# facebookresearch/momentum

Hardware: AMD Instinct MI355X
Metric: character IK solves/sec (72-joint, 10 GN iters) (higher is better)
Workload: dtype f32; 1 GPU; BASELINE configs[1]: B x 72-joint humanoid, P=128, pos+ori on 16 landmarks (M=192), GN lambda=0.05, 10 it; batch_per_gpu=4096, global_batch=4096, joints=72, params=128, rows=192, solved_parameters=96, route=fused, line_search=0, precision=f32

## Files before the change

### include/mmx.h

```cpp
#ifndef MMX_H_
#define MMX_H_

#include <stddef.h>
#include <stdint.h>

#ifdef __cplusplus
extern "C" {
#endif

#define MMX_ABI_VERSION 12
#define MMX_PARAMS_PER_JOINT 7
#define MMX_INVALID_PARENT (-1)
#define MMX_MAX_MODEL_PARAMS 2048

typedef enum mmx_status {
  MMX_OK = 0,
  MMX_ERR_INVALID_ARGUMENT = 1,
  MMX_ERR_SIZE_MISMATCH = 2,
  MMX_ERR_DEVICE = 3,
  MMX_ERR_UNSUPPORTED = 4,
  MMX_ERR_OUT_OF_MEMORY = 5,
  MMX_ERR_NO_DEVICE = 6
} mmx_status;

// ... 135 lines not shown
} mmx_gn_options;

typedef struct mmx_rig mmx_rig;
typedef struct mmx_problem mmx_problem;

void mmx_gn_options_default(mmx_gn_options* opt);

int32_t mmx_abi_version(void);
const char* mmx_last_error(void);
int32_t mmx_device_count(void);

int32_t mmx_rig_create(const mmx_rig_desc* desc, int32_t device, mmx_rig** out);
void mmx_rig_destroy(mmx_rig* rig);
int32_t mmx_rig_num_joints(const mmx_rig* rig);
int32_t mmx_rig_num_params(const mmx_rig* rig);

int32_t mmx_problem_create(
    mmx_rig* rig,
    int32_t batch,
    int32_t num_pos,
    const int32_t* pos_parent,
    int32_t num_ori,
    const int32_t* ori_parent,
    mmx_problem** out);
void mmx_problem_destroy(mmx_problem* problem);

int32_t mmx_problem_set_instance_rig(
    mmx_problem* problem,
    const float* translation_offset,
    const float* pre_rotation,
    int32_t memory,
    void* stream);

int32_t mmx_problem_set_instance_parents(
    mmx_problem* problem,
    const int32_t* pos_parent,
    const int32_t* ori_parent,
    int32_t memory,
    void* stream);

#define MMX_ROUTE_AUTO 0
#define MMX_ROUTE_FUSED 1
#define MMX_ROUTE_WIDE 2
#define MMX_ROUTE_EXPLICIT_JACOBIAN 3
#define MMX_ROUTE_WAVE 4
#define MMX_WAVE_MAX_JOINTS 64
#define MMX_WAVE_MAX_SOLVED 32
#define MMX_WAVE_MAX_UNITS 192
typedef struct mmx_tuning {
  int32_t route;
  int32_t max_refinement_steps;
  float mixed_tolerance;
  int32_t mixed_max_cg;
  int32_t reserved[4];
} mmx_tuning;
int32_t mmx_problem_set_tuning(mmx_problem* problem, const mmx_tuning* tuning);
int32_t mmx_problem_last_route(const mmx_problem* problem);

int32_t mmx_problem_num_rows(const mmx_problem* problem);
int32_t mmx_problem_batch(const mmx_problem* problem);

int32_t mmx_problem_set_enabled(mmx_problem* problem, const uint8_t* enabled);

int32_t mmx_problem_set_constraints(
    mmx_problem* problem,
    const mmx_constraint_data* data,
    void* stream);
int32_t mmx_problem_set_constraints_sized(
    mmx_problem* problem,
    const mmx_constraint_data* data,
    size_t data_size,
    void* stream);

int32_t mmx_eval_jacobian(
    mmx_problem* problem,
    const float* theta_dev,
    float* jac_dev,
    float* res_dev,
    double* err_dev,
    int32_t layout,
    void* stream);

int32_t mmx_eval_jacobian_timed(
    mmx_problem* problem,
    const float* theta_dev,
    float* jac_dev,
    float* res_dev,
    double* err_dev,
    int32_t layout,
    void* stream,
    float* kernel_ms);

int32_t mmx_debug_store_pattern(mmx_problem* problem, float* jac_dev, void* stream, float* kernel_ms);

int32_t mmx_eval_skeleton_state(
    mmx_problem* problem,
    const float* theta_dev,
    float* state_dev,
    void* stream);

int32_t mmx_eval_normal_equations(
    mmx_problem* problem,
    const float* theta_dev,
    float* jtj_dev,
    float* jtr_dev,
    double* err_dev,
    void* stream);

int32_t mmx_solve(
    mmx_problem* problem,
// ... 48 lines not shown
    int32_t* solve_list_host,
    int32_t* num_solved,
    void* stream);

int32_t mmx_debug_tree_normal_equations(mmx_problem* problem, const float* theta_dev, float* jtj_dev, float* jtr_dev, void* stream);

int32_t mmx_solve_host(
    mmx_problem* problem,
    const mmx_gn_options* options,
    float* theta_host,
    double* final_error_host,
    int32_t* iterations_host,
    int32_t* status_host);
int32_t mmx_solve_f64_host(
    mmx_problem* problem,
    const mmx_gn_options* options,
    double* theta_host,
    double* final_error_host,
    int32_t* iterations_host,
    int32_t* status_host);
int32_t mmx_eval_jacobian_host(
    mmx_problem* problem,
    const float* theta_host,
    float* jac_host,
    float* res_host,
    double* err_host,
    int32_t layout);
int32_t mmx_eval_skeleton_state_host(mmx_problem* problem, const float* theta_host, float* state_host);

#define MMX_COMM_ID_BYTES 128
typedef struct mmx_comm mmx_comm;
int32_t mmx_comm_unique_id(uint8_t id[MMX_COMM_ID_BYTES]);
int32_t mmx_comm_create(const uint8_t id[MMX_COMM_ID_BYTES], int32_t world_size, int32_t rank, int32_t device, mmx_comm** out);
int32_t mmx_comm_create_all(int32_t num_devices, const int32_t* devices, mmx_comm** out );
int32_t mmx_comm_world_size(const mmx_comm* comm);
int32_t mmx_comm_rank(const mmx_comm* comm);
int32_t mmx_comm_all_reduce_norms(mmx_comm* comm, double* norms_dev, void* stream);
int32_t mmx_comm_all_reduce_norms_host(mmx_comm* comm, double norms_host[3]);
int32_t mmx_residual_norms(int32_t batch, const double* final_error, const int32_t* iterations, const int32_t* status, double* norms_dev, void* stream);
void mmx_comm_destroy(mmx_comm* comm);

int32_t mmx_host_tables(
    const mmx_rig_desc* desc,
    const uint8_t* enabled,
    int32_t* level,
    int32_t* tin,
    int32_t* tout,
    uint8_t* active_joint_params,
    int32_t* enabled_list,
    int32_t* num_enabled);

int32_t mmx_host_elimination_order(const mmx_rig_desc* desc, const uint8_t* enabled, int32_t* order, int32_t* num_enabled);
int32_t mmx_host_tile_structure(int32_t n, const uint8_t* related, uint32_t* row_mask, uint32_t* col_mask, int64_t* products);
int32_t mmx_problem_tile_structure(mmx_problem* problem, uint32_t* row_mask, uint32_t* col_mask, int32_t* num_blocks, int32_t* num_tiles, int64_t* products);
int32_t mmx_host_tile_level_schedule(int32_t n, const uint8_t* related, int32_t* steps);
int32_t mmx_host_f64_assembly_list(
    const mmx_rig_desc* desc,
    const int32_t* solve_list,
    int32_t n,
    const int32_t* pos_parent,
    int32_t num_pos,
    const int32_t* ori_parent,
    int32_t num_ori,
    int32_t units_per_chunk,
    uint32_t* groups,
    int32_t* num_groups,
    int32_t* extra,
    int32_t* num_extra,
    int32_t* chunk_start,
    int32_t* num_chunks);

#ifdef __cplusplus
}
#endif
#endif
```

### momentum_amd/_abi.py

```python
from __future__ import annotations

import ctypes as C

import numpy as np

c_float_p = C.POINTER(C.c_float)
c_double_p = C.POINTER(C.c_double)
c_int32_p = C.POINTER(C.c_int32)
c_uint8_p = C.POINTER(C.c_uint8)

MMX_ABI_VERSION = 12
MMX_OK = 0
MMX_SOLVE_OK, MMX_SOLVE_NONFINITE, MMX_SOLVE_NOT_PD = 0, 1, 2
MMX_SOLVE_DAMPING_FLOORED = 4
MMX_SOLVE_PRECISION_SUSPECT = 8
MMX_SOLVE_ESCALATED_F64 = 16
MMX_SOLVE_MIXED = 32
MMX_SOLVE_ERROR_MASK = 3
MMX_PRECISION_F32, MMX_PRECISION_F64, MMX_PRECISION_AUTO, MMX_PRECISION_MIXED = 0, 1, 2, 3
MMX_MEM_HOST, MMX_MEM_DEVICE = 0, 1
MMX_LAYOUT_COL_MAJOR, MMX_LAYOUT_ROW_MAJOR = 0, 1
MMX_STEP_GN_FIXED_LAMBDA, MMX_STEP_LM_SCHEDULE, MMX_STEP_TRUST_REGION = 0, 1, 2


# ... 249 lines not shown
        ("do_line_search", C.c_int32),
        ("step_rule", C.c_int32),
        ("lm_lambda_min", C.c_float),
        ("lm_lambda_max", C.c_float),
        ("lm_up", C.c_float),
        ("lm_down", C.c_float),
        ("trust_region_radius", C.c_float),
        ("precision", C.c_int32),
        ("precision_bound", C.c_float),
    ]

    @classmethod
    def make(
        cls,
        min_iterations=1,
        max_iterations=2,
        threshold=1.0,
        regularization=0.05,
        do_line_search=False,
        step_rule=MMX_STEP_GN_FIXED_LAMBDA,
        lm_lambda_min=1e-6,
        lm_lambda_max=1e6,
        lm_up=4.0,
        lm_down=0.5,
        trust_region_radius=1.0,
        precision=MMX_PRECISION_F32,
        precision_bound=1e-5,
    ) -> "GnOptions":
        return cls(
            int(min_iterations),
            int(max_iterations),
            float(threshold),
            float(regularization),
            int(do_line_search),
            int(step_rule),
            float(lm_lambda_min),
            float(lm_lambda_max),
            float(lm_up),
            float(lm_down),
            float(trust_region_radius),
            int(precision),
            float(precision_bound),
        )


ROUTES = {"auto": 0, "fused": 1, "wide": 2, "explicit_jacobian": 3, "wave": 4}
WAVE_MAX_JOINTS = 64
WAVE_MAX_SOLVED = 32
WAVE_MAX_UNITS = 192


class Tuning(C.Structure):

    _fields_ = [("route", C.c_int32), ("max_refinement_steps", C.c_int32), ("mixed_tolerance", C.c_float), ("mixed_max_cg", C.c_int32), ("reserved", C.c_int32 * 4)]


def as_ptr(a: np.ndarray, ctype):
    assert a.flags["C_CONTIGUOUS"], "array must be C-contiguous"
    return a.ctypes.data_as(C.POINTER(ctype))


def void_p(a) -> C.c_void_p:
    if a is None:
        return C.c_void_p(0)
    if isinstance(a, np.ndarray):
        assert a.flags["C_CONTIGUOUS"]
        return C.c_void_p(a.ctypes.data)
    return C.c_void_p(int(a))
```

### momentum_amd/capi.py

```python
from __future__ import annotations

import ctypes as C
import os
from typing import Optional

import numpy as np

from . import _abi
from ._abi import ConstraintData, GnOptions, RigDesc, as_ptr
from .rigs import Rig

_HERE = os.path.dirname(os.path.abspath(__file__))
LIB_PATH = os.environ.get("MMX_LIB") or os.path.join(_HERE, "libmmx_hip.so")
_lib: Optional[C.CDLL] = None

SYMBOLS = [
    "mmx_gn_options_default", "mmx_abi_version", "mmx_last_error", "mmx_device_count",
    "mmx_rig_create", "mmx_rig_destroy", "mmx_rig_num_joints", "mmx_rig_num_params",
    "mmx_problem_create", "mmx_problem_destroy", "mmx_problem_num_rows", "mmx_problem_batch",
    "mmx_problem_set_tuning", "mmx_problem_last_route",
    "mmx_problem_set_enabled", "mmx_problem_set_constraints", "mmx_problem_set_constraints_sized", "mmx_problem_set_instance_rig", "mmx_problem_set_instance_parents", "mmx_eval_jacobian", "mmx_eval_jacobian_timed", "mmx_debug_store_pattern",
    "mmx_eval_skeleton_state", "mmx_eval_normal_equations", "mmx_solve", "mmx_solve_with_history", "mmx_solve_with_step_history", "mmx_problem_solve_diagnostics", "mmx_solve_f64", "mmx_solve_f64_host", "mmx_solve_host",
    "mmx_eval_jacobian_host", "mmx_eval_skeleton_state_host", "mmx_host_tables", "mmx_debug_fused_normal_equations", "mmx_debug_tree_normal_equations",
    "mmx_host_elimination_order", "mmx_host_tile_structure", "mmx_host_tile_level_schedule", "mmx_host_f64_assembly_list", "mmx_problem_tile_structure",
    "mmx_comm_unique_id", "mmx_comm_create", "mmx_comm_create_all", "mmx_comm_world_size", "mmx_comm_rank",
    "mmx_comm_all_reduce_norms", "mmx_comm_all_reduce_norms_host", "mmx_residual_norms", "mmx_comm_destroy",
]


class MmxError(RuntimeError):

    def __init__(self, code: int, msg: str):
        super().__init__(f"mmx error {code}: {msg}")
        self.code = code


def lib() -> C.CDLL:
    global _lib
    if _lib is not None:
        return _lib
    if not os.path.exists(LIB_PATH):
        raise MmxError(-1, f"{LIB_PATH} is missing: build it with `python -m momentum_amd.build` (no CPU fallback exists)")
    try:
        import torch
    except Exception:
        pass
    L = C.CDLL(LIB_PATH)
    vp, i32 = C.c_void_p, C.c_int32
    L.mmx_last_error.restype = C.c_char_p
    L.mmx_gn_options_default.restype = None
    L.mmx_gn_options_default.argtypes = [C.POINTER(GnOptions)]
    L.mmx_rig_create.argtypes = [C.POINTER(RigDesc), i32, C.POINTER(vp)]
    L.mmx_rig_destroy.argtypes = [vp]
    L.mmx_rig_destroy.restype = None
    L.mmx_rig_num_joints.argtypes = [vp]
    L.mmx_rig_num_params.argtypes = [vp]
    L.mmx_problem_create.argtypes = [vp, i32, i32, _abi.c_int32_p, i32, _abi.c_int32_p, C.POINTER(vp)]
    L.mmx_problem_destroy.argtypes = [vp]
    L.mmx_problem_destroy.restype = None
    L.mmx_problem_num_rows.argtypes = [vp]
    L.mmx_problem_batch.argtypes = [vp]
    L.mmx_problem_set_enabled.argtypes = [vp, _abi.c_uint8_p]
    L.mmx_problem_set_tuning.argtypes = [vp, C.POINTER(_abi.Tuning)]
    L.mmx_problem_last_route.argtypes = [vp]
    L.mmx_problem_set_constraints.argtypes = [vp, C.POINTER(ConstraintData), vp]
    L.mmx_problem_set_constraints_sized.argtypes = [vp, C.POINTER(ConstraintData), C.c_size_t, vp]
    L.mmx_problem_set_instance_rig.argtypes = [vp, vp, vp, i32, vp]
    L.mmx_problem_set_instance_parents.argtypes = [vp, vp, vp, i32, vp]
    L.mmx_eval_jacobian.argtypes = [vp, vp, vp, vp, vp, i32, vp]
    L.mmx_eval_jacobian_timed.argtypes = [vp, vp, vp, vp, vp, i32, vp, C.POINTER(C.c_float)]
    L.mmx_debug_store_pattern.argtypes = [vp, vp, vp, C.POINTER(C.c_float)]
    L.mmx_eval_skeleton_state.argtypes = [vp, vp, vp, vp]
    L.mmx_eval_normal_equations.argtypes = [vp, vp, vp, vp, vp, vp]
    L.mmx_solve.argtypes = [vp, C.POINTER(GnOptions), vp, vp, vp, vp, vp, vp]
    L.mmx_solve_with_history.argtypes = [vp, C.POINTER(GnOptions), vp, vp, vp, vp, vp, vp, vp]
    L.mmx_solve_with_step_history.argtypes = [vp, C.POINTER(GnOptions), vp, vp, vp, vp, vp, vp, vp, vp]
    L.mmx_problem_solve_diagnostics.argtypes = [vp, vp, vp]
    L.mmx_solve_f64.argtypes = [vp, C.POINTER(GnOptions), vp, vp, vp, vp, vp, vp]
    L.mmx_solve_host.argtypes = [vp, C.POINTER(GnOptions), vp, vp, vp, vp]
    L.mmx_solve_f64_host.argtypes = [vp, C.POINTER(GnOptions), vp, vp, vp, vp]
    L.mmx_eval_jacobian_host.argtypes = [vp, vp, vp, vp, vp, i32]
    L.mmx_eval_skeleton_state_host.argtypes = [vp, vp, vp]
    L.mmx_debug_tree_normal_equations.argtypes = [vp, vp, vp, vp, vp]
    L.mmx_debug_fused_normal_equations.argtypes = [vp, vp, vp, vp, _abi.c_int32_p, _abi.c_int32_p, vp]
    L.mmx_comm_unique_id.argtypes = [vp]
    L.mmx_comm_create.argtypes = [vp, i32, i32, i32, C.POINTER(vp)]
    L.mmx_comm_create_all.argtypes = [i32, _abi.c_int32_p, C.POINTER(vp)]
    L.mmx_comm_world_size.argtypes = [vp]
    L.mmx_comm_rank.argtypes = [vp]
    L.mmx_comm_all_reduce_norms.argtypes = [vp, vp, vp]
    L.mmx_comm_all_reduce_norms_host.argtypes = [vp, vp]
    L.mmx_residual_norms.argtypes = [i32, vp, vp, vp, vp, vp]
    L.mmx_comm_destroy.argtypes = [vp]
    L.mmx_comm_destroy.restype = None
    L.mmx_host_tables.argtypes = [
        C.POINTER(RigDesc), _abi.c_uint8_p, _abi.c_int32_p, _abi.c_int32_p, _abi.c_int32_p,
        _abi.c_uint8_p, _abi.c_int32_p, _abi.c_int32_p,
    ]
    u32p, i64p = C.POINTER(C.c_uint32), C.POINTER(C.c_int64)
    L.mmx_host_elimination_order.argtypes = [C.POINTER(RigDesc), _abi.c_uint8_p, _abi.c_int32_p, _abi.c_int32_p]
    L.mmx_host_tile_structure.argtypes = [i32, _abi.c_uint8_p, u32p, u32p, i64p]
    L.mmx_host_tile_level_schedule.argtypes = [i32, _abi.c_uint8_p, C.POINTER(C.c_int32)]
    L.mmx_problem_tile_structure.argtypes = [vp, u32p, u32p, _abi.c_int32_p, _abi.c_int32_p, i64p]
    _lib = L
    return L


def _check(rc: int) -> None:
    if rc != 0:
        raise MmxError(rc, lib().mmx_last_error().decode("utf-8", "replace"))


def device_count() -> int:
    return int(lib().mmx_device_count())


def host_tables(rig: Rig, enabled=None) -> dict:
    J, P = rig.num_joints, rig.num_params
    level, tin, tout = (np.zeros(J, np.int32) for _ in range(3))
    active = np.zeros(7 * J, np.uint8)
    elist = np.zeros(P, np.int32)
    n = C.c_int32(0)
    d = rig.desc()
    if enabled is None:
        eptr = _abi.c_uint8_p()
    else:
        e = np.ascontiguousarray(enabled, dtype=np.uint8)
        eptr = as_ptr(e, C.c_uint8)
    _check(
        lib().mmx_host_tables(
            C.byref(d), eptr, as_ptr(level, C.c_int32), as_ptr(tin, C.c_int32), as_ptr(tout, C.c_int32),
            as_ptr(active, C.c_uint8), as_ptr(elist, C.c_int32), C.byref(n),
        )
    )
    order = np.zeros(P, np.int32)
    _check(lib().mmx_host_elimination_order(C.byref(d), eptr, as_ptr(order, C.c_int32), C.byref(n)))
    return dict(level=level, tin=tin, tout=tout, active_joint_params=active, enabled_list=elist[: n.value].copy(),
                elimination_order=order[: n.value].copy())


def host_tile_structure(related: np.ndarray):
    rel = np.ascontiguousarray(related, dtype=np.uint8)
    n = rel.shape[0]
    assert rel.shape == (n, n)
    row, col = np.zeros(32, np.uint32), np.zeros(32, np.uint32)
    prod = C.c_int64(0)
    _check(lib().mmx_host_tile_structure(C.c_int32(n), as_ptr(rel, C.c_uint8), as_ptr(row, C.c_uint32), as_ptr(col, C.c_uint32), C.byref(prod)))
    return dict(row_mask=row, col_mask=col, products=prod.value)


def host_tile_level_schedule(related: np.ndarray):
    rel = np.ascontiguousarray(related, dtype=np.uint8)
    n = rel.shape[0]
    assert rel.shape == (n, n)
    words = np.zeros(1 + 4 * 32, np.int32)
    _check(lib().mmx_host_tile_level_schedule(C.c_int32(n), as_ptr(rel, C.c_uint8), as_ptr(words, C.c_int32)))
    steps = []
    for s in range(int(words[0])):
        steps.append([(int(w) & 0xff, (int(w) >> 8) & 0xf, (int(w) >> 12) & 0xf) for w in words[1 + 4 * s : 5 + 4 * s] if w >= 0])
    return steps


def host_f64_assembly_list(rig: Rig, solve_list, pos_parent, ori_parent, units_per_chunk: int):
    sl = np.ascontiguousarray(solve_list, dtype=np.int32)
    pp = np.ascontiguousarray(pos_parent, dtype=np.int32)
    op = np.ascontiguousarray(ori_parent, dtype=np.int32)
    d = rig.desc()
    ng, ne, nc = C.c_int32(0), C.c_int32(0), C.c_int32(0)
    i32p = C.POINTER(C.c_int32)
    args = lambda g, e, cs: (C.byref(d), as_ptr(sl, C.c_int32), C.c_int32(len(sl)), as_ptr(pp, C.c_int32), C.c_int32(len(pp)), as_ptr(op, C.c_int32),
                             C.c_int32(len(op)), C.c_int32(units_per_chunk), g, C.byref(ng), e, C.byref(ne), cs, C.byref(nc))
    f = lib().mmx_host_f64_assembly_list
    f.restype = C.c_int32
    _check(f(*args(None, None, None)))
    groups = np.zeros(2 * max(ng.value, 1), np.uint32)
    extra = np.zeros(max(ne.value, 1), np.int32)
    cstart = np.zeros(2 * nc.value + 1, np.int32)
    _check(f(*args(groups.ctypes.data_as(C.POINTER(C.c_uint32)), extra.ctypes.data_as(i32p), cstart.ctypes.data_as(i32p))))
    chunks = []
    for ch in range(nc.value):
        entries = []
        for g in range(cstart[ch], cstart[ch + 1]):
            w0, w1 = int(groups[2 * g]), int(groups[2 * g + 1])
            c, ul, count = w0 & 0xfff, (w0 >> 12) & 0x3f, w0 >> 18
            entries.append((c, ul, [w1] if count == 1 else [int(x) for x in extra[w1 : w1 + count]]))
        chunks.append(dict(block_mask=int(cstart[nc.value + 1 + ch]), entries=entries))
    return chunks


def _stream_ptr() -> C.c_void_p:
    import torch
# ... 26 lines not shown
            pass


default_route = "auto"


class Problem:

    def __init__(self, rig_handle: RigHandle, batch: int, pos_parent, ori_parent):
        import torch

        self.rh = rig_handle
        self.B = int(batch)
        self.P = rig_handle.rig.num_params
        self.J = rig_handle.rig.num_joints
        self.pos_parent = np.ascontiguousarray(pos_parent, dtype=np.int32).reshape(-1)
        self.ori_parent = np.ascontiguousarray(ori_parent, dtype=np.int32).reshape(-1)
        self.Kp, self.Ko = len(self.pos_parent), len(self.ori_parent)
        self.M = 3 * self.Kp + 9 * self.Ko
        self.n = self.P
        self.device = torch.device("cuda", rig_handle.device)
        self._h = C.c_void_p(0)
        self._keep = []
        _check(
            lib().mmx_problem_create(
                rig_handle._h, self.B, self.Kp, as_ptr(self.pos_parent, C.c_int32), self.Ko,
                as_ptr(self.ori_parent, C.c_int32), C.byref(self._h),
            )
        )
        self._prefer_wide = default_route == "prefer_wide"
        if default_route not in ("auto", "prefer_wide"):
            self.set_route(default_route)

    def close(self) -> None:
        if self._h:
            lib().mmx_problem_destroy(self._h)
            self._h = C.c_void_p(0)

    def __del__(self):
        try:
            self.close()
        except Exception:
            pass

    def set_route(self, route: str, max_refinement_steps: int = 0) -> None:
        self._prefer_wide = default_route == "prefer_wide" and route == "auto"
        self._set_tuning(route, max_refinement_steps)

    def _set_tuning(self, route: str, max_refinement_steps: int = 0) -> None:
        t = _abi.Tuning()
        t.route = _abi.ROUTES[route]
        t.max_refinement_steps = int(max_refinement_steps)
        t.mixed_tolerance, t.mixed_max_cg = getattr(self, "_mixed", (0.0, 0))
        self._route_args = (route, int(max_refinement_steps))
        _check(lib().mmx_problem_set_tuning(self._h, C.byref(t)))

    def set_mixed(self, tolerance: float = 0.0, max_cg: int = 0) -> None:
        self._mixed = (float(tolerance), int(max_cg))
        self._set_tuning(*getattr(self, "_route_args", ("auto", 0)))

    def last_route(self) -> str:
        r = int(lib().mmx_problem_last_route(self._h))
        return {v: k for k, v in _abi.ROUTES.items()}[r]

    def set_enabled(self, enabled) -> None:
        e = np.ascontiguousarray(enabled, dtype=np.uint8).reshape(-1)
        assert e.shape[0] == self.P
        _check(lib().mmx_problem_set_enabled(self._h, as_ptr(e, C.c_uint8)))
        self.n = int(np.count_nonzero(e))

    def set_constraints(
        self, pos_offset, pos_target, pos_weight, ori_offset, ori_target, ori_weight,
        pos_function_weight: float = 1.0, ori_function_weight: float = 1.0,
        limits=None, limit_function_weight: float = 1.0,
        model_target=None, model_weights=None, model_function_weight: float = 1.0,
        pos_loss=(2.0, 1.0), ori_loss=(2.0, 1.0), joint_blocks=None, ellipsoid_limits=None, function_weights=None,
    ) -> None:
        import torch

        arrs = [pos_offset, pos_target, pos_weight, ori_offset, ori_target, ori_weight]
        shapes = [(self.B, self.Kp, 3), (self.B, self.Kp, 3), (self.B, self.Kp), (self.B, self.Ko, 4), (self.B, self.Ko, 4), (self.B, self.Ko)]
        if model_target is not None:
            arrs += [model_target, model_weights]
            shapes += [(self.B, self.P), (self.B, self.P)]
        on_dev = all(isinstance(a, torch.Tensor) for a in arrs)
        keep, ptrs = [], []
        for a, shp in zip(arrs, shapes):
            if on_dev:
                assert a.is_cuda and a.dtype == torch.float32 and a.is_contiguous() and tuple(a.shape) == shp, (a.shape, shp)
                keep.append(a)
                ptrs.append(C.c_void_p(a.data_ptr() if a.numel() else 0))
            else:
                x = np.ascontiguousarray(a, dtype=np.float32).reshape(shp)
                keep.append(x)
                ptrs.append(C.c_void_p(x.ctypes.data if x.size else 0))
        if model_target is None:
            ptrs += [C.c_void_p(0), C.c_void_p(0)]
        fw_ptr, fw_cols = C.c_void_p(0), 0
        if function_weights is not None:
            if on_dev:
                assert function_weights.is_cuda and function_weights.dtype == torch.float32 and function_weights.is_contiguous() and function_weights.shape[0] == self.B
                keep.append(function_weights)
                fw_ptr, fw_cols = C.c_void_p(function_weights.data_ptr()), int(function_weights.shape[1])
            else:
                fwh = np.ascontiguousarray(function_weights, dtype=np.float32).reshape(self.B, -1)
                keep.append(fwh)
                fw_ptr, fw_cols = C.c_void_p(fwh.ctypes.data), int(fwh.shape[1])
        limits = list(limits) if limits else []
        larr = _abi.limit_array(limits)
        blocks = list(joint_blocks) if joint_blocks else []
        bkeep: list = []
        barr = _abi.joint_block_array(blocks, bkeep, self.B, on_dev)
# ... 285 lines not shown
```

### momentum_amd/csrc/mmx_capi.hip

```cpp
#include "../../include/mmx.h"

#include <hip/hip_runtime.h>

#include <dlfcn.h>

#include <cfloat>
#include <cmath>
#include <cstdio>
#include <cstdlib>
#include <cstring>
#include <algorithm>
#include <new>
#include <map>
#include <memory>
#include <string>
#include <vector>

#include "mmx_host_tables.hpp"
#include "mmx_kernels.hpp"

namespace {

thread_local std::string g_lastError;

// ... 142 lines not shown
  DevBuf oInstOffset, oInstPreRot, oInstPosParent, oInstOriParent, dJointTin;
  std::vector<int32_t> unionPos, unionOri;
  std::vector<int32_t> instPosHost, instOriHost;
  bool instParentsFromHost = false;
  bool instPos = false, instOri = false;
  mmx::HostTables tables;
  mmx::FusedTables fused;
  DevBuf dUnitJoint, dUnitTin, dColStart, dColSources, dEnabledList, dJacRecs, dMultiCols, dZeroCols;
  DevBuf dSubSize, dPosUnitStart, dPosUnits, dSolveList, dSrcStart, dSrcs, dTerms, dTerms16, dComb, dDfsJoint, dLoadedPos;
  DevBuf dLimStart, dLimOf, dPairDest, dPairStart, dPairLim, dPairCols;
  mmx::FusedDev fdev{};
  DevBuf oPosOffset, oPosTarget, oPosWeight, oOriOffset, oOriTarget, oOriWeight, oMpTarget, oMpWeights, dLimits, dEnabledMask, oFnWeights;
  std::vector<mmx_parameter_limit> limits;
  struct JointBlockHost {
    int32_t type = 0, count = 0;
    std::vector<int32_t> parent;
    std::vector<int32_t> parentB;
    DevBuf oLocalPoint, oLocalDir, oGlobal, oPlaneD, oWeight, oProjection;
  };
  std::vector<std::unique_ptr<JointBlockHost>> blocks;
  std::vector<mmx::JointBlockDev> blockDev;
  std::vector<mmx_ellipsoid_limit> ellipsoids;
  DevBuf dEllipsoids;
  DevBuf dBlocks, dGenJoint, dGenTin, dGenBlock;
  int32_t genRows = 0;
  bool haveConstraints = false;
  bool tablesDirty = false;
  mmx::ProblemDev dev{};
  int32_t solveN = 0;
  DevBuf dSolveListV1;
  DevBuf sHess2F64;
  DevBuf dSolveListF64;
  std::vector<int32_t> solveListF64;
  std::vector<std::pair<int32_t, int32_t>> limitPairs;
  DevBuf dTileMasks, dTileList;
  mmx::TileMasks tileMasks;
  std::vector<int32_t> solveListV1;
  DevBuf sJac, sRes, sErr, sJtj, sJtr, sFactor, sThetaInit, sTheta;
  DevBuf sTreeState, sDvec, sRhoVec, sRefState, sGenState;
  DevBuf sJacColMajor;
  DevBuf sJacF64, sHessF64;
  DevBuf dF64Groups, dF64Extra, dF64ChunkStart;
  int32_t f64ListUnitsPerChunk = 0;
  DevBuf sDone, sIters, sStatus, sLastErr, sFinalErr, sHist, sClk, sDelta, sStepIter, sLambda, sTrust;
  DevBuf sFusedArgs;
  DevBuf sDiag;
  DevBuf sDiagAcc;
  DevBuf sDiagErr0;
  bool diagValid = false;
  DevBuf sThetaAuto, sAutoMap, sAutoCount;
  bool autoAbort = false;
  mmx_tuning tuning{};
  int32_t lastRoute = MMX_ROUTE_AUTO;
};

namespace {

std::vector<int32_t> limitParameters(const mmx_rig* rig, const mmx_parameter_limit& lm) {
  std::vector<int32_t> out;
  auto add = [&](int32_t p) {
    if (std::find(out.begin(), out.end(), p) == out.end()) {
      out.push_back(p);
    }
  };
  auto addRow = [&](int32_t row) {
    for (int32_t k = rig->ptOuter[size_t(row)]; k < rig->ptOuter[size_t(row) + 1]; ++k) {
      add(rig->ptInner[size_t(k)]);
    }
  };
  switch (lm.type) {
    case MMX_LIMIT_MINMAX:
      add(lm.index0);
      break;
    case MMX_LIMIT_LINEAR:
    case MMX_LIMIT_HALFPLANE:
      add(lm.index0);
      add(lm.index1);
      break;
    case MMX_LIMIT_MINMAX_JOINT:
      addRow(lm.index0);
      break;
    case MMX_LIMIT_LINEAR_JOINT:
      addRow(lm.index1);
      addRow(lm.index0);
      break;
    default:
      break;
  }
  return out;
}

int32_t uploadProblemTables(mmx_problem* pb) {
  const mmx_rig* rig = pb->rig;
  MMX_HIP(hipSetDevice(rig->device));
  const mmx::HostTables& t = pb->tables;
  std::vector<int32_t> unitJoint(size_t(std::max(pb->U, 1))), unitTin(size_t(std::max(pb->U, 1)));
  for (int32_t c = 0; c < pb->Kp; ++c) {
    unitJoint[c] = pb->posParent[c];
  }
  for (int32_t c = 0; c < pb->Ko; ++c) {
    for (int k = 0; k < 3; ++k) {
      unitJoint[pb->Kp + 3 * c + k] = pb->oriParent[c];
    }
  }
  for (int32_t u = 0; u < pb->U; ++u) {
    unitTin[u] = t.tin[unitJoint[u]];
  }
  static_assert(sizeof(mmx::ColumnSource) == sizeof(mmx::ColumnSourceDev), "ColumnSource layouts must match");
  MMX_HIP(upload(pb->dUnitJoint, unitJoint));
  MMX_HIP(upload(pb->dUnitTin, unitTin));
  MMX_HIP(upload(pb->dJointTin, t.tin));
  pb->dev.jointTin = pb->dJointTin.as<int32_t>();
  {
    std::vector<int32_t> gj, gt, gb, gj2, gt2;
    for (size_t i = 0; i < pb->blocks.size(); ++i) {
      const mmx_problem::JointBlockHost& h = *pb->blocks[i];
      for (size_t c = 0; c < h.parent.size(); ++c) {
        const int32_t j = h.parent[c], j2 = h.parentB.empty() ? -1 : h.parentB[c];
        gj.push_back(j);
        gt.push_back(t.tin[size_t(j)]);
        gb.push_back(int32_t(i));
        gj2.push_back(j2);
        gt2.push_back(j2 < 0 ? -1 : t.tin[size_t(j2)]);
      }
    }
    const size_t G = gb.size();
    gj.insert(gj.end(), gj2.begin(), gj2.end());
    gt.insert(gt.end(), gt2.begin(), gt2.end());
    MMX_HIP(upload(pb->dGenJoint, gj));
    MMX_HIP(upload(pb->dGenTin, gt));
    MMX_HIP(upload(pb->dGenBlock, gb));
    MMX_HIP(upload(pb->dBlocks, pb->blockDev));
    pb->dev.numBlocks = int32_t(pb->blocks.size());
    pb->dev.G = int32_t(G);
    pb->dev.blocks = pb->dBlocks.as<mmx::JointBlockDev>();
    pb->dev.genJoint = pb->dGenJoint.as<int32_t>();
    pb->dev.genTin = pb->dGenTin.as<int32_t>();
    pb->dev.genBlock = pb->dGenBlock.as<int32_t>();
    std::vector<mmx::EllipsoidDev> ed(pb->ellipsoids.size());
    for (size_t i = 0; i < ed.size(); ++i) {
      const mmx_ellipsoid_limit& e = pb->ellipsoids[i];
      static_assert(sizeof(mmx_ellipsoid_limit) == 30 * 4 && sizeof(mmx::EllipsoidDev) == 32 * 4, "ellipsoid layouts");
// ... 317 lines not shown
      std::map<int32_t, std::vector<int32_t>> pairs;
      std::map<int32_t, std::pair<int32_t, int32_t>> pairColumns;
      for (size_t l = 0; l < pb->limits.size(); ++l) {
        std::vector<int32_t> cols;
        for (int32_t p : limitParameters(rig, pb->limits[l])) {
          if (colOf[size_t(p)] >= 0) {
            cols.push_back(colOf[size_t(p)]);
          }
        }
        for (int32_t c : cols) {
          per[size_t(c)].push_back(int32_t(l));
        }
        for (size_t x = 0; x < cols.size(); ++x) {
          for (size_t y = x + 1; y < cols.size(); ++y) {
            const int32_t row = std::max(cols[x], cols[y]), col = std::min(cols[x], cols[y]);
            const int I = row >> 4, Jc = col >> 4, r = row & 15, c = col & 15;
            const int32_t dest = (I * (I + 1) / 2 + Jc) * 256 + r * 16 + ((((c >> 2) ^ (r >> 2)) & 3) << 2) + (c & 3);
            pairs[dest].push_back(int32_t(l));
            pairColumns[dest] = {row, col};
          }
        }
      }
      std::vector<int32_t> limStart(1, 0), limOf, pairDest, pairStart(1, 0), pairLim;
      for (int32_t c = 0; c < fd.n; ++c) {
        limOf.insert(limOf.end(), per[size_t(c)].begin(), per[size_t(c)].end());
        limStart.push_back(int32_t(limOf.size()));
      }
      std::vector<int32_t> pairCols;
      for (const auto& kv : pairs) {
        pairDest.push_back(kv.first);
        pairCols.push_back(pairColumns[kv.first].first);
        pairCols.push_back(pairColumns[kv.first].second);
        pb->limitPairs.push_back(pairColumns[kv.first]);
        pairLim.insert(pairLim.end(), kv.second.begin(), kv.second.end());
        pairStart.push_back(int32_t(pairLim.size()));
      }
      MMX_HIP(upload(pb->dPairCols, pairCols));
      fd.pairCols = pb->dPairCols.as<int32_t>();
      MMX_HIP(upload(pb->dLimStart, limStart));
      MMX_HIP(upload(pb->dLimOf, limOf));
      MMX_HIP(upload(pb->dPairDest, pairDest));
      MMX_HIP(upload(pb->dPairStart, pairStart));
      MMX_HIP(upload(pb->dPairLim, pairLim));
      fd.numLimits = int32_t(pb->limits.size());
      fd.limStart = pb->dLimStart.as<int32_t>();
      fd.limOf = pb->dLimOf.as<int32_t>();
      fd.numPairDests = int32_t(pairDest.size());
      fd.pairDest = pb->dPairDest.as<int32_t>();
      fd.pairStart = pb->dPairStart.as<int32_t>();
      fd.pairLim = pb->dPairLim.as<int32_t>();
    }
    pb->fdev.GT = pb->dev.G + int32_t(pb->ellipsoids.size());
    pb->fdev.genRows = pb->fdev.GT > 0 ? pb->dev.rowsJoint - 3 * pb->U : 0;
  }
  {
    const size_t J = size_t(rig->J);
    std::vector<uint8_t> anyBelow(J, 0), pointBelow(J, 0);
    auto mark = [&](int32_t joint, bool point) {
      for (int32_t a = joint; a >= 0; a = rig->parent[size_t(a)]) {
        anyBelow[size_t(a)] = 1;
        if (point) {
          pointBelow[size_t(a)] = 1;
        }
      }
    };
    for (int32_t c = 0; c < pb->Kp; ++c) {
      mark(pb->posParent[size_t(c)], true);
    }
    for (int32_t c = 0; c < pb->Ko; ++c) {
      mark(pb->oriParent[size_t(c)], false);
    }
    if (pb->instPos) {
      for (int32_t j : pb->unionPos) {
        mark(j, true);
      }
    }
    if (pb->instOri) {
      for (int32_t j : pb->unionOri) {
        mark(j, false);
      }
    }
    for (const auto& h : pb->blocks) {
      const bool fixedAxis = h->type == MMX_JC_FIXED_AXIS_DIFF || h->type == MMX_JC_FIXED_AXIS_COS || h->type == MMX_JC_FIXED_AXIS_ANGLE;
      for (int32_t j : h->parent) {
        mark(j, !fixedAxis);
      }
      for (int32_t j : h->parentB) {
        mark(j, true);
      }
    }
    for (const mmx_ellipsoid_limit& e : pb->ellipsoids) {
      mark(e.parent, true);
    }
    std::vector<uint8_t> keep(size_t(rig->P), pb->dev.hasModel ? 1 : 0);
    for (const mmx_parameter_limit& lm : pb->limits) {
      for (int32_t p : limitParameters(rig, lm)) {
        keep[size_t(p)] = 1;
      }
    }
    std::vector<int32_t> list;
    for (int32_t p : t.eliminationList) {
      bool nz = keep[size_t(p)] != 0;
      for (int32_t e = t.colStart[size_t(p)]; !nz && e < t.colStart[size_t(p) + 1]; ++e) {
        const mmx::ColumnSource& cs = t.colSources[size_t(e)];
        nz = (cs.dof >= 3 && cs.dof < 6) ? anyBelow[size_t(cs.joint)] != 0 : pointBelow[size_t(cs.joint)] != 0;
      }
// ... 25 lines not shown
        for (int32_t e = f.srcStart[size_t(c)]; e < f.srcStart[size_t(c) + 1]; ++e) {
          const mmx::ColumnSource& cs = f.srcs[size_t(e)];
          for (int32_t k = cs.tin; k < cs.tout; ++k) {
            rc[size_t(f.dfsJoint[size_t(k)])] = 1;
          }
          for (int32_t a = cs.parent; a >= 0; a = rig->parent[size_t(a)]) {
            rc[size_t(a)] = 1;
          }
        }
      }
      related.assign(size_t(n) * size_t(n), 0);
      for (int32_t row = 0; row < n; ++row) {
        for (int32_t col = 0; col < row; ++col) {
          const uint8_t* rc = reach.data() + size_t(col) * J;
          bool any = false;
          for (int32_t e = f.srcStart[size_t(row)]; !any && e < f.srcStart[size_t(row) + 1]; ++e) {
            any = rc[size_t(f.srcs[size_t(e)].joint)] != 0;
          }
          related[size_t(row) * size_t(n) + size_t(col)] = any ? 1 : 0;
        }
      }
      for (const auto& rcPair : pb->limitPairs) {
        related[size_t(rcPair.first) * size_t(n) + size_t(rcPair.second)] = 1;
      }
    }
    pb->tileMasks = mmx::eliminationTileMasks(std::min(n, 512), related, dense);
    std::vector<uint32_t> masks(96, 0u);
    uint32_t base = 0;
    for (int i = 0; i < 32; ++i) {
      masks[size_t(i)] = pb->tileMasks.rowMask[i];
      masks[size_t(32 + i)] = pb->tileMasks.colMask[i];
      masks[size_t(64 + i)] = base;
      base += uint32_t(__builtin_popcount(pb->tileMasks.colMask[i]));
    }
    for (int k = 0; k < pb->tileMasks.NB && k < 32; ++k) {
      for (int I = k; I < 32; ++I) {
        if (pb->tileMasks.colMask[k] >> I & 1u) {
          masks.push_back(uint32_t(I) | uint32_t(k) << 8);
        }
      }
    }
    for (int32_t w : pb->tileMasks.levelSteps) {
      masks.push_back(uint32_t(w));
    }
    MMX_HIP(upload(pb->dTileMasks, masks));
    MMX_HIP(upload(pb->dTileList, pb->tileMasks.tiles));
    pb->fdev.tileList = pb->dTileList.as<int32_t>();
    pb->fdev.numTiles = int32_t(pb->tileMasks.tiles.size());
  }

  return MMX_OK;
}

bool fusedUsable(const mmx_problem* pb) {
  const int nb = mmx::fusedBlocksFor(pb->fdev.n);
  if (nb < 0) {
    return false;
  }
  return pb->rig->J < 4096 &&
      mmx::fusedLdsBytes(nb, pb->rig->J, pb->rig->P, pb->U, pb->fdev.nsrc, pb->fdev.n, pb->fdev.numCells, true, pb->fdev.GT, pb->fdev.genRows, true, mmx::fusedCsrFloats(pb->rig->J, pb->fdev.nnz)) +
          size_t(8) * size_t(pb->rig->J + pb->rig->P) <=
      160 * 1024;
}

bool treeNormalEquationsUsable(const mmx_problem* pb) {
  return pb->U > 0 && pb->fdev.n > 0 && pb->fdev.n <= 512 && pb->fdev.nsrc < 4096 &&
      pb->fused.solveList == pb->solveListV1 &&
      mmx::treeNormalEquationsLdsBytes(pb->rig->J, pb->rig->P, pb->U, pb->fdev.nsrc, pb->fdev.n, pb->fdev.GT, pb->fdev.genRows) <= 160 * 1024 - 64 &&
      mmx::treeRefineLdsBytes(pb->rig->J, pb->rig->P, pb->U, pb->fdev.n, pb->fdev.genRows) <= 160 * 1024 - 64;
}

int32_t refineSteps(const mmx_problem* pb) {
  const int32_t m = pb->tuning.max_refinement_steps;
  return m == 0 ? 3 : (m < 0 ? 0 : (m > 3 ? 3 : m));
}

bool phaseClocksWanted() {
  static const bool wanted = getenv("MMX_PHASE_CLOCKS") != nullptr;
  return wanted;
}

hipError_t armPhaseStop(long long* clk, hipStream_t s) {
  static const long long stop = getenv("MMX_PHASE_STOP") != nullptr ? atoll(getenv("MMX_PHASE_STOP")) + 1 : 0;
  return stop > 0 ? hipMemcpyAsync(clk + 31, &stop, sizeof(long long), hipMemcpyHostToDevice, s) : hipSuccess;
}

int32_t checkProblem(const mmx_problem* pb, bool needConstraints) {
  (void)hipGetLastError();
  if (pb == nullptr || pb->rig == nullptr) {
    return fail(MMX_ERR_INVALID_ARGUMENT, "problem handle is null");
  }
  if (needConstraints && !pb->haveConstraints && pb->U > 0) {
    return fail(MMX_ERR_INVALID_ARGUMENT, "mmx_problem_set_constraints has not been called");
  }
  return MMX_OK;
}

}

extern "C" {

void mmx_gn_options_default(mmx_gn_options* o) {
  if (o == nullptr) {
    return;
  }
  o->min_iterations = 1;
// ... 26 lines not shown
    return 0;
  }
  return n;
}

int32_t mmx_host_tables(
    const mmx_rig_desc* desc,
    const uint8_t* enabled,
    int32_t* level,
    int32_t* tin,
    int32_t* tout,
    uint8_t* active_joint_params,
    int32_t* enabled_list,
    int32_t* num_enabled) {
  mmx::HostTables t;
  std::string err;
  const int32_t rc = mmx::buildHostTables(desc, enabled, t, err);
  if (rc != MMX_OK) {
    return fail(rc, err);
  }
  if (level) {
    std::memcpy(level, t.level.data(), sizeof(int32_t) * t.J);
  }
  if (tin) {
    std::memcpy(tin, t.tin.data(), sizeof(int32_t) * t.J);
  }
  if (tout) {
    std::memcpy(tout, t.tout.data(), sizeof(int32_t) * t.J);
  }
  if (active_joint_params) {
    std::memcpy(active_joint_params, t.activeJointParams.data(), t.activeJointParams.size());
  }
  if (enabled_list) {
    std::memcpy(enabled_list, t.enabledList.data(), sizeof(int32_t) * t.enabledList.size());
  }
  if (num_enabled) {
    *num_enabled = int32_t(t.enabledList.size());
  }
  return MMX_OK;
}

int32_t mmx_host_elimination_order(const mmx_rig_desc* desc, const uint8_t* enabled, int32_t* order, int32_t* num_enabled) {
  mmx::HostTables t;
  std::string err;
  const int32_t rc = mmx::buildHostTables(desc, enabled, t, err);
  if (rc != MMX_OK) {
    return fail(rc, err);
  }
  if (order) {
    std::memcpy(order, t.eliminationList.data(), sizeof(int32_t) * t.eliminationList.size());
  }
  if (num_enabled) {
    *num_enabled = int32_t(t.eliminationList.size());
  }
  return MMX_OK;
}

int32_t mmx_host_tile_structure(int32_t n, const uint8_t* related, uint32_t* row_mask, uint32_t* col_mask, int64_t* products) {
  if (n < 0 || n > 512 || (n > 0 && related == nullptr)) {
    return fail(MMX_ERR_INVALID_ARGUMENT, "mmx_host_tile_structure: n outside 0..512 or related is null");
  }
  const std::vector<uint8_t> rel(related, related + size_t(n) * size_t(n));
  const mmx::TileMasks m = mmx::eliminationTileMasks(n, rel, false);
  for (int i = 0; i < 32; ++i) {
    if (row_mask) {
      row_mask[i] = m.rowMask[i];
    }
    if (col_mask) {
      col_mask[i] = m.colMask[i];
    }
  }
  if (products) {
    *products = m.products;
  }
  return MMX_OK;
}

int32_t mmx_host_tile_level_schedule(int32_t n, const uint8_t* related, int32_t* steps) {
  if (n < 0 || n > 512 || (n > 0 && related == nullptr) || steps == nullptr) {
    return fail(MMX_ERR_INVALID_ARGUMENT, "mmx_host_tile_level_schedule: n outside 0..512, or related / steps is null");
  }
  const std::vector<uint8_t> rel(related, related + size_t(n) * size_t(n));
  const mmx::TileMasks m = mmx::eliminationTileMasks(n, rel, false);
  if (m.levelSteps.size() > size_t(1 + 4 * 32)) {
    return fail(MMX_ERR_UNSUPPORTED, "mmx_host_tile_level_schedule: more than 32 steps");
  }
  std::copy(m.levelSteps.begin(), m.levelSteps.end(), steps);
  return MMX_OK;
}

int32_t mmx_host_f64_assembly_list(
    const mmx_rig_desc* desc,
    const int32_t* solve_list,
    int32_t n,
    const int32_t* pos_parent,
    int32_t num_pos,
    const int32_t* ori_parent,
    int32_t num_ori,
    int32_t units_per_chunk,
    uint32_t* groups,
    int32_t* num_groups,
    int32_t* extra,
    int32_t* num_extra,
    int32_t* chunk_start,
    int32_t* num_chunks) {
  if (n < 0 || num_pos < 0 || num_ori < 0 || units_per_chunk <= 0 || units_per_chunk > 64 || (n > 0 && solve_list == nullptr) ||
// ... 82 lines not shown
    return fail(rc, err);
  }
  const int ndev = mmx_device_count();
  if (ndev <= 0) {
    return fail(MMX_ERR_NO_DEVICE, "no HIP device visible; the MI355X path has no CPU fallback");
  }
  if (device < 0 || device >= ndev) {
    return fail(MMX_ERR_INVALID_ARGUMENT, "device index out of range");
  }
  mmx_rig* r = new (std::nothrow) mmx_rig();
  if (r == nullptr) {
    return fail(MMX_ERR_OUT_OF_MEMORY, "host allocation failed");
  }
  r->device = device;
  r->J = d->num_joints;
  r->P = d->num_params;
  const int32_t R = MMX_PARAMS_PER_JOINT * r->J;
  r->parent.assign(d->parent, d->parent + r->J);
  r->preRot.assign(d->pre_rotation, d->pre_rotation + 4 * r->J);
  r->offset.assign(d->translation_offset, d->translation_offset + 3 * r->J);
  r->ptOuter.assign(d->pt_outer, d->pt_outer + R + 1);
  const int32_t nnz = r->ptOuter[R];
  r->ptInner.assign(d->pt_inner, d->pt_inner + nnz);
  r->ptValue.assign(d->pt_value, d->pt_value + nnz);
  if (d->pt_offsets != nullptr) {
    r->ptOffsets.assign(d->pt_offsets, d->pt_offsets + R);
  } else {
    r->ptOffsets.assign(R, 0.f);
  }
  r->topo = std::move(topo);
  auto cleanup = [&](int32_t code) {
    delete r;
    return code;
  };
  if (hipSetDevice(device) != hipSuccess) {
    return cleanup(fail(MMX_ERR_DEVICE, "hipSetDevice failed"));
  }
#define UP(buf, vec)                                                             \
  do {                                                                           \
    hipError_t e_ = upload(buf, vec);                                            \
    if (e_ != hipSuccess) {                                                      \
      return cleanup(fail(MMX_ERR_DEVICE, std::string("rig upload: ") + hipGetErrorString(e_))); \
    }                                                                            \
  } while (0)
  UP(r->dParent, r->parent);
  UP(r->dPreRot, r->preRot);
  UP(r->dOffset, r->offset);
  UP(r->dPtOuter, r->ptOuter);
  UP(r->dPtInner, r->ptInner);
  UP(r->dPtValue, r->ptValue);
  UP(r->dPtOffsets, r->ptOffsets);
  UP(r->dLevelOrder, r->topo.levelOrder);
  UP(r->dLevelStart, r->topo.levelStart);
  std::vector<int32_t> ell(size_t(R) * 4, 0), jumpParent(size_t(r->J));
  bool ellOk = true;
  for (int32_t row = 0; row < R; ++row) {
    const int32_t k0 = r->ptOuter[row], k1 = r->ptOuter[row + 1];
    if (k1 - k0 > 2) {
      ellOk = false;
      break;
    }
    for (int s = 0; s < 2; ++s) {
      int32_t idx = -1, bits = 0;
      if (k0 + s < k1) {
        idx = r->ptInner[k0 + s];
        std::memcpy(&bits, &r->ptValue[k0 + s], 4);
      }
      ell[4 * size_t(row) + 2 * s] = idx;
      ell[4 * size_t(row) + 2 * s + 1] = bits;
    }
  }
  for (int32_t j = 0; j < r->J; ++j) {
    jumpParent[j] = ((r->parent[j] + 1) << 16) | (r->parent[j] + 1);
  }
  if (ellOk) {
    UP(r->dPtEll, ell);
  }
  UP(r->dJumpParent, jumpParent);
  std::vector<int32_t> rowRec;
  if (R < 65536 && r->P <= 65535) {
    std::vector<int32_t> rows;
    for (int32_t row = 0; row < R; ++row) {
      if (r->ptOuter[row + 1] > r->ptOuter[row]) {
        rows.push_back(row);
      }
    }
    for (size_t t = 0; t < rows.size(); ++t) {
      const int32_t row = rows[t], next = t + 1 < rows.size() ? rows[t + 1] : R;
      const int32_t k0 = r->ptOuter[row], cnt = r->ptOuter[row + 1] - k0;
      if (cnt > 65535 || next - row > 65535) {
        rowRec.clear();
        break;
      }
      int32_t bits = 0;
      std::memcpy(&bits, &r->ptValue[k0], 4);
      rowRec.insert(rowRec.end(), {row | ((next - row) << 16), r->ptInner[k0] | (cnt << 16), bits, k0});
    }
    if (!rowRec.empty()) {
      UP(r->dPtRowRec, rowRec);
    }
  }
#undef UP
  mmx::RigDev& dv = r->dev;
  dv.ptRowRec = rowRec.empty() ? nullptr : r->dPtRowRec.as<int4>();
  dv.numRowRec = int32_t(rowRec.size() / 4);
  dv.ptEll = ellOk ? r->dPtEll.as<int4>() : nullptr;
  dv.jumpParent = r->dJumpParent.as<int32_t>();
  dv.jumpRounds = 0;
  while ((1 << dv.jumpRounds) < int32_t(r->topo.levelStart.size()) - 1) {
    ++dv.jumpRounds;
  }
  dv.J = r->J;
  dv.P = r->P;
  dv.R = R;
  dv.numLevels = int32_t(r->topo.levelStart.size()) - 1;
  dv.parent = r->dParent.as<int32_t>();
  dv.preRot = r->dPreRot.as<float>();
  dv.offset = r->dOffset.as<float>();
  dv.ptOuter = r->dPtOuter.as<int32_t>();
  dv.ptInner = r->dPtInner.as<int32_t>();
  dv.ptValue = r->dPtValue.as<float>();
  dv.ptOffsets = r->dPtOffsets.as<float>();
  dv.ptOffsetsNonZero = 0;
  for (float v : r->ptOffsets) {
    dv.ptOffsetsNonZero |= v != 0.f ? 1 : 0;
  }
  dv.levelOrder = r->dLevelOrder.as<int32_t>();
  dv.levelStart = r->dLevelStart.as<int32_t>();
  *out = r;
  return MMX_OK;
}

void mmx_rig_destroy(mmx_rig* rig) {
  if (rig != nullptr) {
    (void)hipSetDevice(rig->device);
    delete rig;
  }
}

int32_t mmx_rig_num_joints(const mmx_rig* rig) {
  return rig ? rig->J : 0;
}
int32_t mmx_rig_num_params(const mmx_rig* rig) {
  return rig ? rig->P : 0;
}

int32_t mmx_problem_create(
    mmx_rig* rig,
    int32_t batch,
    int32_t num_pos,
    const int32_t* pos_parent,
    int32_t num_ori,
    const int32_t* ori_parent,
    mmx_problem** out) {
  MMX_ZONE("mmx_problem_create");
  if (out == nullptr) {
    return fail(MMX_ERR_INVALID_ARGUMENT, "out is null");
  }
  *out = nullptr;
  if (rig == nullptr) {
    return fail(MMX_ERR_INVALID_ARGUMENT, "rig handle is null");
  }
  if (batch <= 0 || num_pos < 0 || num_ori < 0) {
    return fail(MMX_ERR_INVALID_ARGUMENT, "batch must be > 0 and constraint counts >= 0");
  }
// ... 24 lines not shown
  pb->dev.lossOri = mmx::LossDev{0, 2.f, 1.f, 1.f};
  if (num_pos > 0) {
    pb->posParent.assign(pos_parent, pos_parent + num_pos);
  }
  if (num_ori > 0) {
    pb->oriParent.assign(ori_parent, ori_parent + num_ori);
  }
  pb->tables = rig->topo;
  pb->rigDev = rig->dev;
  pb->dev.wPos = 1.f;
  pb->dev.wOri = 1.f;
  const int32_t rc = uploadProblemTables(pb);
  if (rc != MMX_OK) {
    delete pb;
    return rc;
  }
  *out = pb;
  return MMX_OK;
}

void mmx_problem_destroy(mmx_problem* pb) {
  if (pb != nullptr) {
    if (pb->rig != nullptr) {
      (void)hipSetDevice(pb->rig->device);
    }
    delete pb;
  }
}

int32_t mmx_problem_num_rows(const mmx_problem* pb) {
  return pb ? pb->M : 0;
}
int32_t mmx_problem_batch(const mmx_problem* pb) {
  return pb ? pb->B : 0;
}

int32_t mmx_problem_set_tuning(mmx_problem* pb, const mmx_tuning* tuning) {
  int32_t rc = checkProblem(pb, false);
  if (rc != MMX_OK) {
    return rc;
  }
  if (tuning == nullptr) {
    return fail(MMX_ERR_INVALID_ARGUMENT, "tuning is null");
  }
  if (tuning->route < MMX_ROUTE_AUTO || tuning->route > MMX_ROUTE_WAVE) {
    return fail(MMX_ERR_INVALID_ARGUMENT, "mmx_tuning::route: unknown MMX_ROUTE_* value");
  }
  if (tuning->max_refinement_steps < -1 || tuning->max_refinement_steps > 3) {
    return fail(MMX_ERR_INVALID_ARGUMENT, "mmx_tuning::max_refinement_steps: -1 (none), 0 (default) or 1..3");
  }
  if (!(tuning->mixed_tolerance >= 0.f) || tuning->mixed_tolerance > 1e-2f || tuning->mixed_max_cg < 0 || tuning->mixed_max_cg > 64) {
    return fail(MMX_ERR_INVALID_ARGUMENT, "mmx_tuning::mixed_tolerance: 0 (default) or (0, 1e-2]; mixed_max_cg: 0 (default) or 1..64");
  }
  for (int32_t r : tuning->reserved) {
    if (r != 0) {
      return fail(MMX_ERR_INVALID_ARGUMENT, "mmx_tuning::reserved must be zero");
    }
  }
  pb->tuning = *tuning;
  return MMX_OK;
}

int32_t mmx_problem_last_route(const mmx_problem* pb) {
  return pb != nullptr ? pb->lastRoute : MMX_ROUTE_AUTO;
}

int32_t mmx_problem_set_enabled(mmx_problem* pb, const uint8_t* enabled) {
  MMX_ZONE("mmx_problem_set_enabled");
  int32_t rc = checkProblem(pb, false);
  if (rc != MMX_OK) {
    return rc;
  }
  if (enabled == nullptr) {
    return fail(MMX_ERR_INVALID_ARGUMENT, "enabled is null");
  }
  if (!pb->tablesDirty && pb->tables.enabled.size() == size_t(pb->rig->P)) {
    bool same = true;
    for (size_t p = 0; p < pb->tables.enabled.size() && same; ++p) {
      same = (pb->tables.enabled[p] != 0) == (enabled[p] != 0);
    }
    if (same) {
      return MMX_OK;
    }
  }
  const mmx_rig_desc d = pb->rig->desc();
  std::string err;
  mmx::HostTables t;
  rc = mmx::buildHostTables(&d, enabled, t, err);
  if (rc != MMX_OK) {
    return fail(rc, err);
  }
  pb->tables = std::move(t);
  return uploadProblemTables(pb);
}

int32_t mmx_problem_set_instance_rig(mmx_problem* pb, const float* translation_offset, const float* pre_rotation, int32_t memory, void* stream) {
  MMX_ZONE("mmx_problem_set_instance_rig");
  int32_t rc = checkProblem(pb, false);
  if (rc != MMX_OK) {
    return rc;
  }
  if (memory != MMX_MEM_HOST && memory != MMX_MEM_DEVICE) {
    return fail(MMX_ERR_INVALID_ARGUMENT, "instance rig: unknown memory space");
  }
  MMX_HIP(hipSetDevice(pb->rig->device));
  hipStream_t s = static_cast<hipStream_t>(stream);
  const size_t B = size_t(pb->B), J = size_t(pb->rig->J);
  auto bring = [&](DevBuf& buf, const float* src, size_t count, const float*& dst) -> hipError_t {
    if (src == nullptr) {
      dst = nullptr;
      return hipSuccess;
    }
    if (memory == MMX_MEM_DEVICE) {
      dst = src;
      return hipSuccess;
    }
    hipError_t e = buf.ensure(count * sizeof(float));
// ... 542 lines not shown
  MMX_HIP(pb->sErr.ensure(B * sizeof(double)));
  MMX_HIP(pb->sJtj.ensure(B * n * n * sizeof(float)));
  MMX_HIP(pb->sJtr.ensure(B * n * sizeof(float)));
  return MMX_OK;
}
}

int32_t mmx_eval_normal_equations(
    mmx_problem* pb,
    const float* theta_dev,
    float* jtj_dev,
    float* jtr_dev,
    double* err_dev,
    void* stream) {
  MMX_ZONE("mmx_eval_normal_equations (Get JtJ and JtR)");
  int32_t rc = checkProblem(pb, true);
  if (rc != MMX_OK) {
    return rc;
  }
  if (theta_dev == nullptr || jtj_dev == nullptr || jtr_dev == nullptr) {
    return fail(MMX_ERR_INVALID_ARGUMENT, "theta / jtj / jtr is null");
  }
  if (pb->dev.n > mmx::kMaxSolved) {
    return fail(MMX_ERR_UNSUPPORTED, "more than 2048 enabled parameters (kMaxModelParams)");
  }
  MMX_HIP(hipSetDevice(pb->rig->device));
  hipStream_t s = static_cast<hipStream_t>(stream);
  rc = ensureStepScratch(pb);
  if (rc != MMX_OK) {
    return rc;
  }
  MMX_HIP(mmx::launchFkJacobian(
      pb->rigDev, pb->dev, theta_dev, pb->sJac.as<float>(), pb->sRes.as<float>(), err_dev, nullptr, nullptr, s));
  MMX_HIP(mmx::launchNormalEquations(
      pb->dev, pb->rig->P, pb->sJac.as<float>(), pb->sRes.as<float>(), jtj_dev, jtr_dev, nullptr, false, s));
  return MMX_OK;
}

int32_t mmx_debug_tree_normal_equations(mmx_problem* pb, const float* theta_dev, float* jtj_dev, float* jtr_dev, void* stream) {
  MMX_ZONE("mmx_debug_tree_normal_equations");
  int32_t rc = checkProblem(pb, true);
  if (rc != MMX_OK) {
    return rc;
  }
  if (theta_dev == nullptr || jtj_dev == nullptr || jtr_dev == nullptr) {
    return fail(MMX_ERR_INVALID_ARGUMENT, "theta / jtj / jtr is null");
  }
  if (!treeNormalEquationsUsable(pb) || pb->solveN != pb->dev.n) {
    return fail(MMX_ERR_UNSUPPORTED, "mmx_debug_tree_normal_equations: problem outside the tree-moment kernel's scope (or structurally zero columns present)");
  }
  MMX_HIP(hipSetDevice(pb->rig->device));
  hipStream_t s = static_cast<hipStream_t>(stream);
  MMX_HIP(mmx::zeroAsync(jtj_dev, size_t(pb->B) * size_t(pb->dev.n) * size_t(pb->dev.n) * sizeof(float), s));
  MMX_HIP(mmx::launchTreeNormalEquations(pb->rigDev, pb->dev, pb->fdev, theta_dev, jtj_dev, jtr_dev, nullptr, nullptr, nullptr, nullptr, nullptr, false, s));
  return MMX_OK;
}

static int32_t solveImpl(
    mmx_problem* pb,
    const mmx_gn_options* o,
    float* theta_dev,
    double* final_error,
    int32_t* iterations,
    int32_t* status,
    double* error_history,
    float* parameter_history,
    double* step_history,
    void* stream);

int32_t mmx_solve(
    mmx_problem* pb,
    const mmx_gn_options* o,
    float* theta_dev,
    double* final_error,
    int32_t* iterations,
    int32_t* status,
    double* error_history,
    void* stream) {
  return solveImpl(pb, o, theta_dev, final_error, iterations, status, error_history, nullptr, nullptr, stream);
}

int32_t mmx_solve_with_history(
    mmx_problem* pb,
    const mmx_gn_options* o,
    float* theta_dev,
    double* final_error,
    int32_t* iterations,
    int32_t* status,
    double* error_history,
    float* parameter_history,
    void* stream) {
  return solveImpl(pb, o, theta_dev, final_error, iterations, status, error_history, parameter_history, nullptr, stream);
}

int32_t mmx_solve_with_step_history(
    mmx_problem* pb,
    const mmx_gn_options* o,
    float* theta_dev,
    double* final_error,
    int32_t* iterations,
    int32_t* status,
    double* error_history,
    float* parameter_history,
    double* step_history,
    void* stream) {
  if (step_history != nullptr && o != nullptr && o->step_rule != MMX_STEP_LM_SCHEDULE) {
    return fail(MMX_ERR_INVALID_ARGUMENT, "mmx_solve_with_step_history: step_history is the LM schedule's (MMX_STEP_LM_SCHEDULE)");
// ... 115 lines not shown
    return fail(MMX_ERR_INVALID_ARGUMENT, "unknown do_line_search rule");
  }
  const size_t B = size_t(pb->B), P = size_t(pb->rig->P);
  hipStream_t s = static_cast<hipStream_t>(stream);
  const bool escalation = sel.map != nullptr;
  pb->lastRoute = MMX_ROUTE_FUSED;
  MMX_HIP(pb->sIters.ensure(B * sizeof(int32_t)));
  MMX_HIP(pb->sStatus.ensure(B * sizeof(int32_t)));
  MMX_HIP(pb->sFinalErr.ensure(B * sizeof(double)));
  mmx::SolveStateDev fst{};
  fst.iterations = iterations != nullptr ? iterations : pb->sIters.as<int32_t>();
  fst.status = status != nullptr ? status : pb->sStatus.as<int32_t>();
  fst.finalError = final_error != nullptr ? final_error : pb->sFinalErr.as<double>();
  fst.errorHistory = error_history;
  fst.paramHistory = parameter_history;
  fst.stepHistory = step_history;
  if (!escalation) {
    MMX_HIP(pb->sDiag.ensure(B * 4 * sizeof(float)));
    fst.diag = pb->sDiag.as<float>();
    pb->diagValid = true;
    if (step_history != nullptr && o->max_iterations > 0) {
      MMX_HIP(mmx::zeroAsync(step_history, B * size_t(o->max_iterations) * 2 * sizeof(double), s));
    }
    if (error_history != nullptr && o->max_iterations > 0) {
      MMX_HIP(mmx::zeroAsync(error_history, B * size_t(o->max_iterations) * sizeof(double), s));
    }
    if (parameter_history != nullptr && o->max_iterations > 0) {
      MMX_HIP(mmx::zeroAsync(parameter_history, B * size_t(o->max_iterations) * P * sizeof(float), s));
    }
  }
  fst.precisionBound = o->precision_bound > 0.f ? o->precision_bound : 1e-5f;
  mmx::FusedParams fp{};
  fp.lambda = o->regularization;
  fp.threshold = o->threshold;
  fp.minIterations = o->min_iterations;
  fp.maxIterations = o->max_iterations;
  fp.refine = 0;
  fp.doLineSearch = o->do_line_search;
  fp.stepRule = o->step_rule;
  fp.lmLambdaMin = o->lm_lambda_min;
  fp.lmLambdaMax = o->lm_lambda_max;
  fp.lmUp = o->lm_up;
  fp.lmDown = o->lm_down;
  fp.trustRadius = 1.f;
  fp.mixTol = pb->tuning.mixed_tolerance > 0.f ? pb->tuning.mixed_tolerance : 3e-9f;
  fp.mixMaxCg = pb->tuning.mixed_max_cg > 0 ? pb->tuning.mixed_max_cg : 12;
  long long* clk = nullptr;
  if (phaseClocksWanted()) {
    MMX_HIP(pb->sClk.ensure(32 * sizeof(long long)));
    MMX_HIP(hipMemsetAsync(pb->sClk.p, 0, 32 * sizeof(long long), s));
    clk = pb->sClk.as<long long>();
    MMX_HIP(armPhaseStop(clk, s));
  }
  MMX_HIP(mmx::launchFusedMixed(pb->rigDev, pb->dev, pb->fdev, theta_dev, fst, fp, sel, pb->B, clk, s));
  if (clk != nullptr) {
    long long h[32];
    MMX_HIP(hipMemcpyAsync(h, clk, sizeof(h), hipMemcpyDeviceToHost, s));
    MMX_HIP(hipStreamSynchronize(s));
    static const char* names[24] = {"-", "A-C fk + units (double)", "(reused state)", "D subtree sums", "E srcTables", "F g (double adjoint)",
                                    "G combine + pull", "H cholesky(tail)", "-", "-", "K update",
                                    "G extras: records", "G term records", "H.bc panel", "H.d mfma", "D own sums", "CG z0 solve + rz",
                                    "CG operator (double)", "CG decide + direction", "CG dots + update", "CG solve", "G extras: loads", "H.b load+barrier", "H.b chain"};
    long long tot = 0;
    for (int i = 0; i < 24; ++i) {
      tot += h[i];
    }
    fprintf(stderr, "[mmx phase clocks, MIXED, block 0, all iterations] total %lld\n", tot);
    for (int i = 0; i < 24; ++i) {
      fprintf(stderr, "  %-26s %10lld  %5.1f%%\n", names[i], h[i], 100.0 * double(h[i]) / double(tot > 0 ? tot : 1));
    }
  }
  return MMX_OK;
}

static int32_t solveImpl(
    mmx_problem* pb,
    const mmx_gn_options* o,
    float* theta_dev,
    double* final_error,
    int32_t* iterations,
    int32_t* status,
    double* error_history,
    float* parameter_history,
    double* step_history,
    void* stream) {
  if (o == nullptr || o->precision == MMX_PRECISION_F32) {
    return solveF32Impl(pb, o, theta_dev, final_error, iterations, status, error_history, parameter_history, step_history, stream);
  }
  if (o->precision != MMX_PRECISION_F64 && o->precision != MMX_PRECISION_AUTO && o->precision != MMX_PRECISION_MIXED) {
    return fail(MMX_ERR_INVALID_ARGUMENT, "unknown precision (MMX_PRECISION_*)");
  }
  int32_t rc = checkProblem(pb, true);
  if (rc != MMX_OK) {
    return rc;
  }
  if (theta_dev == nullptr) {
    return fail(MMX_ERR_INVALID_ARGUMENT, "options / theta is null");
  }
  if (pb->tuning.route == MMX_ROUTE_WAVE) {
    return fail(MMX_ERR_UNSUPPORTED, "MMX_ROUTE_WAVE: only MMX_PRECISION_F32 (not F64 / AUTO / MIXED)");
  }
  const bool mixedOk = mixedUsable(pb, o);
  if (parameter_history != nullptr && !(o->precision == MMX_PRECISION_MIXED && mixedOk)) {
    return fail(MMX_ERR_UNSUPPORTED, "parameter_history is single precision's (MMX_PRECISION_F32) and the mixed-precision instantiation's: the double instantiation does not record it");
  }
  const size_t B = size_t(pb->B), P = size_t(pb->rig->P);
  MMX_HIP(hipSetDevice(pb->rig->device));
// ... 57 lines not shown
    return fail(MMX_ERR_INVALID_ARGUMENT, "options / theta is null");
  }
  if (o->max_iterations < 0 || o->min_iterations < 0) {
    return fail(MMX_ERR_INVALID_ARGUMENT, "iteration counts must be >= 0");
  }
  if (o->step_rule != MMX_STEP_GN_FIXED_LAMBDA && o->step_rule != MMX_STEP_LM_SCHEDULE && o->step_rule != MMX_STEP_TRUST_REGION) {
    return fail(MMX_ERR_INVALID_ARGUMENT, "unknown step_rule");
  }
  if (o->do_line_search != MMX_LINE_SEARCH_NONE && o->do_line_search != MMX_LINE_SEARCH_GAUSS_NEWTON &&
      o->do_line_search != MMX_LINE_SEARCH_DIRECTIONAL) {
    return fail(MMX_ERR_INVALID_ARGUMENT, "unknown do_line_search rule");
  }
  const size_t B = size_t(pb->B), P = size_t(pb->rig->P);
  mmx::ProblemDev ds = pb->dev;
  ds.n = pb->solveN;
  ds.enabledList = pb->dSolveListV1.as<int32_t>();
  const int n = ds.n;
  MMX_HIP(hipSetDevice(pb->rig->device));
  hipStream_t s = static_cast<hipStream_t>(stream);
  const int32_t route = pb->tuning.route;
  if (route == MMX_ROUTE_WAVE) {
    if (const char* why = waveRefusal(pb, o)) {
      return fail(MMX_ERR_UNSUPPORTED, why);
    }
    if (step_history != nullptr) {
      return fail(MMX_ERR_UNSUPPORTED, "MMX_ROUTE_WAVE: step_history is the LM schedule's");
    }
    pb->lastRoute = MMX_ROUTE_WAVE;
    pb->diagValid = false;
    MMX_HIP(pb->sIters.ensure(B * sizeof(int32_t)));
    MMX_HIP(pb->sStatus.ensure(B * sizeof(int32_t)));
    MMX_HIP(pb->sFinalErr.ensure(B * sizeof(double)));
    mmx::SolveStateDev wst{};
    wst.iterations = iterations != nullptr ? iterations : pb->sIters.as<int32_t>();
    wst.status = status != nullptr ? status : pb->sStatus.as<int32_t>();
    wst.finalError = final_error != nullptr ? final_error : pb->sFinalErr.as<double>();
    wst.errorHistory = error_history;
    wst.paramHistory = parameter_history;
    if (error_history != nullptr && o->max_iterations > 0) {
      MMX_HIP(mmx::zeroAsync(error_history, B * size_t(o->max_iterations) * sizeof(double), s));
    }
    if (parameter_history != nullptr && o->max_iterations > 0) {
      MMX_HIP(mmx::zeroAsync(parameter_history, B * size_t(o->max_iterations) * P * sizeof(float), s));
    }
    mmx::FusedParams wp{};
    wp.lambda = o->regularization;
    wp.threshold = o->threshold;
    wp.minIterations = o->min_iterations;
    wp.maxIterations = o->max_iterations;
    wp.refine = refineSteps(pb);
    wp.doLineSearch = o->do_line_search;
    wp.stepRule = o->step_rule;
    MMX_ZONE("wave solve: all iterations in one launch, one wavefront per instance");
    MMX_HIP(mmx::launchWaveSolve(pb->rigDev, pb->dev, pb->fdev, theta_dev, wst, wp, s));
    return MMX_OK;
  }
  const bool forceWide = route == MMX_ROUTE_WIDE;
  const bool trust = o->step_rule == MMX_STEP_TRUST_REGION;
  const bool trustNeedsWide = trust && (!fusedUsable(pb) || pb->fdev.GT > 0);
  const bool preferWide = (forceWide || trustNeedsWide || (!trust && mmx::fusedBlocksFor(pb->fdev.n) >= 10)) &&
      treeNormalEquationsUsable(pb) && route != MMX_ROUTE_FUSED && route != MMX_ROUTE_EXPLICIT_JACOBIAN;
  const bool legacy = route == MMX_ROUTE_EXPLICIT_JACOBIAN;
  const bool takeFused = fusedUsable(pb) && !legacy && !preferWide && !(pb->fdev.GT > 0 && o->step_rule == MMX_STEP_TRUST_REGION);
  if (route == MMX_ROUTE_FUSED && !takeFused) {
    return fail(MMX_ERR_UNSUPPORTED, "MMX_ROUTE_FUSED: the problem does not fit the one-launch solve (more than 224 solved parameters, or its tables beyond the LDS budget)");
  }
  if (route == MMX_ROUTE_WIDE && !preferWide) {
    return fail(MMX_ERR_UNSUPPORTED, "MMX_ROUTE_WIDE: the problem is outside the tree kernels' scope");
  }
  if (takeFused) {
    pb->lastRoute = MMX_ROUTE_FUSED;
    MMX_HIP(pb->sIters.ensure(B * sizeof(int32_t)));
    MMX_HIP(pb->sStatus.ensure(B * sizeof(int32_t)));
    MMX_HIP(pb->sFinalErr.ensure(B * sizeof(double)));
    mmx::SolveStateDev fst{};
    fst.done = nullptr;
    fst.iterations = iterations != nullptr ? iterations : pb->sIters.as<int32_t>();
    fst.status = status != nullptr ? status : pb->sStatus.as<int32_t>();
    fst.lastError = nullptr;
    fst.finalError = final_error != nullptr ? final_error : pb->sFinalErr.as<double>();
    fst.errorHistory = error_history;
    fst.paramHistory = parameter_history;
    fst.stepHistory = step_history;
    MMX_HIP(pb->sDiag.ensure(B * 4 * sizeof(float)));
    fst.diag = pb->sDiag.as<float>();
    fst.precisionBound = o->precision_bound > 0.f ? o->precision_bound : 1e-5f;
    pb->diagValid = true;
    if (step_history != nullptr && o->max_iterations > 0) {
      MMX_HIP(mmx::zeroAsync(step_history, B * size_t(o->max_iterations) * 2 * sizeof(double), s));
    }
    if (error_history != nullptr && o->max_iterations > 0) {
      MMX_HIP(mmx::zeroAsync(error_history, B * size_t(o->max_iterations) * sizeof(double), s));
    }
    if (parameter_history != nullptr && o->max_iterations > 0) {
      MMX_HIP(mmx::zeroAsync(parameter_history, B * size_t(o->max_iterations) * P * sizeof(float), s));
    }
    mmx::FusedParams fp{};
    fp.lambda = o->regularization;
    fp.threshold = o->threshold;
    fp.minIterations = o->min_iterations;
    fp.maxIterations = o->max_iterations;
    fp.refine = refineSteps(pb);
    fp.doLineSearch = o->do_line_search;
    fp.stepRule = o->step_rule;
    fp.lmLambdaMin = o->lm_lambda_min;
    fp.lmLambdaMax = o->lm_lambda_max;
    fp.lmUp = o->lm_up;
    fp.lmDown = o->lm_down;
    fp.trustRadius = o->trust_region_radius > 0.f ? o->trust_region_radius : 1.f;
    fp.autoAbort = pb->autoAbort ? 1 : 0;
    long long* clk = nullptr;
    if (phaseClocksWanted()) {
      MMX_HIP(pb->sClk.ensure(32 * sizeof(long long)));
      MMX_HIP(hipMemsetAsync(pb->sClk.p, 0, 32 * sizeof(long long), s));
      clk = pb->sClk.as<long long>();
      MMX_HIP(armPhaseStop(clk, s));
    }
    {
      MMX_ZONE("fused solve: all iterations of GaussNewtonSolverT::doIteration in one launch");
      MMX_HIP(pb->sFusedArgs.ensure(mmx::fusedArgsBytes()));
      MMX_HIP(mmx::launchFusedSolve(pb->rigDev, pb->dev, pb->fdev, theta_dev, fst, fp, nullptr, nullptr, clk, pb->sFusedArgs.p, s));
    }
    if (clk != nullptr) {
      long long h[32];
      MMX_HIP(hipMemcpyAsync(h, clk, sizeof(h), hipMemcpyDeviceToHost, s));
      MMX_HIP(hipStreamSynchronize(s));
      static const char* names[24] = {"A jointParams", "B fk", "C units", "D subtree sums", "E srcTables", "F g + zero tiles",
                                      "G combine + pull", "H cholesky(tail)", "I solve", "J tail (d0 += rho)", "K update",
                                      "G extras: records", "G term records", "H.bc panel", "H.d mfma", "D own sums", "J jd",
                                      "J tangent+own", "J subtree", "J rho", "J solve", "G extras: loads", "H.b load+barrier", "H.b chain"};
      long long tot = h[24] + h[25] + h[26];
      for (int i = 0; i < 24; ++i) {
        tot += h[i];
      }
      fprintf(stderr, "[mmx phase clocks, block 0, all iterations] total %lld  (termRounds %d, numComb %d, nsrc %d, n %d)\n", tot, pb->fdev.termRounds, pb->fdev.numComb, pb->fdev.nsrc, pb->fdev.n);
      for (int i = 0; i < 24; ++i) {
        fprintf(stderr, "  %-16s %10lld  %5.1f%%\n", names[i], h[i], 100.0 * double(h[i]) / double(tot > 0 ? tot : 1));
      }
      fprintf(stderr, "  (of B fk: joint parameters %lld, local transforms %lld, pointer jumping %lld, axes = the rest of B)\n", h[26], h[24], h[25]);
    }
    return MMX_OK;
  }
  if (trust && !(preferWide && treeNormalEquationsUsable(pb) && route != MMX_ROUTE_EXPLICIT_JACOBIAN)) {
    return fail(MMX_ERR_UNSUPPORTED, "MMX_STEP_TRUST_REGION: available in the one-launch solve and on the wide route (tree kernels); this problem takes neither (MMX_ROUTE_EXPLICIT_JACOBIAN, or outside the tree kernels' scope)");
  }
  if (n > mmx::kMaxSolved) {
    return fail(MMX_ERR_UNSUPPORTED, "more than 2048 solved parameters (kMaxModelParams; 512 on the tree routes, the explicit-Jacobian route takes the rest)");
  }
  const bool wide = mmx::choleskyStepLdsBytes(ds.n, ds.M) > 160 * 1024;
  const bool treeRefine = (wide || preferWide) && treeNormalEquationsUsable(pb) && route != MMX_ROUTE_EXPLICIT_JACOBIAN;
  if (route == MMX_ROUTE_WIDE && !treeRefine) {
    return fail(MMX_ERR_UNSUPPORTED, "MMX_ROUTE_WIDE: the tree-refined wide solve is not available for this problem");
  }
  pb->lastRoute = treeRefine ? MMX_ROUTE_WIDE : MMX_ROUTE_EXPLICIT_JACOBIAN;
  rc = ensureStepScratch(pb, !treeRefine);
  if (rc != MMX_OK) {
    return rc;
  }
  MMX_HIP(pb->sThetaInit.ensure(B * P * sizeof(float)));
  MMX_HIP(pb->sDone.ensure(B * sizeof(int32_t)));
  MMX_HIP(pb->sIters.ensure(B * sizeof(int32_t)));
  MMX_HIP(pb->sStatus.ensure(B * sizeof(int32_t)));
  MMX_HIP(pb->sLastErr.ensure(B * sizeof(double)));
  MMX_HIP(pb->sFinalErr.ensure(B * sizeof(double)));
  mmx::SolveStateDev st{};
  st.done = pb->sDone.as<int32_t>();
  st.iterations = iterations != nullptr ? iterations : pb->sIters.as<int32_t>();
  st.status = status != nullptr ? status : pb->sStatus.as<int32_t>();
  st.lastError = pb->sLastErr.as<double>();
  st.finalError = final_error != nullptr ? final_error : pb->sFinalErr.as<double>();
  st.errorHistory = error_history;
  st.paramHistory = nullptr;
  st.stepHistory = step_history;
  pb->diagValid = false;
// ... 29 lines not shown
  sp.diagErr0 = wideDiag ? pb->sDiagErr0.as<float>() : nullptr;
  sp.lambda = o->regularization;
  sp.threshold = o->threshold;
  sp.minIterations = o->min_iterations;
  sp.maxIterations = o->max_iterations;
  sp.refine = refineSteps(pb);
  sp.tileMasks = pb->dTileMasks.as<uint32_t>();
  sp.numTiles = int32_t(pb->tileMasks.tiles.size());
  sp.delta = deferred ? pb->sDelta.as<float>() : nullptr;
  sp.stepIter = deferred ? pb->sStepIter.as<int32_t>() : nullptr;
  sp.lambdaPer = schedule ? pb->sLambda.as<float>() : nullptr;
  sp.stepHistory = step_history;
  sp.doLineSearch = trust ? 0 : o->do_line_search;
  sp.stepRule = o->step_rule;
  if (trust) {
    MMX_HIP(pb->sTrust.ensure(B * 6 * sizeof(int32_t) + 16));
    char* base = static_cast<char*>(pb->sTrust.p);
    sp.tr.lambda = reinterpret_cast<float*>(base);
    sp.tr.radius = reinterpret_cast<float*>(base + B * 4);
    sp.tr.phase = reinterpret_cast<int32_t*>(base + B * 8);
    sp.tr.newton = reinterpret_cast<int32_t*>(base + B * 12);
    sp.tr.step = reinterpret_cast<int32_t*>(base + B * 16);
    sp.tr.mask = reinterpret_cast<int32_t*>(base + B * 20);
    sp.tr.active = reinterpret_cast<int32_t*>(base + B * 24);
    MMX_HIP(mmx::launchTrustInit(sp.tr, pb->B, o->trust_region_radius > 0.f ? o->trust_region_radius : 1.f, s));
  }
  sp.lmLambdaMin = o->lm_lambda_min;
  sp.lmLambdaMax = o->lm_lambda_max;
  sp.lmUp = o->lm_up;
  sp.lmDown = o->lm_down;
  if (phaseClocksWanted()) {
    MMX_HIP(pb->sClk.ensure(32 * sizeof(long long)));
    MMX_HIP(hipMemsetAsync(pb->sClk.p, 0, 32 * sizeof(long long), s));
    sp.clk = pb->sClk.as<long long>();
  }
  float* factorScratch = nullptr;
  if (wide || treeRefine) {
    MMX_HIP(pb->sFactor.ensure(size_t(B) * mmx::choleskyFactorFloats(ds.n) * sizeof(float)));
    factorScratch = pb->sFactor.as<float>();
  }
  const size_t NPs = (size_t(n) + 15) & ~size_t(15);
  float* genState = nullptr;
  if (treeRefine) {
    MMX_HIP(pb->sJtj.ensure(std::max(size_t(B) * size_t(pb->dev.n) * size_t(pb->dev.n), size_t(B) * mmx::choleskyFactorFloats(ds.n)) * sizeof(float)));
    MMX_HIP(pb->sTreeState.ensure(size_t(B) * mmx::treeStateFloats(pb->rig->J, pb->fdev.U) * sizeof(float)));
    MMX_HIP(pb->sDvec.ensure(size_t(B) * NPs * sizeof(float)));
    MMX_HIP(pb->sRhoVec.ensure(size_t(B) * NPs * sizeof(float)));
    MMX_HIP(pb->sRefState.ensure(size_t(B) * sizeof(int32_t)));
    if (pb->fdev.GT > 0) {
      MMX_HIP(pb->sGenState.ensure(size_t(B) * mmx::treeGenStateFloats(pb->fdev.n, pb->fdev.genRows) * sizeof(float)));
      genState = pb->sGenState.as<float>();
    }
  }
  for (int it = 0; it < o->max_iterations; ++it) {
    sp.iteration = it;
    MMX_ZONE("GaussNewtonSolverT::doIteration");
    if (treeRefine) {
      {
        MMX_ZONE("Get JtJ and JtR");
        MMX_HIP(mmx::launchTreeNormalEquations(
            pb->rigDev, pb->dev, pb->fdev, theta_dev, pb->sJtj.as<float>(), pb->sJtr.as<float>(), st.done, pb->sErr.as<double>(),
            pb->sTreeState.as<float>(), sp.clk != nullptr ? sp.clk + 8 : nullptr, genState, true, s));
      }
      MMX_ZONE("Dense gauss newton step");
      auto linearSolve = [&](const mmx::SolveStateDev& who) -> int32_t {
        MMX_HIP(mmx::launchCholeskyFactorTiled(
            ds, pb->rig->P, pb->sJtj.as<float>(), pb->sJtr.as<float>(), factorScratch, pb->sDvec.as<float>(), pb->sRefState.as<int32_t>(),
            pb->sErr.as<double>(), theta_dev, who, sp, s));
        for (int round = 0; round < sp.refine; ++round) {
          MMX_HIP(mmx::launchTreeRefine(
              pb->rigDev, pb->dev, pb->fdev, theta_dev, pb->sTreeState.as<float>(), genState, pb->sDvec.as<float>(), pb->sRhoVec.as<float>(), pb->sRefState.as<int32_t>(),
              sp.lambda, sp.lambdaPer, s));
          MMX_HIP(mmx::launchCholeskyFinishTiled(
              ds, pb->rig->P, factorScratch, pb->sDvec.as<float>(), pb->sRhoVec.as<float>(), pb->sRefState.as<int32_t>(), pb->sErr.as<double>(),
              theta_dev, who, sp, round, s));
        }
        return MMX_OK;
      };
      if (trust) {
        MMX_ZONE("TrustRegionQR: trust steps");
        MMX_HIP(mmx::launchTrustBegin(sp.tr, st, sp.lambdaPer, pb->B, s));
        mmx::SolveStateDev masked = st;
        masked.done = sp.tr.mask;
        for (int pass = 0; pass < 40; ++pass) {
          rc = linearSolve(masked);
          if (rc != MMX_OK) {
            return rc;
          }
          MMX_HIP(mmx::launchTrustDecide(ds, factorScratch, pb->sJtr.as<float>(), pb->sErr.as<double>(), st, sp, s));
          MMX_HIP(mmx::zeroAsync(sp.tr.active, sizeof(int32_t), s));
          MMX_HIP(mmx::launchStepUpdate(pb->rigDev, ds, theta_dev, pb->sJtr.as<float>(), pb->sErr.as<double>(), sp, s));
          int32_t active = 0;
          MMX_HIP(hipMemcpyAsync(&active, sp.tr.active, sizeof(int32_t), hipMemcpyDeviceToHost, s));
          MMX_HIP(hipStreamSynchronize(s));
          if (active == 0) {
            break;
          }
        }
        MMX_HIP(mmx::launchTrustEnd(st, sp, pb->sErr.as<double>(), pb->B, s));
      } else {
        rc = linearSolve(st);
        if (rc != MMX_OK) {
          return rc;
        }
      }
    } else {
      {
        MMX_ZONE("Get JtJ and JtR");
        MMX_HIP(mmx::launchFkJacobian(
            pb->rigDev, pb->dev, theta_dev, pb->sJac.as<float>(), pb->sRes.as<float>(), pb->sErr.as<double>(), nullptr, st.done, s, nullptr, nullptr, true));
        MMX_HIP(mmx::launchNormalEquations(
            ds, pb->rig->P, pb->sJac.as<float>(), pb->sRes.as<float>(), pb->sJtj.as<float>(), pb->sJtr.as<float>(), st.done, wide, s));
      }
      {
        MMX_ZONE("Dense gauss newton step");
        MMX_HIP(mmx::launchCholeskyStep(
            ds, pb->rig->P, pb->sJac.as<float>(), pb->sRes.as<float>(), pb->sJtj.as<float>(), pb->sJtr.as<float>(), pb->sErr.as<double>(),
            theta_dev, st, sp, factorScratch, s));
      }
    }
    if (deferred && !trust) {
      MMX_ZONE("Line search");
      MMX_HIP(mmx::launchStepUpdate(pb->rigDev, ds, theta_dev, pb->sJtr.as<float>(), pb->sErr.as<double>(), sp, s));
    }
// ... 157 lines not shown
        }
      }
      alist = mmx::F64AssemblyList{pb->dF64Groups.as<uint2>(), pb->dF64Extra.as<int32_t>(), pb->dF64ChunkStart.as<int32_t>(), uc};
    }
  }
  MMX_HIP(mmx::launchSolveF64(
      pb->rigDev, pb->dev, pb->dSolveListF64.as<int32_t>(), pb->solveN, theta_dev, st, fp, pb->sJacF64.as<double>(), pb->sHessF64.as<double>(), trustF64 ? pb->sHess2F64.as<double>() : nullptr, s, alist, select));
  return MMX_OK;
}

int32_t mmx_debug_fused_normal_equations(
    mmx_problem* pb,
    const float* theta_dev,
    float* jtj_dev,
    float* jtr_dev,
    int32_t* solve_list_host,
    int32_t* num_solved,
    void* stream) {
  int32_t rc = checkProblem(pb, true);
  if (rc != MMX_OK) {
    return rc;
  }
  const int n = pb->fdev.n;
  if (num_solved != nullptr) {
    *num_solved = n;
  }
  if (solve_list_host != nullptr) {
    std::memcpy(solve_list_host, pb->fused.solveList.data(), sizeof(int32_t) * size_t(n));
  }
  if (theta_dev == nullptr || jtj_dev == nullptr || jtr_dev == nullptr) {
    return MMX_OK;
  }
  if (!fusedUsable(pb)) {
    return fail(MMX_ERR_UNSUPPORTED, "problem shape outside the fused kernel's instantiations");
  }
  const size_t B = size_t(pb->B), P = size_t(pb->rig->P);
  MMX_HIP(hipSetDevice(pb->rig->device));
  hipStream_t s = static_cast<hipStream_t>(stream);
  MMX_HIP(pb->sTheta.ensure(B * P * sizeof(float)));
  MMX_HIP(pb->sIters.ensure(B * sizeof(int32_t)));
  MMX_HIP(pb->sStatus.ensure(B * sizeof(int32_t)));
  MMX_HIP(pb->sFinalErr.ensure(B * sizeof(double)));
  MMX_HIP(hipMemcpyAsync(pb->sTheta.p, theta_dev, B * P * sizeof(float), hipMemcpyDeviceToDevice, s));
  mmx::SolveStateDev fst{};
  fst.iterations = pb->sIters.as<int32_t>();
  fst.status = pb->sStatus.as<int32_t>();
  fst.finalError = pb->sFinalErr.as<double>();
  mmx::FusedParams fp{};
  fp.lambda = 0.05f;
  fp.threshold = 1.f;
  fp.minIterations = 1;
  fp.maxIterations = 1;
  fp.refine = 0;
  MMX_HIP(mmx::launchFusedSolve(pb->rigDev, pb->dev, pb->fdev, pb->sTheta.as<float>(), fst, fp, jtj_dev, jtr_dev, nullptr, nullptr, s));
  return MMX_OK;
}

int32_t mmx_solve_host(
    mmx_problem* pb,
    const mmx_gn_options* o,
    float* theta_host,
    double* final_error_host,
    int32_t* iterations_host,
    int32_t* status_host) {
  MMX_ZONE("mmx_solve_host");
  int32_t rc = checkProblem(pb, true);
  if (rc != MMX_OK) {
    return rc;
  }
  if (theta_host == nullptr) {
    return fail(MMX_ERR_INVALID_ARGUMENT, "theta is null");
  }
  const size_t B = size_t(pb->B), P = size_t(pb->rig->P);
  MMX_HIP(hipSetDevice(pb->rig->device));
  MMX_HIP(pb->sTheta.ensure(B * P * sizeof(float)));
  MMX_HIP(pb->sIters.ensure(B * sizeof(int32_t)));
  MMX_HIP(pb->sStatus.ensure(B * sizeof(int32_t)));
  MMX_HIP(pb->sFinalErr.ensure(B * sizeof(double)));
  MMX_HIP(hipMemcpy(pb->sTheta.p, theta_host, B * P * sizeof(float), hipMemcpyHostToDevice));
  rc = mmx_solve(pb, o, pb->sTheta.as<float>(), pb->sFinalErr.as<double>(), pb->sIters.as<int32_t>(), pb->sStatus.as<int32_t>(), nullptr, nullptr);
  if (rc != MMX_OK) {
    return rc;
  }
  MMX_HIP(hipDeviceSynchronize());
  MMX_HIP(hipMemcpy(theta_host, pb->sTheta.p, B * P * sizeof(float), hipMemcpyDeviceToHost));
  if (final_error_host) {
    MMX_HIP(hipMemcpy(final_error_host, pb->sFinalErr.p, B * sizeof(double), hipMemcpyDeviceToHost));
  }
  if (iterations_host) {
    MMX_HIP(hipMemcpy(iterations_host, pb->sIters.p, B * sizeof(int32_t), hipMemcpyDeviceToHost));
  }
  if (status_host) {
    MMX_HIP(hipMemcpy(status_host, pb->sStatus.p, B * sizeof(int32_t), hipMemcpyDeviceToHost));
  }
  return MMX_OK;
}

int32_t mmx_solve_f64_host(
    mmx_problem* pb,
    const mmx_gn_options* o,
    double* theta_host,
    double* final_error_host,
    int32_t* iterations_host,
    int32_t* status_host) {
  MMX_ZONE("mmx_solve_f64_host");
  int32_t rc = checkProblem(pb, true);
  if (rc != MMX_OK) {
// ... 94 lines not shown
```

### momentum_amd/csrc/mmx_device.hpp

```cpp
#pragma once

#include <hip/hip_runtime.h>

#include <cstdint>

#include "../../include/mmx.h"

namespace mmx {

constexpr int kJs = 17;
constexpr float kPivotFloor = 3.814697265625e-6f;
constexpr float kFactorDamping = 1e-5f;
constexpr float kPrecisionGain = 0.042f;
constexpr float kPivotFloorOrOne = kPivotFloor > 0.f ? kPivotFloor : 1.f;

constexpr float kLn2 = 0.693147180559945309417232121458176568f;

struct F3 {
  float x, y, z;
};
struct Q4 {
  float x, y, z, w;
};

// ... 21 lines not shown
      a.w * b.y + a.y * b.w + a.z * b.x - a.x * b.z,
      a.w * b.z + a.z * b.w + a.x * b.y - a.y * b.x,
      a.w * b.w - a.x * b.x - a.y * b.y - a.z * b.z};
}
__device__ __forceinline__ F3 qrot(Q4 q, F3 v) {
  const F3 qv{q.x, q.y, q.z};
  F3 uv = cross(qv, v);
  uv = uv + uv;
  return v + q.w * uv + cross(qv, uv);
}
__device__ __forceinline__ F3 qmatCol(Q4 q, int c) {
  const float tx = 2.f * q.x, ty = 2.f * q.y, tz = 2.f * q.z;
  const float twx = tx * q.w, twy = ty * q.w, twz = tz * q.w;
  const float txx = tx * q.x, txy = ty * q.x, txz = tz * q.x;
  const float tyy = ty * q.y, tyz = tz * q.y, tzz = tz * q.z;
  if (c == 0) {
    return F3{1.f - (tyy + tzz), txy + twz, txz - twy};
  }
  if (c == 1) {
    return F3{txy - twz, 1.f - (txx + tzz), tyz + twx};
  }
  return F3{txz + twy, tyz - twx, 1.f - (txx + tyy)};
}
__device__ __forceinline__ Q4 qnormalized(Q4 q) {
  const float n2 = q.x * q.x + q.y * q.y + q.z * q.z + q.w * q.w;
  if (n2 > 0.f) {
    const float n = sqrtf(n2);
    return Q4{q.x / n, q.y / n, q.z / n, q.w / n};
  }
  return q;
}

struct ColumnSourceDev {
  int32_t joint, dof, tin, tout, parent;
  float weight;
};

struct JacRecDev {
  int32_t joint, dof, col, tin, tout, parent;
  float weight;
  int32_t valid;
};

struct RigDev {
  int32_t J, P, R, numLevels;
  const int32_t* parent;
  const float* preRot;
  const float* offset;
  const int32_t* ptOuter;
  const int32_t* ptInner;
  const float* ptValue;
  const float* ptOffsets;
  int32_t ptOffsetsNonZero;
  const int32_t* levelOrder;
  const int32_t* levelStart;
  const int4* ptEll;
  const int4* ptRowRec;
  int32_t numRowRec;
  const int32_t* jumpParent;
  int32_t jumpRounds;
  const float* instPreRot;
  const float* instOffset;
};

template <class T>
__device__ __forceinline__ T* asGlobal(T* p) {
  return (T*)(__attribute__((address_space(1))) T*)(unsigned long long)p;
}

__device__ __forceinline__ void selectInstanceRig(RigDev& rig, int b) {
  if (rig.instPreRot != nullptr) {
    rig.preRot = rig.instPreRot + size_t(b) * 4 * size_t(rig.J);
  }
  if (rig.instOffset != nullptr) {
    rig.offset = rig.instOffset + size_t(b) * 3 * size_t(rig.J);
  }
}

struct LossDev {
  int32_t type;
  float alpha, invC2;
  float c;
};
__device__ __forceinline__ float lossValue(const LossDev& l, float s) {
  const float q = s * l.invC2;
  switch (l.type) {
    case 0:
      return q;
    case 1:
      return sqrtf(q + 1.f) - 1.f;
    case 2:
      return logf(0.5f * q + 1.f);
    case 3:
      return 1.f - expf(-0.5f * q);
    default:
      return (powf(q / fabsf(l.alpha - 2.f) + 1.f, 0.5f * l.alpha) - 1.f) * fabsf(l.alpha - 2.f) / l.alpha;
  }
}
__device__ __forceinline__ float lossDeriv(const LossDev& l, float s) {
  const float q = s * l.invC2;
  switch (l.type) {
    case 0:
      return l.invC2;
    case 1:
      return 0.5f * l.invC2 / sqrtf(q + 1.f);
    case 2:
// ... 945 lines not shown
```

### momentum_amd/csrc/mmx_fused.hip

```cpp
#include "mmx_device.hpp"
#include "mmx_kernels.hpp"
#include "mmx_mixed.hpp"
#include "mmx_tree.hpp"

#include <cfloat>
#include <cstdlib>

namespace mmx {

struct FusedLds {
  int16_t* mStart;
  int* mTin;
  int* mInfo;
  float* mW;
  float* th;
  float* js;
  float* up;
  float* ur;
  float* uy;
  float* us;
  float* own1;
  float* sub1;
  float* g;
  float* d0;
// ... 417 lines not shown
  __syncthreads();
  for (int lvl = 1; lvl < rig.numLevels; ++lvl) {
    if (j < rig.J && myLevel == lvl) {
      const double* w = m.js + kJsD * rig.parent[j];
      const DQ qp{w[3], w[4], w[5], w[6]};
      const D3 t = D3{w[0], w[1], w[2]} + dqrot(qp, w[7] * D3{loc[0], loc[1], loc[2]});
      const DQ q = dqmul(qp, DQ{loc[3], loc[4], loc[5], loc[6]});
      slot[0] = t.x, slot[1] = t.y, slot[2] = t.z, slot[3] = q.x, slot[4] = q.y, slot[5] = q.z, slot[6] = q.w, slot[7] = w[7] * loc[7];
    }
    __syncthreads();
  }
  if (withAxes) {
    if (j < rig.J) {
      fkAxesInPlaceD(rig.preRot + 4 * j, j, rig.parent[j], m.js);
    }
    __syncthreads();
  }
}

template <bool kStore>
__device__ __forceinline__ double mixUnits(const ProblemDev& pb, const FusedLds& s, const MixLds& m, int b, int U, int tid) {
  double e = 0.0;
  for (int u = tid; u < U; u += 256) {
    const UnitD un = evalUnitD(pb, loadUnitInput(pb, b, u), m.js, u);
    if (kStore) {
      m.up[3 * u] = un.v.x, m.up[3 * u + 1] = un.v.y, m.up[3 * u + 2] = un.v.z;
      m.uf[3 * u] = un.f.x, m.uf[3 * u + 1] = un.f.y, m.uf[3 * u + 2] = un.f.z;
      m.us[u] = un.sigma;
    }
    e += un.werr;
  }
  return e;
}

template <bool kStore>
__device__ __forceinline__ double blockErrorD(
    const RigView& rig, const ProblemDev& pb, const FusedLds& s, const MixLds& m, const double* th, int b, int U, int tid, int myLevel, double* unrounded = nullptr, const MixRowRec& regRec = MixRowRec{},
    const RigDev* rowsRig = nullptr, bool hasRows = false) {
  blockFkD(rig, m, th, tid, myLevel, kStore, regRec);
  double e = mixUnits<kStore>(pb, s, m, b, U, tid);
  if (hasRows) {
    e += paramRowsErrorD<false>(*rowsRig, pb, rig.P, th, b, tid);
  }
  const double tot = blockSumD(s.red, e, tid);
  if (unrounded != nullptr) {
    *unrounded = tot;
  }
  return double(float(tot));
}

template <class FV, typename YFn>
__device__ __forceinline__ void mixAdjoint(const FV& fd, const FusedLds& s, const MixLds& m, int J, int NP, int n, int nsrc, int tid, YFn yOf, double* out) {
  double *sub, *slot;
  if (size_t(7 * fd.U) <= mixXDoubles(J, nsrc) && size_t(nsrc) <= mixYDoubles(J, 0)) {
    for (int u = tid; u < fd.U; u += 256) {
      const D3 pu{m.up[3 * u], m.up[3 * u + 1], m.up[3 * u + 2]};
      const D3 y = yOf(u, fd.unitPos[u], pu);
      const D3 Nv = dcross(pu, y);
      const bool point = u < fd.Kp;
      double* o = m.X + 7 * u;
      o[0] = point ? y.x : 0.0, o[1] = point ? y.y : 0.0, o[2] = point ? y.z : 0.0;
      o[3] = Nv.x, o[4] = Nv.y, o[5] = Nv.z;
      o[6] = point ? ddot(pu, y) : 0.0;
    }
    __syncthreads();
    for (int item = tid; item < 7 * fd.numLoaded; item += 256) {
      const int li = item / 7, c = item - 7 * li;
      const int k = fd.loadedPos[li];
      double acc = 0.0;
      const int e1 = fd.posUnitStart[k + 1];
      for (int e = fd.posUnitStart[k]; e < e1; ++e) {
        acc += m.X[7 * fd.posUnits[e] + c];
      }
      m.Y[item] = acc;
    }
    __syncthreads();
    for (int item = tid; item < 7 * J; item += 256) {
      const int k = item / 7, c = item - 7 * k;
      double acc = 0.0;
      const int l1 = m.hi[k];
      for (int li = m.lo[k]; li < l1; ++li) {
        acc += m.Y[7 * li + c];
      }
      m.X[item] = acc;
    }
    sub = m.X, slot = m.Y;
  } else {
    for (int li = tid; li < fd.numLoaded; li += 256) {
      const int k = fd.loadedPos[li];
      D3 Fv{0.0, 0.0, 0.0}, Nv{0.0, 0.0, 0.0};
      double Dd = 0.0;
      const int e1 = fd.posUnitStart[k + 1];
      for (int e = fd.posUnitStart[k]; e < e1; ++e) {
        const int u = fd.posUnits[e];
        const D3 pu{m.up[3 * u], m.up[3 * u + 1], m.up[3 * u + 2]};
        const D3 y = yOf(u, k, pu);
        Nv = Nv + dcross(pu, y);
        if (u < fd.Kp) {
          Fv = Fv + y;
          Dd += ddot(pu, y);
        }
      }
      double* o = m.X + 7 * li;
      o[0] = Fv.x, o[1] = Fv.y, o[2] = Fv.z, o[3] = Nv.x, o[4] = Nv.y, o[5] = Nv.z, o[6] = Dd;
    }
    __syncthreads();
    for (int item = tid; item < 7 * J; item += 256) {
// ... 734 lines not shown
}
template <int NB, int MODE, bool kTR, bool kGen = false, int kRule = -1, bool kArgLazy = false, bool kMix = false>
__global__ void __launch_bounds__(256, (NB <= 6 && !kGen ? (FusedFour<NB, kTR, kGen, kRule>::value && !kMix ? 4 : 3) : (NB <= 8 ? 2 : 1))) fusedSolveKernel(
    const FusedArgs* __restrict__ argsDev,
    const RigDev rigArg,
    const ProblemDev pbArg,
    FusedDev fdV,
    float* __restrict__ theta,
    SolveStateDev stV,
    FusedParams fpV,
    float* __restrict__ dbgH,
    float* __restrict__ dbgG,
    long long* __restrict__ dbgClk,
    MixSelect sel) {
  static_assert(!kMix || (!kTR && !kGen && kRule == -1 && !kArgLazy), "the mixed-precision instantiation: generic rule, reference rows");
  constexpr int T = NB * (NB + 1) / 2;
  constexpr int NP = 16 * NB;
  constexpr bool kLook = NB <= 8;
  long long clkLast = 0;
  const int dbgStop = (MODE == 2 && dbgClk != nullptr) ? int(dbgClk[31]) : 0;
#define MMX_CLK(slot)                                             \
  if (MODE == 2 && blockIdx.x == 0 && threadIdx.x == 0) {         \
    const long long now_ = clock64();                             \
    dbgClk[slot] += now_ - clkLast;                               \
    clkLast = now_;                                               \
  }                                                               \
  if (MODE == 2 && dbgStop == (slot) + 1) {                       \
    __builtin_amdgcn_endpgm();                                    \
  }
  extern __shared__ __attribute__((aligned(16))) float smem[];
  int bSel = blockIdx.x;
  if (kMix && sel.map != nullptr) {
    if (int(blockIdx.x) >= *sel.count) {
      return;
    }
    bSel = sel.map[blockIdx.x];
  }
  const int b = bSel, tid = threadIdx.x;
  const int wave = tid >> 6, lane = tid & 63;
  RigDev rigV;
  ProblemDev pbV;
  if (!kArgLazy) {
    rigV = rigArg;
    pbV = pbArg;
    selectInstanceRig(rigV, b);
    selectInstanceWeights(pbV, b);
  }
  const RigDev& rig = kArgLazy ? argsDev->rig : rigV;
  const ProblemDev& pb = kArgLazy ? argsDev->pb : pbV;
  const FusedDev& fd = kArgLazy ? argsDev->fd : fdV;
  const SolveStateDev& st = kArgLazy ? argsDev->st : stV;
  const FusedParams& fp = kArgLazy ? argsDev->fp : fpV;
  const int J = rig.J, P = rig.P, U = fd.U, n = fd.n, nsrc = fd.nsrc;
  const int kR = rig.R;

  FusedLds s;
  int16_t *lParentPos, *lSubSize, *lPosUnitStart, *lPosUnits, *lUnitJoint, *lSolveList, *lDfsJoint, *lLoadedPos, *lColToSolve;
  int *lParent, *lPtOuter = nullptr, *lPtInner = nullptr;
  float *srcGu, *cells, *arena, *lPtValue = nullptr;
  constexpr bool kFour = FusedFour<NB, kTR, kGen, kRule>::value && !kMix;
  constexpr bool kCsrLds = !kFour && !kMix;
  constexpr bool kLeanSolve = kFour;
  constexpr bool kRide = kFour && NB >= 2;
  constexpr bool kLeanOps = kFour;
  constexpr bool kLeanAcc = kFour;
  const int kNnz = fd.nnz;
  const FusedLayout lay = fusedLayout(NB, J, P, U, nsrc, n, fd.numCells, kRule < 0, kGen ? fd.GT : 0, kGen ? fd.genRows : 0, kTR, 0, kMix);
  MixLds m{};
  {
    float* p = smem;
    auto take = [&](size_t count) {
      float* r = p;
      p += alignUp4(count);
      return r;
    };
    auto takeS = [&](size_t count) { return reinterpret_cast<int16_t*>(take((count + 1) / 2)); };
    s.mStart = takeS(NP + 1);
    s.mTin = reinterpret_cast<int*>(take(nsrc));
    s.mInfo = reinterpret_cast<int*>(take(nsrc));
    s.mW = take(nsrc);
    lParent = reinterpret_cast<int*>(take(J));
    lParentPos = takeS(J);
    lSubSize = takeS(J);
    lPosUnitStart = takeS(J + 1);
    lPosUnits = takeS(U);
    lUnitJoint = takeS(U);
    lSolveList = takeS(n);
    lDfsJoint = takeS(J);
    lLoadedPos = takeS(J);
    lColToSolve = takeS(P);
    if (kCsrLds) {
      lPtOuter = reinterpret_cast<int*>(take(kR + 1));
      lPtInner = reinterpret_cast<int*>(take(kNnz));
      lPtValue = take(kNnz);
    }
    if (kMix) {
      s.th = s.js = s.up = s.us = s.ur = s.g = s.d0 = nullptr;
      m.lo = takeS(J);
      m.hi = takeS(J);
    } else {
      s.th = take(P);
      s.js = take(size_t(kJs) * J);
      s.up = take(3 * size_t(U));
      s.ur = take(3 * size_t(U));
      s.us = take(U);
      s.g = take(NP);
      s.d0 = take(NP);
    }
    s.uy = take(lay.uyFloats);
    s.rho = s.uy + lay.auxOff, s.invDiag = s.rho + NP, srcGu = s.rho, cells = s.rho + lay.cellOff;
    s.red = reinterpret_cast<double*>(take(kMix ? 40 : 16));
    s.flags = reinterpret_cast<int*>(take(8));
    s.gEv = s.gRes = s.gW = s.gJ = nullptr;
    if (kGen) {
      const int rowsGp = (fd.genRows + 3) & ~3;
      s.gEv = take(size_t(kGenEv) * size_t(fd.GT));
      s.gRes = take(rowsGp);
      s.gW = take(rowsGp);
      s.gJ = take(size_t(rowsGp) * size_t(srcStrideFor(NP)));
    }
    arena = take(lay.arenaFloats);
    if (kMix) {
      m.X = reinterpret_cast<double*>(arena);
      m.Y = m.X + mixXDoubles(J, nsrc);
    }
    s.srcT = arena;
    s.tanOwn = arena, s.jd = arena + lay.t9, s.tanPre = arena + lay.t9, s.dfull = arena + 2 * lay.t9;
    float* region = p;
    s.fkA = reinterpret_cast<double*>(take(fkBufFloats(J)));
    s.fkB = reinterpret_cast<double*>(p);
    s.own2 = take(size_t(kC2) * J);
    s.sub2 = take(size_t(kC2) * J);
    s.umom = take(lay.umomFloats);
    s.own1 = region, s.sub1 = s.umom;
    s.L = region;
    if (kMix) {
      double* d = reinterpret_cast<double*>(smem + (lay.total - alignUp4(2 * mixPersistentDoubles(J, P, U, NP))));
      m.th = d, d += P;
      m.js = d, d += size_t(kJsD) * J;
      m.up = d, d += 3 * size_t(U);
      m.uf = d, d += 3 * size_t(U);
      m.us = d, d += U;
      m.g = d, d += NP;
      m.x = d, d += NP;
      m.r = d, d += NP;
      m.p = d, d += NP;
      m.q = d;
    }
  }

  float* thg = theta + size_t(b) * P;
  if (kMix) {
    const float* th0 = sel.thetaInit != nullptr ? sel.thetaInit + size_t(b) * P : thg;
    for (int i = tid; i < P; i += 256) {
      m.th[i] = double(th0[i]);
    }
  } else {
    for (int i = tid; i < P; i += 256) {
      s.th[i] = thg[i];
    }
  }
  for (int c = tid; c <= NP; c += 256) {
    s.mStart[c] = int16_t(fd.srcStart[c]);
  }
  for (int e = tid; e < nsrc; e += 256) {
    const ColumnSourceDev cs = fd.srcs[e];
    s.mTin[e] = cs.tin | (cs.tout << 16);
    s.mInfo[e] = cs.joint | (cs.dof << 12) | ((cs.parent + 1) << 16);
    s.mW[e] = cs.weight;
  }
  for (int i = tid; i < J; i += 256) {
    lParent[i] = rig.parent[i];
    lSubSize[i] = int16_t(fd.subSize[i]);
  }
  for (int i = tid; i <= J; i += 256) {
    lPosUnitStart[i] = int16_t(fd.posUnitStart[i]);
  }
  if (kCsrLds) {
    for (int i = tid; i <= kR; i += 256) {
      lPtOuter[i] = rig.ptOuter[i];
    }
    for (int i = tid; i < kNnz; i += 256) {
      lPtInner[i] = rig.ptInner[i];
      lPtValue[i] = rig.ptValue[i];
    }
  }
  for (int i = tid; i < U; i += 256) {
    lPosUnits[i] = int16_t(fd.posUnits[i]);
    lUnitJoint[i] = int16_t(pb.unitTin[i]);
  }
  for (int i = tid; i < n; i += 256) {
    lSolveList[i] = int16_t(fd.solveList[i]);
// ... 786 lines not shown
    MMX_CLK(8)
    const int nRefine = (!notPd && !kMix) ? fp.refine : 0;
    float prevCorr2 = FLT_MAX;
    for (int rf = 0; rf < nRefine; ++rf) {
      {
        auto xd = [&](int c) {
          const int cs = fv.colToSolve[c];
          return cs >= 0 ? s.d0[cs] : 0.f;
        };
        auto od = [&](int r, float a) { s.jd[r] = a; };
        if (kCsrLds) {
          for (int r = tid; r < rv.R; r += 256) {
            float a = 0.f;
            const int k1 = rv.ptOuter[r + 1];
            for (int k = rv.ptOuter[r]; k < k1; ++k) {
              a += rv.ptValue[k] * xd(rv.ptInner[k]);
            }
            od(r, a);
          }
        } else if (rv.rowRec != nullptr) {
          csrRowsFromRecords<256>(rv.rowRec, rv.numRowRec, rv.ptInner, rv.ptValue, rv.R, tid, xd, od);
        } else {
          csrRowsPrefetched<256>(rv.ptOuter, rv.ptInner, rv.ptValue, rv.R, tid, xd, od);
        }
      }
      __syncthreads();
      MMX_CLK(16)
      if (kGen) {
        const int gst = srcStrideFor(NP);
        for (int r = tid; r < fd.genRows; r += 256) {
          float a = s.gRes[r];
          for (int c = 0; c < n; ++c) {
            a -= s.gJ[r * gst + c] * s.d0[c];
          }
          s.gW[r] = a;
        }
      }
      for (int k = tid; k < J; k += 256) {
        const int q = fv.dfsJoint[k];
        const float* ja = s.js + kJs * q;
        const float* d = s.jd + 7 * q;
        const F3 ta{ja[0], ja[1], ja[2]};
        F3 Tv{0.f, 0.f, 0.f};
        if (d[0] != 0.f || d[1] != 0.f || d[2] != 0.f) {
          const int par = rv.parent[q];
          Tv = d[0] * transAxisCol(s.js, par, 0) + d[1] * transAxisCol(s.js, par, 1) + d[2] * transAxisCol(s.js, par, 2);
        }
        const F3 Om = d[3] * F3{ja[8], ja[9], ja[10]} + d[4] * F3{ja[11], ja[12], ja[13]} + d[5] * F3{ja[14], ja[15], ja[16]};
        const F3 C = Tv - cross(Om, ta) - (kLn2 * d[6]) * ta;
        float* o = s.tanOwn + kTan * k;
        o[0] = C.x, o[1] = C.y, o[2] = C.z, o[3] = Om.x, o[4] = Om.y, o[5] = Om.z, o[6] = d[6], o[7] = 0.f;
      }
      __syncthreads();
      if (J <= 256) {
        float acc[7];
        int target = -1;
        if (tid < J) {
#pragma unroll
          for (int c = 0; c < 7; ++c) {
            acc[c] = s.tanOwn[kTan * tid + c];
          }
          target = lParentPos[tid];
          s.tanPre[kTan * tid + 7] = __int_as_float(target);
#pragma unroll
          for (int c = 0; c < 7; ++c) {
            s.tanPre[kTan * tid + c] = acc[c];
          }
        }
        __syncthreads();
        for (int r = 0; r < rv.jumpRounds; ++r) {
          int next = -1;
          if (target >= 0) {
            const float* t = s.tanPre + kTan * target;
#pragma unroll
            for (int c = 0; c < 7; ++c) {
              acc[c] += t[c];
            }
            next = __float_as_int(t[7]);
          }
          __syncthreads();
          if (target >= 0) {
            float* o = s.tanPre + kTan * tid;
#pragma unroll
            for (int c = 0; c < 7; ++c) {
              o[c] = acc[c];
            }
            o[7] = __int_as_float(next);
          }
          target = next;
          __syncthreads();
        }
      } else {
        treeSum<7, false, kTan>(fv, s.tanOwn, s.tanPre, J, wave, lane);
        __syncthreads();
      }
      const bool unitPath = U <= J;
      float* refOwn = unitPath ? arena + lay.t9 : arena;
      float* refSub = unitPath ? arena : arena + lay.t9;
      FusedLds sr = s;
      sr.own1 = refOwn;
      if (unitPath) {
        for (int u = tid; u < U; u += 256) {
          const float* pre = s.tanPre + kTan * fv.unitPos[u];
          const F3 p{s.up[3 * u], s.up[3 * u + 1], s.up[3 * u + 2]};
          const bool point = u < fv.Kp;
          F3 v = cross(F3{pre[3], pre[4], pre[5]}, p);
          if (point) {
            v = F3{pre[0], pre[1], pre[2]} + v + (kLn2 * pre[6]) * p;
          }
          const float sg = s.us[u];
          firstOrderMoments(
              refSub + kC1 * u, p, sg * (s.ur[3 * u] - sg * v.x), sg * (s.ur[3 * u + 1] - sg * v.y), sg * (s.ur[3 * u + 2] - sg * v.z), point);
        }
        __syncthreads();
        gatherOwnSums<kC1, kC1, 256, FusedViewS>(fv, sr, refSub, tid);
      } else {
        for (int k = tid; k < J; k += 256) {
          const int e0 = fv.posUnitStart[k], e1 = fv.posUnitStart[k + 1];
          float a1[kC1] = {0.f, 0.f, 0.f, 0.f, 0.f, 0.f, 0.f};
          if (e1 > e0) {
            const float* pre = s.tanPre + kTan * k;
            for (int e = e0; e < e1; ++e) {
              const int u = fv.posUnits[e];
              const F3 p{s.up[3 * u], s.up[3 * u + 1], s.up[3 * u + 2]};
              const bool point = u < fv.Kp;
              F3 v = cross(F3{pre[3], pre[4], pre[5]}, p);
              if (point) {
                v = F3{pre[0], pre[1], pre[2]} + v + (kLn2 * pre[6]) * p;
              }
              const float sg = s.us[u];
              float o[kC1];
              firstOrderMoments(o, p, sg * (s.ur[3 * u] - sg * v.x), sg * (s.ur[3 * u + 1] - sg * v.y), sg * (s.ur[3 * u + 2] - sg * v.z), point);
#pragma unroll
              for (int c = 0; c < kC1; ++c) {
                a1[c] += o[c];
              }
            }
          }
#pragma unroll
          for (int c = 0; c < kC1; ++c) {
            refOwn[kC1 * k + c] = a1[c];
          }
        }
      }
      __syncthreads();
      MMX_CLK(17)
      treeSum<kC1, true>(fv, refOwn, refSub, J, wave, lane);
      __syncthreads();
      MMX_CLK(18)
      const bool perSource = nsrc <= kTan * J;
      float* perS = refOwn;
      if (perSource) {
        for (int e = tid; e < nsrc; e += 256) {
          const int info = s.mInfo[e];
          perS[e] = s.mW[e] * sourceGradient(info & 0xfff, (info >> 12) & 7, (info >> 16) - 1, s.js, refSub + kC1 * (s.mTin[e] & 0xffff));
        }
        __syncthreads();
      }
      for (int c = tid; c < NP; c += 256) {
        float a = 0.f;
        if (c < n) {
          auto slotShare = [&](int sl) {
            if (perSource) {
              return perS[sl];
            }
            const int info = s.mInfo[sl];
            return s.mW[sl] * sourceGradient(info & 0xfff, (info >> 12) & 7, (info >> 16) - 1, s.js, refSub + kC1 * (s.mTin[sl] & 0xffff));
          };
          a = slotShare(c);
          const int e1 = NP + s.mStart[c + 1];
          for (int e = NP + s.mStart[c]; e < e1; ++e) {
            a += slotShare(e);
          }
          if (hasParamRows) {
            a += paramRowsColumn(rig, pb, fd, s.th, s.d0, lColToSolve, P, b, c, lSolveList[c]).g;
          }
          if (kGen) {
            const int gst = srcStrideFor(NP);
            for (int r = 0; r < fd.genRows; ++r) {
              a += s.gJ[r * gst + c] * s.gW[r];
            }
          }
          a -= mu * s.d0[c];
        }
        s.rho[c] = a;
      }
      __syncthreads();
      MMX_CLK(19)
      solveLLt<NB, kLeanSolve>(s.L, s.invDiag, s.rho, tid);
      MMX_CLK(20)
      float c2 = 0.f, d2 = 0.f;
      for (int c = tid; c < n; c += 256) {
        const float cr = s.rho[c], dn = s.d0[c] + cr;
        s.d0[c] = dn;
        c2 += cr * cr;
        d2 += dn * dn;
      }
      c2 = waveReduceSumF(c2);
      d2 = waveReduceSumF(d2);
      if (lane == 0) {
        s.red[4 + wave] = double(c2);
        s.red[wave] = double(d2);
      }
// ... 450 lines not shown
    out->up = sc + a, out->uy = sc + a + u3, out->us = sc + a + 2 * u3;
    out->umom = sc + endU;
    out->own2 = sc, out->own1 = sc + oOwn1;
    out->sub2 = sc + a, out->sub1 = sc + a + o2;
    out->srcT = sc;
  }
  return X + S;
}

struct TreeNeExtraLds {
  int* col;
  float* pdiag;
  float *gEv, *gRes, *gJ;
  int* unitPos;
};
__host__ __device__ inline size_t treeNeExtraLdsFloats(int P, int n, int GT, int genRows, int U, TreeNeExtraLds* out, float* base) {
  const size_t NP = (size_t(n) + 15) & ~size_t(15), rowsGp = (size_t(genRows) + 3) & ~size_t(3);
  const size_t oCol = 0, oPd = oCol + alignUp4(P), oGev = oPd + NP, oGres = oGev + alignUp4(size_t(kGenEv) * GT), oGj = oGres + rowsGp;
  if (out != nullptr) {
    out->col = reinterpret_cast<int*>(base + oCol), out->pdiag = base + oPd, out->gEv = base + oGev, out->gRes = base + oGres, out->gJ = base + oGj;
  }
  const size_t oUp = oGj + rowsGp * size_t(srcStrideFor(int(NP)));
  if (out != nullptr) {
    out->unitPos = reinterpret_cast<int*>(base + oUp);
  }
  return oUp + alignUp4(U);
}

template <bool kExtraRows, int kWaves = 4, bool kCompact = false>
__global__ void __launch_bounds__(64 * kWaves, kCompact ? 2 : 1) treeNormalEquationsKernel(
    RigDev rig,
    ProblemDev pb,
    FusedDev fd,
    const float* __restrict__ theta,
    float* __restrict__ jtj,
    float* __restrict__ jtr,
    const int32_t* __restrict__ done,
    double* __restrict__ errOut,
    float* __restrict__ state,
    long long* __restrict__ clk,
    float* __restrict__ genState,
    int tileMajor) {
  extern __shared__ __attribute__((aligned(16))) float smem[];
  static_assert(kWaves == 4 || ((kWaves == 8 || kWaves == 16) && !kExtraRows), "the helpers of the extra rows are written for 256 threads");
  constexpr int kT = 64 * kWaves;
  const int b = blockIdx.x, tid = threadIdx.x;
  const int wave = __builtin_amdgcn_readfirstlane(tid >> 6), lane = tid & 63;
  if (done != nullptr && done[b] != 0) {
    return;
  }
  selectInstanceRig(rig, b);
  selectInstanceWeights(pb, b);
  const int J = rig.J, P = rig.P, U = fd.U, n = fd.n, nsrc = fd.nsrc;
  const int NB = (n + 15) >> 4, NP = 16 * NB, T = NB * (NB + 1) / 2;
  static_assert(!kCompact || !kExtraRows, "the compact carve is the plain instantiation's");
  TreeNeLds t;
  const size_t baseFloats = kCompact ? treeNeCompactLdsFloats(J, P, U, nsrc, &t, smem) : treeNeLdsFloats(J, P, U, nsrc, &t, smem);
  TreeNeExtraLds x{};
  if (kExtraRows) {
    treeNeExtraLdsFloats(P, n, fd.GT, fd.genRows, U, &x, smem + baseFloats);
  }
  const bool hasParamRows = kExtraRows && pb.M > pb.rowsJoint;
  const bool hasGen = kExtraRows && fd.GT > 0;
  const int gst = srcStrideFor(NP), rowsGp = (fd.genRows + 3) & ~3;
  if (hasGen) {
    for (int i = tid; i < rowsGp * gst; i += 256) {
      x.gJ[i] = 0.f;
    }
    for (int i = tid; i < rowsGp; i += 256) {
      x.gRes[i] = 0.f;
    }
  }
  long long tclk = clock64();
#define MMX_TCLK(slot)                 \
  if (clk != nullptr && b == 0) {      \
    __syncthreads();                   \
    if (tid == 0) {                    \
      const long long now = clock64(); \
      clk[slot] += now - tclk;         \
      tclk = now;                      \
    }                                  \
  }
  FusedLds s{};
  s.th = t.th, s.js = t.js, s.fkA = t.fkA, s.fkB = t.fkB, s.jd = t.jd;
  s.up = t.up, s.uy = t.uy, s.us = t.us, s.own1 = t.own1, s.own2 = t.own2, s.sub1 = t.sub1, s.sub2 = t.sub2, s.umom = t.umom;
  s.srcT = t.srcT, s.red = t.red;
  RigView rv;
  rv.J = J, rv.P = P, rv.R = rig.R, rv.numLevels = rig.numLevels, rv.jumpRounds = rig.jumpRounds;
  rv.parent = rig.parent, rv.preRot = rig.preRot, rv.offset = rig.offset;
  rv.ptOuter = rig.ptOuter, rv.ptInner = rig.ptInner, rv.ptValue = rig.ptValue, rv.ptOffsets = rig.ptOffsets;
  rv.hasOffsets = rig.ptOffsetsNonZero != 0;
  rv.levelOrder = rig.levelOrder, rv.levelStart = rig.levelStart;
  rv.rowRec = rig.ptRowRec, rv.numRowRec = rig.numRowRec;
  FusedView fv;
  fv.U = U, fv.Kp = fd.Kp, fv.subSize = t.subSize, fv.dfsJoint = fd.dfsJoint, fv.loadedPos = t.loadedPos, fv.numLoaded = fd.numLoaded;
  fv.colToSolve = nullptr, fv.unitPos = pb.unitTin, fv.posUnitStart = t.posUnitStart, fv.posUnits = t.posUnits, fv.solveList = fd.solveList;
  for (int i = tid; i < P; i += kT) {
    s.th[i] = theta[size_t(b) * P + i];
  }
  for (int i = tid; i < J; i += kT) {
    t.subSize[i] = fd.subSize[i];
    t.loadedPos[i] = i < fd.numLoaded ? fd.loadedPos[i] : 0;
  }
  for (int i = tid; i <= J; i += kT) {
    t.posUnitStart[i] = fd.posUnitStart[i];
  }
  for (int i = tid; i < U; i += kT) {
    t.posUnits[i] = fd.posUnits[i];
  }
  for (int e = tid; e < nsrc; e += kT) {
// ... 296 lines not shown
    __syncthreads();
    auto hEntry = [&](int row, int col) {
      return tileMajor ? Ht + size_t(tileIndex(row >> 4, col >> 4)) * 256 + (col & 15) * 16 + (row & 15) : Hb + size_t(row) * n + col;
    };
    for (int c = tid; c < n; c += 256) {
      *hEntry(c, c) += x.pdiag[c];
    }
    if (pb.wLimit > 0.f) {
      const float tWeight = 1e+1f * pb.wLimit;
      for (int d = tid; d < fd.numPairDests; d += 256) {
        float accp = 0.f;
        const int k1 = fd.pairStart[d + 1];
        for (int k = fd.pairStart[d]; k < k1; ++k) {
          const LimitRow row = evalLimit(rig, pb.limits[fd.pairLim[k]], s.th, pb.enabledMask, tWeight);
          float ca = 0.f, cb = 0.f;
#pragma unroll
          for (int e = 0; e < kLimitEntries; ++e) {
            const int sc = row.idx[e] >= 0 ? x.col[row.idx[e]] : -1;
            ca += sc == fd.pairCols[2 * d] ? row.coef[e] : 0.f;
            cb += sc == fd.pairCols[2 * d + 1] ? row.coef[e] : 0.f;
          }
          accp += ca * cb;
        }
        *hEntry(fd.pairCols[2 * d], fd.pairCols[2 * d + 1]) += accp;
      }
    }
  }
  MMX_TCLK(7)
#undef MMX_TCLK
}

size_t treeNormalEquationsLdsBytes(int J, int P, int U, int nsrc, int n, int GT, int genRows) {
  return (treeNeLdsFloats(J, P, U, nsrc, nullptr, nullptr) + treeNeExtraLdsFloats(P, n, GT, genRows, U, nullptr, nullptr)) * sizeof(float);
}
size_t treeGenStateFloats(int n, int genRows) {
  const size_t rowsGp = (size_t(genRows) + 3) & ~size_t(3);
  return rowsGp * size_t(srcStrideFor((n + 15) & ~15)) + rowsGp;
}

hipError_t launchTreeNormalEquations(
    const RigDev& rig,
    const ProblemDev& pb,
    const FusedDev& fd,
    const float* theta,
    float* jtj,
    float* jtr,
    const int32_t* done,
    double* errOut,
    float* state,
    long long* clk,
    float* genState,
    bool tileMajor,
    hipStream_t stream) {
  const size_t lds = treeNormalEquationsLdsBytes(rig.J, rig.P, fd.U, fd.nsrc, fd.n, fd.GT, fd.genRows);
  if (lds > 160 * 1024 - 64) {
    return hipErrorInvalidValue;
  }
  const bool extra = pb.M > pb.rowsJoint || fd.GT > 0 || pb.instPosParent != nullptr || pb.instOriParent != nullptr;
  if (!extra && state != nullptr) {
    const size_t compact = treeNeCompactLdsFloats(rig.J, rig.P, fd.U, fd.nsrc, nullptr, nullptr) * sizeof(float);
    if (compact > 0 && compact <= 80 * 1024 - 64) {
      static LdsLimitCache ldsLimitC;
      hipError_t rc = ldsLimitC.ensure(reinterpret_cast<const void*>(treeNormalEquationsKernel<false, 8, true>), compact);
      if (rc != hipSuccess) {
        return rc;
      }
      hipLaunchKernelGGL((treeNormalEquationsKernel<false, 8, true>), dim3(pb.B), dim3(512), compact, stream, rig, pb, fd, theta, jtj, jtr, done, errOut, state, clk, genState, tileMajor ? 1 : 0);
      return hipGetLastError();
    }
  }
  if (!extra) {
    constexpr int kNeWaves = 16;
    static LdsLimitCache ldsLimit8;
    hipError_t rc = ldsLimit8.ensure(reinterpret_cast<const void*>(treeNormalEquationsKernel<false, kNeWaves>), lds);
    if (rc != hipSuccess) {
      return rc;
    }
    hipLaunchKernelGGL((treeNormalEquationsKernel<false, kNeWaves>), dim3(pb.B), dim3(64 * kNeWaves), lds, stream, rig, pb, fd, theta, jtj, jtr, done, errOut, state, clk, genState, tileMajor ? 1 : 0);
    return hipGetLastError();
  }
  static LdsLimitCache ldsLimit;
  {
    hipError_t rc = ldsLimit.ensure(reinterpret_cast<const void*>(treeNormalEquationsKernel<true>), lds);
    if (rc != hipSuccess) {
      return rc;
    }
  }
  hipLaunchKernelGGL(treeNormalEquationsKernel<true>, dim3(pb.B), dim3(256), lds, stream, rig, pb, fd, theta, jtj, jtr, done, errOut, state, clk, genState, tileMajor ? 1 : 0);
  return hipGetLastError();
}

struct TreeRefLds {
  float *js, *up, *ur, *us, *jd, *tanOwn, *tanPre, *own1, *sub1, *d0, *th, *gJ, *gRes;
  int *col, *subSize, *loadedPos, *posUnitStart, *posUnits, *kRange, *unitPos;
};
__host__ __device__ inline size_t treeRefineLdsFloats(int J, int P, int U, int n, TreeRefLds* out, float* base, int genRows = 0) {
  size_t off = 0;
  auto take = [&](size_t count) {
    const size_t o = off;
    off += alignUp4(count);
    return o;
  };
  const size_t NP = (size_t(n) + 15) & ~size_t(15);
  const size_t oJs = take(size_t(kJs) * J), oUp = take(3 * size_t(U)), oUr = take(3 * size_t(U)), oUs = take(U);
  const size_t r1 = size_t(kC1) * (U > J ? U : J);
  const size_t oR1 = take(r1 > 7 * size_t(J) ? r1 : 7 * size_t(J));
  const size_t oR2 = take(size_t(kTan > kC1 ? kTan : kC1) * J);
  const size_t oPre = take(size_t(kTan) * J);
  const size_t oD = take(NP), oCol = take(P), oSub = take(J), oLoaded = take(J), oPus = take(size_t(J) + 1), oPu = take(U);
  const size_t oKr = take(2 * ((size_t(J) + 15) / 16)), oTh = take(P);
  const size_t rowsGp = (size_t(genRows) + 3) & ~size_t(3);
  const size_t oGj = take(rowsGp * size_t(srcStrideFor(int(NP)))), oGres = take(rowsGp), oUpos = take(U);
  if (out != nullptr) {
    out->gJ = base + oGj, out->gRes = base + oGres;
    out->unitPos = reinterpret_cast<int*>(base + oUpos);
    out->kRange = reinterpret_cast<int*>(base + oKr);
    out->th = base + oTh;
    out->posUnitStart = reinterpret_cast<int*>(base + oPus), out->posUnits = reinterpret_cast<int*>(base + oPu);
    out->subSize = reinterpret_cast<int*>(base + oSub), out->loadedPos = reinterpret_cast<int*>(base + oLoaded);
    out->js = base + oJs, out->up = base + oUp, out->ur = base + oUr, out->us = base + oUs;
    out->jd = base + oR1, out->sub1 = base + oR1, out->tanOwn = base + oR2, out->own1 = base + oR2, out->tanPre = base + oPre;
    out->d0 = base + oD;
    out->col = reinterpret_cast<int*>(base + oCol);
  }
  return off;
}

template <int kWaves>
__global__ void __launch_bounds__(64 * kWaves, kWaves == 4 ? 2 : 1) treeRefineKernel(
    RigDev rig,
    ProblemDev pb,
    FusedDev fd,
    const float* __restrict__ theta,
    const float* __restrict__ state,
    const float* __restrict__ genState,
    const float* __restrict__ dvec,
    float* __restrict__ rhoVec,
    const int32_t* __restrict__ refState,
    float lambdaAll,
    const float* __restrict__ lambdaPer) {
  extern __shared__ __attribute__((aligned(16))) float smem[];
  constexpr int kT = 64 * kWaves;
  const int b = blockIdx.x, tid = threadIdx.x;
  const int wave = __builtin_amdgcn_readfirstlane(tid >> 6), lane = tid & 63;
  if (refState[b] != 0) {
    return;
  }
  selectInstanceWeights(pb, b);
  const int J = rig.J, P = rig.P, U = fd.U, n = fd.n;
  const int NP = (n + 15) & ~15;
  const float lambda = lambdaPer != nullptr ? lambdaPer[b] : lambdaAll;
  TreeRefLds t;
  treeRefineLdsFloats(J, P, U, n, &t, smem, fd.genRows);
  const bool hasGen = fd.GT > 0 && genState != nullptr;
  const int gst = srcStrideFor(NP), rowsGp = (fd.genRows + 3) & ~3;
  FusedLds s{};
  s.js = t.js, s.up = t.up, s.ur = t.ur, s.us = t.us, s.own1 = t.own1, s.sub1 = t.sub1, s.jd = t.jd, s.tanOwn = t.tanOwn, s.tanPre = t.tanPre, s.d0 = t.d0;
  FusedView fv;
  fv.U = U, fv.Kp = fd.Kp, fv.subSize = t.subSize, fv.dfsJoint = fd.dfsJoint, fv.loadedPos = t.loadedPos, fv.numLoaded = fd.numLoaded;
  fv.colToSolve = t.col, fv.unitPos = pb.unitTin, fv.posUnitStart = t.posUnitStart, fv.posUnits = t.posUnits, fv.solveList = fd.solveList;
  {
    const TreeStateLayout sl = treeStateLayout(J, U);
    const float* stb = state + size_t(b) * sl.total;
    for (int i = tid; i < kJs * J; i += kT) {
      s.js[i] = stb[sl.js + i];
    }
    for (int i = tid; i < 3 * U; i += kT) {
      s.up[i] = stb[sl.up + i];
      s.ur[i] = stb[sl.ur + i];
    }
    for (int i = tid; i < U; i += kT) {
      s.us[i] = stb[sl.us + i];
    }
    for (int i = tid; i < NP; i += kT) {
      s.d0[i] = i < n ? dvec[size_t(b) * NP + i] : 0.f;
    }
    for (int i = tid; i < P; i += kT) {
      t.col[i] = -1;
      t.th[i] = theta[size_t(b) * P + i];
    }
    if (hasGen) {
      const float* gs = genState + size_t(b) * (size_t(rowsGp) * gst + rowsGp);
      for (int i = tid; i < rowsGp * gst; i += kT) {
        t.gJ[i] = gs[i];
      }
      for (int i = tid; i < rowsGp; i += kT) {
        t.gRes[i] = gs[size_t(rowsGp) * gst + i];
      }
    }
    for (int i = tid; i < J; i += kT) {
      t.subSize[i] = fd.subSize[i];
      t.loadedPos[i] = i < fd.numLoaded ? fd.loadedPos[i] : 0;
    }
    for (int i = tid; i <= J; i += kT) {
      t.posUnitStart[i] = fd.posUnitStart[i];
    }
    for (int i = tid; i < U; i += kT) {
      t.posUnits[i] = fd.posUnits[i];
    }
  }
  __syncthreads();
  if (pb.instPosParent != nullptr || pb.instOriParent != nullptr) {
    fv.numLoaded = buildInstanceUnitTables(pb, fd, b, J, U, tid, t.unitPos, t.posUnitStart, t.posUnits, t.loadedPos);
    fv.unitPos = t.unitPos;
  }
  treeSumRanges(t.subSize, t.loadedPos, fv.numLoaded, J, tid, t.kRange);
  for (int c = tid; c < n; c += kT) {
    t.col[fd.solveList[c]] = c;
  }
  if (hasGen) {
    for (int r = tid; r < fd.genRows; r += kT) {
      float a = t.gRes[r];
      for (int c = 0; c < n; ++c) {
        a -= t.gJ[r * gst + c] * s.d0[c];
      }
      t.gRes[r] = a;
    }
  }
  __syncthreads();
  csrRowsPrefetched<kT>(
      rig.ptOuter, rig.ptInner, rig.ptValue, rig.R, tid,
      [&](int c) {
        const int cs = t.col[c];
        return cs >= 0 ? s.d0[cs] : 0.f;
      },
      [&](int r, float a) { s.jd[r] = a; });
  __syncthreads();
  for (int k = tid; k < J; k += kT) {
    const int q = fd.dfsJoint[k];
    const float* ja = s.js + kJs * q;
    const float* d = s.jd + 7 * q;
    const F3 ta{ja[0], ja[1], ja[2]};
    F3 Tv{0.f, 0.f, 0.f};
    if (d[0] != 0.f || d[1] != 0.f || d[2] != 0.f) {
      const int par = rig.parent[q];
      Tv = d[0] * transAxisCol(s.js, par, 0) + d[1] * transAxisCol(s.js, par, 1) + d[2] * transAxisCol(s.js, par, 2);
    }
    const F3 Om = d[3] * F3{ja[8], ja[9], ja[10]} + d[4] * F3{ja[11], ja[12], ja[13]} + d[5] * F3{ja[14], ja[15], ja[16]};
    const F3 C = Tv - cross(Om, ta) - (kLn2 * d[6]) * ta;
    float* o = s.tanOwn + kTan * k;
    o[0] = C.x, o[1] = C.y, o[2] = C.z, o[3] = Om.x, o[4] = Om.y, o[5] = Om.z, o[6] = d[6], o[7] = 0.f;
  }
  __syncthreads();
  treeSumT<7, false, kTan, 8>(fv.subSize, fv.loadedPos, fv.numLoaded, s.tanOwn, s.tanPre, J, wave, kWaves, lane);
  __syncthreads();
  if (U <= J) {
    for (int u = tid; u < U; u += kT) {
      const float* pre = s.tanPre + kTan * fv.unitPos[u];
      const F3 p{s.up[3 * u], s.up[3 * u + 1], s.up[3 * u + 2]};
      const bool point = u < fv.Kp;
      F3 v = cross(F3{pre[3], pre[4], pre[5]}, p);
      if (point) {
        v = F3{pre[0], pre[1], pre[2]} + v + (kLn2 * pre[6]) * p;
      }
      const float sg = s.us[u];
      firstOrderMoments(s.sub1 + kC1 * u, p, sg * (s.ur[3 * u] - sg * v.x), sg * (s.ur[3 * u + 1] - sg * v.y), sg * (s.ur[3 * u + 2] - sg * v.z), point);
    }
    __syncthreads();
    gatherOwnSums<kC1, kC1, kT>(fv, s, s.sub1, tid);
  } else {
    for (int k = tid; k < J; k += kT) {
      const int e0 = fv.posUnitStart[k], e1 = fv.posUnitStart[k + 1];
      float a1[kC1] = {0.f, 0.f, 0.f, 0.f, 0.f, 0.f, 0.f};
      if (e1 > e0) {
        const float* pre = s.tanPre + kTan * k;
        for (int e = e0; e < e1; ++e) {
          const int u = fv.posUnits[e];
          const F3 p{s.up[3 * u], s.up[3 * u + 1], s.up[3 * u + 2]};
          const bool point = u < fv.Kp;
          F3 v = cross(F3{pre[3], pre[4], pre[5]}, p);
          if (point) {
            v = F3{pre[0], pre[1], pre[2]} + v + (kLn2 * pre[6]) * p;
          }
          const float sg = s.us[u];
          float o[kC1];
          firstOrderMoments(o, p, sg * (s.ur[3 * u] - sg * v.x), sg * (s.ur[3 * u + 1] - sg * v.y), sg * (s.ur[3 * u + 2] - sg * v.z), point);
#pragma unroll
          for (int c = 0; c < kC1; ++c) {
            a1[c] += o[c];
          }
        }
      }
#pragma unroll
      for (int c = 0; c < kC1; ++c) {
        s.own1[kC1 * k + c] = a1[c];
      }
    }
  }
  __syncthreads();
  treeSumT<kC1, true, kC1, 8>(fv.subSize, fv.loadedPos, fv.numLoaded, s.own1, s.sub1, J, wave, kWaves, lane, t.kRange);
  __syncthreads();
  for (int c = tid; c < NP; c += kT) {
    float a = 0.f;
    if (c < n) {
      auto slotShare = [&](int e) {
        const ColumnSourceDev cs = fd.srcs[e];
        return cs.weight * sourceGradient(cs.joint, cs.dof, cs.parent, s.js, s.sub1 + kC1 * cs.tin);
      };
      a = slotShare(c);
      const int e1 = fd.slotBase + fd.srcStart[c + 1];
      for (int e = fd.slotBase + fd.srcStart[c]; e < e1; ++e) {
        a += slotShare(e);
      }
      if (pb.M > pb.rowsJoint) {
        a += paramRowsColumn(rig, pb, fd, t.th, s.d0, t.col, P, b, c, fd.solveList[c]).g;
      }
      if (hasGen) {
        for (int r = 0; r < fd.genRows; ++r) {
          a += t.gJ[r * gst + c] * t.gRes[r];
        }
      }
      a -= lambda * s.d0[c];
    }
    rhoVec[size_t(b) * NP + c] = a;
  }
}

size_t treeStateFloats(int J, int U) {
  return treeStateLayout(J, U).total;
}
size_t treeRefineLdsBytes(int J, int P, int U, int n, int genRows) {
  return treeRefineLdsFloats(J, P, U, n, nullptr, nullptr, genRows) * sizeof(float);
}

hipError_t launchTreeRefine(
    const RigDev& rig,
    const ProblemDev& pb,
    const FusedDev& fd,
    const float* theta,
    const float* state,
    const float* genState,
    const float* dvec,
    float* rhoVec,
    const int32_t* refState,
    float lambda,
    const float* lambdaPer,
    hipStream_t stream) {
  const size_t lds = treeRefineLdsBytes(rig.J, rig.P, fd.U, fd.n, fd.genRows);
  if (lds > 160 * 1024 - 64) {
    return hipErrorInvalidValue;
  }
  const bool extra = pb.M > pb.rowsJoint || fd.GT > 0 || pb.instPosParent != nullptr || pb.instOriParent != nullptr;
  if (!extra) {
    constexpr int kRefWaves = 8;
    static LdsLimitCache ldsLimitWide;
    hipError_t rc = ldsLimitWide.ensure(reinterpret_cast<const void*>(treeRefineKernel<kRefWaves>), lds);
    if (rc != hipSuccess) {
      return rc;
    }
    hipLaunchKernelGGL((treeRefineKernel<kRefWaves>), dim3(pb.B), dim3(64 * kRefWaves), lds, stream, rig, pb, fd, theta, state, genState, dvec, rhoVec, refState, lambda, lambdaPer);
    return hipGetLastError();
  }
  static LdsLimitCache ldsLimit;
  {
    hipError_t rc = ldsLimit.ensure(reinterpret_cast<const void*>(treeRefineKernel<4>), lds);
    if (rc != hipSuccess) {
      return rc;
    }
  }
  hipLaunchKernelGGL(treeRefineKernel<4>, dim3(pb.B), dim3(256), lds, stream, rig, pb, fd, theta, state, genState, dvec, rhoVec, refState, lambda, lambdaPer);
  return hipGetLastError();
}
#endif

#if !defined(MMX_FUSED_GROUP) || MMX_FUSED_GROUP == 0
size_t fusedCsrFloats(int J, int nnz) {
  auto a4 = [](size_t x) { return (x + 3) & ~size_t(3); };
  return a4(7 * size_t(J) + 1) + 2 * a4(nnz);
}
size_t fusedLdsBytes(int NB, int J, int P, int U, int nsrc, int n, int numCells, bool cellsBehindRho, int GT, int genRows, bool separateUy, size_t csrFloats, bool mix) {
  return fusedLayout(NB, J, P, U, nsrc, n, numCells, cellsBehindRho, GT, genRows, separateUy, csrFloats, mix).total * sizeof(float);
}
#endif

template <int NB, int MODE, bool kTR, bool kGen = false, int kRule = -1>
static hipError_t launchFusedMode(
    const RigDev& rig,
    const ProblemDev& pb,
    const FusedDev& fd,
    float* theta,
    const SolveStateDev& st,
    const FusedParams& fp,
    float* dbgH,
    float* dbgG,
    long long* dbgClk,
    void* argsBuf,
    hipStream_t stream) {
  constexpr bool kFourL = FusedFour<NB, kTR, kGen, kRule>::value;
  const size_t lds = fusedLdsBytes(NB, rig.J, rig.P, fd.U, fd.nsrc, fd.n, fd.numCells, kRule < 0, kGen ? fd.GT : 0, kGen ? fd.genRows : 0, kTR, kFourL ? 0 : fusedCsrFloats(rig.J, fd.nnz));
  if (lds > 160 * 1024) {
    return hipErrorInvalidValue;
  }
  constexpr bool kLazyBuilt = kFourL && MODE == 0;
  const bool lazy = kLazyBuilt && argsBuf != nullptr && rig.instPreRot == nullptr && rig.instOffset == nullptr && pb.fnWeights == nullptr;
  if (lazy) {
    static LdsLimitCache ldsLimit;
    hipError_t rc = ldsLimit.ensure(reinterpret_cast<const void*>(fusedSolveKernel<NB, MODE, kTR, kGen, kRule, kLazyBuilt>), lds);
    if (rc != hipSuccess) {
      return rc;
    }
    FusedArgs* dst = static_cast<FusedArgs*>(argsBuf);
    hipLaunchKernelGGL(stashFusedArgsKernel, dim3(1), dim3(1), 0, stream, FusedArgs{rig, pb, fd, st, fp}, dst);
    hipLaunchKernelGGL((fusedSolveKernel<NB, MODE, kTR, kGen, kRule, kLazyBuilt>), dim3(pb.B), dim3(256), lds, stream, dst, RigDev{}, ProblemDev{}, FusedDev{}, theta, SolveStateDev{}, FusedParams{}, dbgH, dbgG, dbgClk, MixSelect{});
  } else {
    static LdsLimitCache ldsLimit;
    hipError_t rc = ldsLimit.ensure(reinterpret_cast<const void*>(fusedSolveKernel<NB, MODE, kTR, kGen, kRule, false>), lds);
    if (rc != hipSuccess) {
      return rc;
    }
    hipLaunchKernelGGL((fusedSolveKernel<NB, MODE, kTR, kGen, kRule, false>), dim3(pb.B), dim3(256), lds, stream, static_cast<const FusedArgs*>(nullptr), rig, pb, fd, theta, st, fp, dbgH, dbgG, dbgClk, MixSelect{});
  }
  return hipGetLastError();
}

template <int NB>
static hipError_t launchFusedNB(
    const RigDev& rig,
    const ProblemDev& pb,
    const FusedDev& fd,
    float* theta,
    const SolveStateDev& st,
    const FusedParams& fp,
    float* dbgH,
    float* dbgG,
    long long* dbgClk,
    void* argsBuf,
    hipStream_t stream) {
  if (fd.GT > 0) {
    if (fp.stepRule == 2) {
      return hipErrorInvalidValue;
    }
    if (dbgH != nullptr || dbgG != nullptr) {
      return launchFusedMode<NB, 1, false, true>(rig, pb, fd, theta, st, fp, dbgH, dbgG, nullptr, argsBuf, stream);
    }
    return launchFusedMode<NB, 0, false, true>(rig, pb, fd, theta, st, fp, nullptr, nullptr, nullptr, argsBuf, stream);
  }
  if (fp.stepRule == 2) {
    return launchFusedMode<NB, 0, true>(rig, pb, fd, theta, st, fp, nullptr, nullptr, nullptr, argsBuf, stream);
  }
  if (dbgClk != nullptr) {
    return launchFusedMode<NB, 2, false>(rig, pb, fd, theta, st, fp, dbgH, dbgG, dbgClk, argsBuf, stream);
  }
  if (dbgH != nullptr || dbgG != nullptr) {
    return launchFusedMode<NB, 1, false>(rig, pb, fd, theta, st, fp, dbgH, dbgG, dbgClk, argsBuf, stream);
  }
  if (pb.M == pb.rowsJoint) {
    if (fp.stepRule == 0 && fp.doLineSearch == 0) {
      return launchFusedMode<NB, 0, false, false, 0>(rig, pb, fd, theta, st, fp, nullptr, nullptr, nullptr, argsBuf, stream);
    }
    if (fp.stepRule == 1) {
      return launchFusedMode<NB, 0, false, false, 1>(rig, pb, fd, theta, st, fp, nullptr, nullptr, nullptr, argsBuf, stream);
    }
  }
  return launchFusedMode<NB, 0, false>(rig, pb, fd, theta, st, fp, dbgH, dbgG, dbgClk, argsBuf, stream);
}

template <int NB>
static hipError_t launchFusedMixedNB(const RigDev& rig, const ProblemDev& pb, const FusedDev& fd, float* theta, const SolveStateDev& st, const FusedParams& fp, const MixSelect& sel, int blocks, long long* dbgClk, hipStream_t stream) {
  const size_t lds = fusedLdsBytes(NB, rig.J, rig.P, fd.U, fd.nsrc, fd.n, fd.numCells, true, 0, 0, false, 0, true);
  if (lds > 160 * 1024) {
    return hipErrorInvalidValue;
  }
  if (NB == 6 && dbgClk != nullptr) {
    static LdsLimitCache ldsLimitClk;
    hipError_t rc = ldsLimitClk.ensure(reinterpret_cast<const void*>(fusedSolveKernel<NB == 6 ? 6 : 1, 2, false, false, -1, false, true>), lds);
    if (rc != hipSuccess) {
      return rc;
    }
    hipLaunchKernelGGL((fusedSolveKernel<NB == 6 ? 6 : 1, 2, false, false, -1, false, true>), dim3(blocks), dim3(256), lds, stream, static_cast<const FusedArgs*>(nullptr), rig, pb, fd, theta, st, fp, nullptr, nullptr, dbgClk, sel);
    return hipGetLastError();
  }
  static LdsLimitCache ldsLimit;
  hipError_t rc = ldsLimit.ensure(reinterpret_cast<const void*>(fusedSolveKernel<NB, 0, false, false, -1, false, true>), lds);
  if (rc != hipSuccess) {
    return rc;
  }
  hipLaunchKernelGGL((fusedSolveKernel<NB, 0, false, false, -1, false, true>), dim3(blocks), dim3(256), lds, stream, static_cast<const FusedArgs*>(nullptr), rig, pb, fd, theta, st, fp, nullptr, nullptr, nullptr, sel);
  return hipGetLastError();
}

#ifndef MMX_FUSED_GROUP
#define MMX_FUSED_GROUP 0
#endif

#define MMX_FUSED_ARGS \
  const RigDev &rig, const ProblemDev &pb, const FusedDev &fd, float *theta, const SolveStateDev &st, const FusedParams &fp, \
      float *dbgH, float *dbgG, long long *dbgClk, void *argsBuf, hipStream_t stream
#define MMX_FUSED_PASS rig, pb, fd, theta, st, fp, dbgH, dbgG, dbgClk, argsBuf, stream

hipError_t launchFusedGroup0(int nb, MMX_FUSED_ARGS);
hipError_t launchFusedGroup1(int nb, MMX_FUSED_ARGS);
hipError_t launchFusedGroup2(int nb, MMX_FUSED_ARGS);
hipError_t launchFusedGroup3(int nb, MMX_FUSED_ARGS);
#define MMX_MIXED_ARGS \
  const RigDev &rig, const ProblemDev &pb, const FusedDev &fd, float *theta, const SolveStateDev &st, const FusedParams &fp, const MixSelect &sel, int blocks, long long *dbgClk, hipStream_t stream
hipError_t launchFusedMixedGroup5(int nb, MMX_MIXED_ARGS);
hipError_t launchFusedMixedGroup6(int nb, MMX_MIXED_ARGS);
#define MMX_MIXED_CASE(NB_) \
  case NB_:                 \
    return launchFusedMixedNB<NB_>(rig, pb, fd, theta, st, fp, sel, blocks, dbgClk, stream);

#define MMX_CASE(NB_) \
  case NB_:           \
    return launchFusedNB<NB_>(MMX_FUSED_PASS);

#if MMX_FUSED_GROUP == 0
hipError_t launchFusedGroup0(int nb, MMX_FUSED_ARGS) {
  switch (nb) {
    MMX_CASE(1) MMX_CASE(2) MMX_CASE(3) default : return hipErrorInvalidValue;
  }
}
#elif MMX_FUSED_GROUP == 1
// ... 90 lines not shown
```

### momentum_amd/csrc/mmx_host_tables.cpp

```cpp
#include "mmx_host_tables.hpp"

#include <algorithm>

namespace mmx {

int32_t validateRigDesc(const mmx_rig_desc* d, std::string& err) {
  if (d == nullptr) {
    err = "rig descriptor is null";
    return MMX_ERR_INVALID_ARGUMENT;
  }
  const int32_t J = d->num_joints, P = d->num_params;
  if (J <= 0 || P <= 0) {
    err = "rig needs at least one joint and one model parameter";
    return MMX_ERR_INVALID_ARGUMENT;
  }
  if (J > 32767) {
    err = "num_joints exceeds 32767 (joint and level indices are packed into 16 bits on the device)";
    return MMX_ERR_INVALID_ARGUMENT;
  }
  if (P > MMX_MAX_MODEL_PARAMS) {
    err = "num_params exceeds kMaxModelParams (2048)";
    return MMX_ERR_INVALID_ARGUMENT;
  }
  if (!d->parent || !d->pre_rotation || !d->translation_offset || !d->pt_outer || !d->pt_inner || !d->pt_value) {
// ... 257 lines not shown
    markLoaded(f.unitJoint[u]);
  }
  for (const std::vector<int32_t>* lst : {unionPos, unionOri}) {
    if (lst != nullptr) {
      for (int32_t j : *lst) {
        markLoaded(j);
      }
    }
  }
  std::vector<uint8_t> hasPoint(J, 0);
  auto markPoint = [&](int32_t a) {
    while (a >= 0 && !hasPoint[a]) {
      hasPoint[a] = 1;
      a = d->parent[a];
    }
  };
  for (int32_t c = 0; c < Kp; ++c) {
    markPoint(posParent[c]);
  }
  if (unionPos != nullptr) {
    for (int32_t j : *unionPos) {
      markPoint(j);
    }
  }
  f.solveList.clear();
  f.srcStart.assign(1, 0);
  f.srcs.clear();
  f.structNonZero.assign(size_t(P), 0);
  for (int32_t p : t.eliminationList) {
    bool nz = false;
    for (int32_t e = t.colStart[p]; e < t.colStart[p + 1]; ++e) {
      const ColumnSource& s = t.colSources[e];
      const bool rot = s.dof >= 3 && s.dof < 6;
      if (rot ? loaded[s.joint] : hasPoint[s.joint]) {
        nz = true;
      }
    }
    f.structNonZero[size_t(p)] = nz ? 1 : 0;
    if (!nz && !(forceSolve != nullptr && forceSolve[p] != 0)) {
      continue;
    }
    f.solveList.push_back(p);
    for (int32_t e = t.colStart[p]; nz && e < t.colStart[p + 1]; ++e) {
      const ColumnSource& s = t.colSources[e];
      const bool rot = s.dof >= 3 && s.dof < 6;
      if (rot ? loaded[s.joint] : hasPoint[s.joint]) {
        f.srcs.push_back(s);
      }
    }
    f.srcStart.push_back(int32_t(f.srcs.size()));
  }
  (void)err;
  return MMX_OK;
}

TileMasks eliminationTileMasks(int32_t n, const std::vector<uint8_t>& related, bool dense) {
  TileMasks m;
  const int32_t NB = (n + 15) / 16;
  m.NB = NB;
  if (NB > 32) {
    return m;
  }
  for (int32_t I = 0; I < NB; ++I) {
    m.rowMask[I] = dense ? (I == 31 ? 0xffffffffu : ((1u << (I + 1)) - 1u)) : (1u << I);
  }
  if (!dense) {
    for (int32_t row = 0; row < n; ++row) {
      for (int32_t col = 0; col < row; ++col) {
        if (related[size_t(row) * size_t(n) + size_t(col)]) {
          m.rowMask[row >> 4] |= 1u << (col >> 4);
        }
      }
    }
    for (int32_t k = 0; k < NB; ++k) {
      for (int32_t a = k + 1; a < NB; ++a) {
        if (!(m.rowMask[a] >> k & 1u)) {
          continue;
        }
        for (int32_t bb = k + 1; bb <= a; ++bb) {
          if (m.rowMask[bb] >> k & 1u) {
            m.rowMask[a] |= 1u << bb;
          }
        }
      }
    }
  }
  for (int32_t I = 0; I < NB; ++I) {
    for (int32_t k = 0; k <= I; ++k) {
      if (m.rowMask[I] >> k & 1u) {
        m.colMask[k] |= 1u << I;
        m.tiles.push_back(I | (k << 8));
        const uint32_t below = k == 0 ? 0u : ((1u << k) - 1u);
        m.products += __builtin_popcount(m.rowMask[I] & m.rowMask[k] & below);
      }
    }
  }
  {
    int32_t level[32] = {};
    int32_t maxLevel = -1;
    for (int32_t k = 0; k < NB; ++k) {
      int32_t lv = 0;
      for (int32_t j = 0; j < k; ++j) {
        if (m.rowMask[k] >> j & 1u) {
          lv = std::max(lv, level[j] + 1);
        }
      }
// ... 109 lines not shown
```

### momentum_amd/csrc/mmx_host_tables.hpp

```cpp
#pragma once

#include <cstdint>
#include <string>
#include <vector>

#include "../../include/mmx.h"

namespace mmx {

struct ColumnSource {
  int32_t joint;
  int32_t dof;
  int32_t tin;
  int32_t tout;
  int32_t parent;
  float weight;
};

struct JacRec {
  int32_t joint, dof, col, tin, tout, parent;
  float weight;
  int32_t valid;
};

// ... 11 lines not shown
  std::vector<int32_t> colStart;
  std::vector<ColumnSource> colSources;
  int32_t maxColSources = 0;
  std::vector<JacRec> jacRecs;
  std::vector<int32_t> multiCols;
  std::vector<int32_t> zeroCols;
};

struct FusedTables {
  int32_t U = 0;
  std::vector<int32_t> dfsJoint;
  std::vector<int32_t> subSize;
  std::vector<int32_t> unitJoint;
  std::vector<int32_t> posUnitStart;
  std::vector<int32_t> posUnits;
  std::vector<uint8_t> structNonZero;
  std::vector<int32_t> solveList;
  std::vector<int32_t> srcStart;
  std::vector<ColumnSource> srcs;
  int32_t maxDepth = 0;
};

int32_t buildFusedTables(
    const mmx_rig_desc* d,
    const HostTables& t,
    int32_t Kp,
    const int32_t* posParent,
    int32_t Ko,
    const int32_t* oriParent,
    const uint8_t* forceSolve,
    const std::vector<int32_t>* unionPos,
    const std::vector<int32_t>* unionOri,
    FusedTables& out,
    std::string& err);

struct TileMasks {
  int32_t NB = 0;
  uint32_t rowMask[32] = {};
  uint32_t colMask[32] = {};
  std::vector<int32_t> tiles;
  int64_t products = 0;
  std::vector<int32_t> levelSteps;
};
TileMasks eliminationTileMasks(int32_t n, const std::vector<uint8_t>& related , bool dense);

struct F64AssemblyListHost {
  std::vector<uint32_t> groups;
  std::vector<int32_t> extra, chunkStart;
};
bool buildF64AssemblyListHost(
    const HostTables& t, const std::vector<int32_t>& solveList, const int32_t* posParent, int32_t Kp, const int32_t* oriParent, int32_t Ko,
    int32_t unitsPerChunk, F64AssemblyListHost& out);

int32_t validateRigDesc(const mmx_rig_desc* d, std::string& err);

int32_t buildHostTables(const mmx_rig_desc* d, const uint8_t* enabled, HostTables& out, std::string& err);

}
```

### momentum_amd/csrc/mmx_mixed.hpp

```cpp
#pragma once

#include "mmx_device.hpp"
#include "mmx_device_d.hpp"

namespace mmx {

constexpr int kJsD = 17;
constexpr int kTanD = 8;
constexpr float kMixFactorDamping = 1e-6f;
constexpr double kLn2D = 0.693147180559945309417232121458176568;

struct MixLds {
  double* th;
  double* js;
  double* up;
  double* uf;
  double* us;
  double* g;
  double* x;
  double* r;
  double* p;
  double* q;
  double* X;
  double* Y;
  int16_t* lo;
  int16_t* hi;
};
__host__ __device__ inline size_t mixXDoubles(int J, int nsrc) {
  return size_t(7 * J > nsrc ? 7 * J : nsrc);
}
__host__ __device__ inline size_t mixYDoubles(int J, int P) {
  return size_t(kTanD * J > P ? kTanD * J : P);
}
__host__ __device__ inline size_t mixPersistentDoubles(int J, int P, int U, int NP) {
  return size_t(P) + size_t(kJsD) * J + 7 * size_t(U) + 5 * size_t(NP);
}

__device__ __forceinline__ void mixSinCos(double x, double* sOut, double* cOut) {
  if (!(fabs(x) < 1e5)) {
    x = fma(-rint(x * 1.59154943091895335769e-01), 6.28318530717958647693e+00, x);
  }
  const double fn = rint(x * 6.36619772367581382433e-01);
  double r = fma(-fn, 1.57079632673412561417e+00, x);
  r = fma(-fn, 6.07710050650619224932e-11, r);
  const int q = int(fn) & 3;
  const double z = r * r;
  const double ps = 8.33333333332248946124e-03 + z * (-1.98412698298579493134e-04 + z * (2.75573137070700676789e-06 + z * (-2.50507602534068634195e-08 + z * 1.58969099521155010221e-10)));
  const double sn = r + (z * r) * (-1.66666666666666324348e-01 + z * ps);
  const double pc = z * (4.16666666666666019037e-02 + z * (-1.38888888888741095749e-03 + z * (2.48015872894767294178e-05 + z * (-2.75573143513906633035e-07 + z * (2.08757232129817482790e-09 + z * -1.13596475577881948265e-11)))));
  const double hz = 0.5 * z, w = 1.0 - hz;
  const double cs = w + (((1.0 - w) - hz) + z * pc);
  const double sv = (q & 1) ? cs : sn, cv = (q & 1) ? sn : cs;
  *sOut = (q & 2) ? -sv : sv;
  *cOut = ((q + 1) & 2) ? -cv : cv;
}
__device__ __forceinline__ void fkLocalFromParamsD(const double* p, const float* pre, const float* off, double* o, double* oq) {
  double sx, cx, sy, cy, sz, cz;
  mixSinCos(0.5 * p[3], &sx, &cx);
  mixSinCos(0.5 * p[4], &sy, &cy);
  mixSinCos(0.5 * p[5], &sz, &cz);
  const DQ q0{double(pre[0]), double(pre[1]), double(pre[2]), double(pre[3])};
  const DQ q1 = dqmul(q0, DQ{0.0, 0.0, sz, cz});
  const DQ q2 = dqmul(q1, DQ{0.0, sy, 0.0, cy});
  const DQ ql = dqmul(q2, DQ{sx, 0.0, 0.0, cx});
  o[0] = double(off[0]) + p[0], o[1] = double(off[1]) + p[1], o[2] = double(off[2]) + p[2];
  o[3] = ql.x, o[4] = ql.y, o[5] = ql.z, o[6] = ql.w;
  o[7] = exp2(p[6]);
  oq[0] = q1.x, oq[1] = q1.y, oq[2] = q1.z, oq[3] = q1.w;
  oq[4] = q2.x, oq[5] = q2.y, oq[6] = q2.z, oq[7] = q2.w;
}
__device__ __forceinline__ void fkStoreLocalDD(double* bufA, int Jp, int j, const double* o, int parentPlus1) {
  FkXf x;
  x.tx = o[0], x.ty = o[1], x.tz = o[2], x.qx = o[3], x.qy = o[4], x.qz = o[5], x.qw = o[6];
  x.s = o[7], x.jl = parentPlus1;
  fkStoreD(bufA, Jp, j, x);
}
__device__ __forceinline__ void fkAxesInPlaceD(const float* pre, int j, int par, double* js) {
  DQ qp{0.0, 0.0, 0.0, 1.0};
  if (par >= 0) {
// ... 116 lines not shown
```

Baseline: 2.097 million solves/s.

## Prune joints not referenced by constraints into a compacted solve view

```diff
diff --git a/include/mmx.h b/include/mmx.h
--- a/include/mmx.h
+++ b/include/mmx.h
@@ -211,10 +211,12 @@
   int32_t max_refinement_steps;
   float mixed_tolerance;
   int32_t mixed_max_cg;
-  int32_t reserved[4];
+  int32_t joint_pruning;
+  int32_t reserved[3];
 } mmx_tuning;
 int32_t mmx_problem_set_tuning(mmx_problem* problem, const mmx_tuning* tuning);
 int32_t mmx_problem_last_route(const mmx_problem* problem);
+int32_t mmx_problem_num_solve_joints(const mmx_problem* problem);
 
 int32_t mmx_problem_num_rows(const mmx_problem* problem);
 int32_t mmx_problem_batch(const mmx_problem* problem);
@@ -369,6 +371,7 @@
 
 int32_t mmx_host_elimination_order(const mmx_rig_desc* desc, const uint8_t* enabled, int32_t* order, int32_t* num_enabled);
 int32_t mmx_host_tile_structure(int32_t n, const uint8_t* related, uint32_t* row_mask, uint32_t* col_mask, int64_t* products);
+int32_t mmx_host_live_joints(const mmx_rig_desc* desc, int32_t n, const int32_t* joints, uint8_t* live, int32_t* compact_of, int32_t* num_live);
 int32_t mmx_problem_tile_structure(mmx_problem* problem, uint32_t* row_mask, uint32_t* col_mask, int32_t* num_blocks, int32_t* num_tiles, int64_t* products);
 int32_t mmx_host_tile_level_schedule(int32_t n, const uint8_t* related, int32_t* steps);
 int32_t mmx_host_f64_assembly_list(
diff --git a/momentum_amd/_abi.py b/momentum_amd/_abi.py
--- a/momentum_amd/_abi.py
+++ b/momentum_amd/_abi.py
@@ -325,7 +325,7 @@
 
 class Tuning(C.Structure):
 
-    _fields_ = [("route", C.c_int32), ("max_refinement_steps", C.c_int32), ("mixed_tolerance", C.c_float), ("mixed_max_cg", C.c_int32), ("reserved", C.c_int32 * 4)]
+    _fields_ = [("route", C.c_int32), ("max_refinement_steps", C.c_int32), ("mixed_tolerance", C.c_float), ("mixed_max_cg", C.c_int32), ("joint_pruning", C.c_int32), ("reserved", C.c_int32 * 3)]
 
 
 def as_ptr(a: np.ndarray, ctype):
diff --git a/momentum_amd/capi.py b/momentum_amd/capi.py
--- a/momentum_amd/capi.py
+++ b/momentum_amd/capi.py
@@ -18,11 +18,11 @@
     "mmx_gn_options_default", "mmx_abi_version", "mmx_last_error", "mmx_device_count",
     "mmx_rig_create", "mmx_rig_destroy", "mmx_rig_num_joints", "mmx_rig_num_params",
     "mmx_problem_create", "mmx_problem_destroy", "mmx_problem_num_rows", "mmx_problem_batch",
-    "mmx_problem_set_tuning", "mmx_problem_last_route",
+    "mmx_problem_set_tuning", "mmx_problem_last_route", "mmx_problem_num_solve_joints",
     "mmx_problem_set_enabled", "mmx_problem_set_constraints", "mmx_problem_set_constraints_sized", "mmx_problem_set_instance_rig", "mmx_problem_set_instance_parents", "mmx_eval_jacobian", "mmx_eval_jacobian_timed", "mmx_debug_store_pattern",
     "mmx_eval_skeleton_state", "mmx_eval_normal_equations", "mmx_solve", "mmx_solve_with_history", "mmx_solve_with_step_history", "mmx_problem_solve_diagnostics", "mmx_solve_f64", "mmx_solve_f64_host", "mmx_solve_host",
     "mmx_eval_jacobian_host", "mmx_eval_skeleton_state_host", "mmx_host_tables", "mmx_debug_fused_normal_equations", "mmx_debug_tree_normal_equations",
-    "mmx_host_elimination_order", "mmx_host_tile_structure", "mmx_host_tile_level_schedule", "mmx_host_f64_assembly_list", "mmx_problem_tile_structure",
+    "mmx_host_elimination_order", "mmx_host_tile_structure", "mmx_host_tile_level_schedule", "mmx_host_f64_assembly_list", "mmx_problem_tile_structure", "mmx_host_live_joints",
     "mmx_comm_unique_id", "mmx_comm_create", "mmx_comm_create_all", "mmx_comm_world_size", "mmx_comm_rank",
     "mmx_comm_all_reduce_norms", "mmx_comm_all_reduce_norms_host", "mmx_residual_norms", "mmx_comm_destroy",
 ]
@@ -63,6 +63,7 @@
     L.mmx_problem_set_enabled.argtypes = [vp, _abi.c_uint8_p]
     L.mmx_problem_set_tuning.argtypes = [vp, C.POINTER(_abi.Tuning)]
     L.mmx_problem_last_route.argtypes = [vp]
+    L.mmx_problem_num_solve_joints.argtypes = [vp]
     L.mmx_problem_set_constraints.argtypes = [vp, C.POINTER(ConstraintData), vp]
     L.mmx_problem_set_constraints_sized.argtypes = [vp, C.POINTER(ConstraintData), C.c_size_t, vp]
     L.mmx_problem_set_instance_rig.argtypes = [vp, vp, vp, i32, vp]
@@ -102,6 +103,7 @@
     L.mmx_host_tile_structure.argtypes = [i32, _abi.c_uint8_p, u32p, u32p, i64p]
     L.mmx_host_tile_level_schedule.argtypes = [i32, _abi.c_uint8_p, C.POINTER(C.c_int32)]
     L.mmx_problem_tile_structure.argtypes = [vp, u32p, u32p, _abi.c_int32_p, _abi.c_int32_p, i64p]
+    L.mmx_host_live_joints.argtypes = [C.POINTER(RigDesc), i32, _abi.c_int32_p, _abi.c_uint8_p, _abi.c_int32_p, _abi.c_int32_p]
     _lib = L
     return L
 
@@ -137,6 +139,17 @@
     _check(lib().mmx_host_elimination_order(C.byref(d), eptr, as_ptr(order, C.c_int32), C.byref(n)))
     return dict(level=level, tin=tin, tout=tout, active_joint_params=active, enabled_list=elist[: n.value].copy(),
                 elimination_order=order[: n.value].copy())
+
+
+def host_live_joints(rig: Rig, joints) -> dict:
+    J = rig.num_joints
+    jl = np.ascontiguousarray(joints, dtype=np.int32).reshape(-1)
+    live, compact = np.zeros(J, np.uint8), np.zeros(J, np.int32)
+    n = C.c_int32(0)
+    d = rig.desc()
+    jptr = as_ptr(jl, C.c_int32) if jl.size else _abi.c_int32_p()
+    _check(lib().mmx_host_live_joints(C.byref(d), C.c_int32(jl.size), jptr, as_ptr(live, C.c_uint8), as_ptr(compact, C.c_int32), C.byref(n)))
+    return dict(live=live, compact_of=compact, num_live=int(n.value))
 
 
 def host_tile_structure(related: np.ndarray):
@@ -269,12 +282,20 @@
         t.route = _abi.ROUTES[route]
         t.max_refinement_steps = int(max_refinement_steps)
         t.mixed_tolerance, t.mixed_max_cg = getattr(self, "_mixed", (0.0, 0))
+        t.joint_pruning = 0 if getattr(self, "_joint_pruning", True) else -1
         self._route_args = (route, int(max_refinement_steps))
         _check(lib().mmx_problem_set_tuning(self._h, C.byref(t)))
 
     def set_mixed(self, tolerance: float = 0.0, max_cg: int = 0) -> None:
         self._mixed = (float(tolerance), int(max_cg))
         self._set_tuning(*getattr(self, "_route_args", ("auto", 0)))
+
+    def set_joint_pruning(self, on: bool = True) -> None:
+        self._joint_pruning = bool(on)
+        self._set_tuning(*getattr(self, "_route_args", ("auto", 0)))
+
+    def num_solve_joints(self) -> int:
+        return int(lib().mmx_problem_num_solve_joints(self._h))
 
     def last_route(self) -> str:
         r = int(lib().mmx_problem_last_route(self._h))
diff --git a/momentum_amd/csrc/mmx_capi.hip b/momentum_amd/csrc/mmx_capi.hip
--- a/momentum_amd/csrc/mmx_capi.hip
+++ b/momentum_amd/csrc/mmx_capi.hip
@@ -218,6 +218,13 @@
   bool autoAbort = false;
   mmx_tuning tuning{};
   int32_t lastRoute = MMX_ROUTE_AUTO;
+  mmx::LiveJoints liveJoints;
+  bool viewBuilt = false;
+  mmx::RigDev vRig{};
+  int32_t vNnz = 0;
+  DevBuf vParent, vPreRot, vOffset, vPtOuter, vPtInner, vPtValue, vPtOffsets, vLevelOrder, vLevelStart, vPtEll, vJumpParent, vPtRowRec;
+  DevBuf vUnitJoint, vUnitTin, vJointTin, vGenJoint, vGenTin, vEllipsoids, vLimits;
+  DevBuf vSubSize, vDfsJoint, vLoadedPos, vPosUnitStart, vSrcs;
 };
 
 namespace {
@@ -254,6 +261,267 @@
       break;
   }
   return out;
+}
+
+struct RigDerived {
+  std::vector<int32_t> ell, jumpParent, rowRec;
+  bool ellOk = true;
+  int32_t jumpRounds = 0;
+};
+RigDerived deriveRigTables(
+    int32_t J, int32_t P, const std::vector<int32_t>& parent, const std::vector<int32_t>& ptOuter, const std::vector<int32_t>& ptInner,
+    const std::vector<float>& ptValue, int32_t numLevels) {
+  RigDerived o;
+  const int32_t R = MMX_PARAMS_PER_JOINT * J;
+  o.ell.assign(size_t(R) * 4, 0);
+  o.jumpParent.assign(size_t(J), 0);
+  for (int32_t row = 0; row < R; ++row) {
+    const int32_t k0 = ptOuter[size_t(row)], k1 = ptOuter[size_t(row) + 1];
+    if (k1 - k0 > 2) {
+      o.ellOk = false;
+      break;
+    }
+    for (int s = 0; s < 2; ++s) {
+      int32_t idx = -1, bits = 0;
+      if (k0 + s < k1) {
+        idx = ptInner[size_t(k0 + s)];
+        std::memcpy(&bits, &ptValue[size_t(k0 + s)], 4);
+      }
+      o.ell[4 * size_t(row) + 2 * s] = idx;
+      o.ell[4 * size_t(row) + 2 * s + 1] = bits;
+    }
+  }
+  for (int32_t j = 0; j < J; ++j) {
+    o.jumpParent[size_t(j)] = ((parent[size_t(j)] + 1) << 16) | (parent[size_t(j)] + 1);
+  }
+  if (R < 65536 && P <= 65535) {
+    std::vector<int32_t> rows;
+    for (int32_t row = 0; row < R; ++row) {
+      if (ptOuter[size_t(row) + 1] > ptOuter[size_t(row)]) {
+        rows.push_back(row);
+      }
+    }
+    for (size_t t = 0; t < rows.size(); ++t) {
+      const int32_t row = rows[t], next = t + 1 < rows.size() ? rows[t + 1] : R;
+      const int32_t k0 = ptOuter[size_t(row)], cnt = ptOuter[size_t(row) + 1] - k0;
+      if (cnt > 65535 || next - row > 65535) {
+        o.rowRec.clear();
+        break;
+      }
+      int32_t bits = 0;
+      std::memcpy(&bits, &ptValue[size_t(k0)], 4);
+      o.rowRec.insert(o.rowRec.end(), {row | ((next - row) << 16), ptInner[size_t(k0)] | (cnt << 16), bits, k0});
+    }
+  }
+  while ((1 << o.jumpRounds) < numLevels) {
+    ++o.jumpRounds;
+  }
+  return o;
+}
+
+std::vector<int32_t> referencedJoints(const mmx_problem* pb) {
+  std::vector<int32_t> ref(pb->posParent);
+  ref.insert(ref.end(), pb->oriParent.begin(), pb->oriParent.end());
+  for (const auto& h : pb->blocks) {
+    ref.insert(ref.end(), h->parent.begin(), h->parent.end());
+    ref.insert(ref.end(), h->parentB.begin(), h->parentB.end());
+  }
+  for (const mmx_ellipsoid_limit& e : pb->ellipsoids) {
+    ref.push_back(e.parent);
+    ref.push_back(e.ellipsoid_parent);
+  }
+  for (const mmx_parameter_limit& lm : pb->limits) {
+    if (lm.type == MMX_LIMIT_MINMAX_JOINT || lm.type == MMX_LIMIT_LINEAR_JOINT) {
+      ref.push_back(lm.index0 / MMX_PARAMS_PER_JOINT);
+    }
+    if (lm.type == MMX_LIMIT_LINEAR_JOINT) {
+      ref.push_back(lm.index1 / MMX_PARAMS_PER_JOINT);
+    }
+  }
+  return ref;
+}
+
+int32_t uploadSolveView(mmx_problem* pb, const std::vector<mmx::ColumnSource>& slots) {
+  const mmx_rig* rig = pb->rig;
+  pb->viewBuilt = false;
+  const std::vector<int32_t> ref = referencedJoints(pb);
+  mmx::LiveJoints& lj = pb->liveJoints;
+  mmx::buildLiveJoints(rig->parent.data(), rig->J, ref.data(), int32_t(ref.size()), lj);
+  if (lj.identity() || pb->instPos || pb->instOri) {
+    return MMX_OK;
+  }
+  const mmx::HostTables& t = pb->tables;
+  const mmx::FusedTables& f = pb->fused;
+  const int32_t J = rig->J, Jc = lj.numLive;
+  const size_t nJ = size_t(J), nJc = size_t(Jc), nU = size_t(std::max(pb->U, 1));
+  std::vector<int32_t> parent(nJc), ptOuter(1, 0), ptInner;
+  std::vector<float> preRot(4 * nJc), offset(3 * nJc), ptValue, ptOffsets;
+  for (int32_t c = 0; c < Jc; ++c) {
+    const int32_t j = lj.fullOf[size_t(c)];
+    parent[size_t(c)] = rig->parent[size_t(j)] < 0 ? rig->parent[size_t(j)] : lj.compactOf[size_t(rig->parent[size_t(j)])];
+    std::copy_n(&rig->preRot[4 * size_t(j)], 4, &preRot[4 * size_t(c)]);
+    std::copy_n(&rig->offset[3 * size_t(j)], 3, &offset[3 * size_t(c)]);
+    for (int32_t d = 0; d < MMX_PARAMS_PER_JOINT; ++d) {
+      const size_t row = size_t(MMX_PARAMS_PER_JOINT) * size_t(j) + size_t(d);
+      ptInner.insert(ptInner.end(), rig->ptInner.begin() + rig->ptOuter[row], rig->ptInner.begin() + rig->ptOuter[row + 1]);
+      ptValue.insert(ptValue.end(), rig->ptValue.begin() + rig->ptOuter[row], rig->ptValue.begin() + rig->ptOuter[row + 1]);
+      ptOuter.push_back(int32_t(ptInner.size()));
+      ptOffsets.push_back(rig->ptOffsets[row]);
+    }
+  }
+  std::vector<int32_t> levelStart, levelOrder(nJc), posOf(nJ, -1), cTin(nJc), cTout(nJc);
+  {
+    int32_t maxLevel = 0;
+    for (int32_t j : lj.fullOf) {
+      maxLevel = std::max(maxLevel, t.level[size_t(j)]);
+    }
+    levelStart.assign(size_t(maxLevel) + 2, 0);
+    for (int32_t j : lj.fullOf) {
+      levelStart[size_t(t.level[size_t(j)]) + 1]++;
+    }
+    for (int32_t l = 0; l <= maxLevel; ++l) {
+      levelStart[size_t(l) + 1] += levelStart[size_t(l)];
+    }
+    std::vector<int32_t> cursor(levelStart.begin(), levelStart.end() - 1);
+    for (int32_t c = 0; c < Jc; ++c) {
+      levelOrder[size_t(cursor[size_t(t.level[size_t(lj.fullOf[size_t(c)])])]++)] = c;
+    }
+    int32_t next = 0;
+    for (int32_t k = 0; k < J; ++k) {
+      if (lj.live[size_t(f.dfsJoint[size_t(k)])]) {
+        posOf[size_t(k)] = next++;
+      }
+    }
+    std::vector<int32_t> liveBefore(nJ + 1, 0);
+    for (int32_t k = 0; k < J; ++k) {
+      liveBefore[size_t(k) + 1] = liveBefore[size_t(k)] + (posOf[size_t(k)] >= 0 ? 1 : 0);
+    }
+    for (int32_t c = 0; c < Jc; ++c) {
+      const int32_t j = lj.fullOf[size_t(c)];
+      cTin[size_t(c)] = liveBefore[size_t(t.tin[size_t(j)])];
+      cTout[size_t(c)] = liveBefore[size_t(t.tout[size_t(j)])];
+    }
+  }
+  const int32_t numLevels = int32_t(levelStart.size()) - 1;
+  const RigDerived rd = deriveRigTables(Jc, rig->P, parent, ptOuter, ptInner, ptValue, numLevels);
+  MMX_HIP(upload(pb->vParent, parent));
+  MMX_HIP(upload(pb->vPreRot, preRot));
+  MMX_HIP(upload(pb->vOffset, offset));
+  MMX_HIP(upload(pb->vPtOuter, ptOuter));
+  MMX_HIP(upload(pb->vPtInner, ptInner));
+  MMX_HIP(upload(pb->vPtValue, ptValue));
+  MMX_HIP(upload(pb->vPtOffsets, ptOffsets));
+  MMX_HIP(upload(pb->vLevelOrder, levelOrder));
+  MMX_HIP(upload(pb->vLevelStart, levelStart));
+  if (rd.ellOk) {
+    MMX_HIP(upload(pb->vPtEll, rd.ell));
+  }
+  MMX_HIP(upload(pb->vJumpParent, rd.jumpParent));
+  if (!rd.rowRec.empty()) {
+    MMX_HIP(upload(pb->vPtRowRec, rd.rowRec));
+  }
+  mmx::RigDev& v = pb->vRig;
+  v = rig->dev;
+  v.J = Jc;
+  v.R = MMX_PARAMS_PER_JOINT * Jc;
+  v.numLevels = numLevels;
+  v.parent = pb->vParent.as<int32_t>();
+  v.preRot = pb->vPreRot.as<float>();
+  v.offset = pb->vOffset.as<float>();
+  v.ptOuter = pb->vPtOuter.as<int32_t>();
+  v.ptInner = pb->vPtInner.as<int32_t>();
+  v.ptValue = pb->vPtValue.as<float>();
+  v.ptOffsets = pb->vPtOffsets.as<float>();
+  v.levelOrder = pb->vLevelOrder.as<int32_t>();
+  v.levelStart = pb->vLevelStart.as<int32_t>();
+  v.ptEll = rd.ellOk ? pb->vPtEll.as<int4>() : nullptr;
+  v.ptRowRec = rd.rowRec.empty() ? nullptr : pb->vPtRowRec.as<int4>();
+  v.numRowRec = int32_t(rd.rowRec.size() / 4);
+  v.jumpParent = pb->vJumpParent.as<int32_t>();
+  v.jumpRounds = rd.jumpRounds;
+  v.instPreRot = nullptr;
+  v.instOffset = nullptr;
+  pb->vNnz = ptOuter.back();
+  auto cj = [&](int32_t j) { return j < 0 ? j : lj.compactOf[size_t(j)]; };
+  std::vector<int32_t> unitJoint(nU, 0), unitTin(nU, 0);
+  for (int32_t u = 0; u < pb->U; ++u) {
+    unitJoint[size_t(u)] = cj(f.unitJoint[size_t(u)]);
+    unitTin[size_t(u)] = cTin[size_t(unitJoint[size_t(u)])];
+  }
+  MMX_HIP(upload(pb->vUnitJoint, unitJoint));
+  MMX_HIP(upload(pb->vUnitTin, unitTin));
+  MMX_HIP(upload(pb->vJointTin, cTin));
+  {
+    std::vector<int32_t> gj, gt, gj2, gt2;
+    for (const auto& h : pb->blocks) {
+      for (size_t c = 0; c < h->parent.size(); ++c) {
+        const int32_t j = cj(h->parent[c]), j2 = h->parentB.empty() ? -1 : cj(h->parentB[c]);
+        gj.push_back(j);
+        gt.push_back(cTin[size_t(j)]);
+        gj2.push_back(j2);
+        gt2.push_back(j2 < 0 ? -1 : cTin[size_t(j2)]);
+      }
+    }
+    gj.insert(gj.end(), gj2.begin(), gj2.end());
+    gt.insert(gt.end(), gt2.begin(), gt2.end());
+    MMX_HIP(upload(pb->vGenJoint, gj));
+    MMX_HIP(upload(pb->vGenTin, gt));
+    std::vector<mmx::EllipsoidDev> ed(pb->ellipsoids.size());
+    for (size_t i = 0; i < ed.size(); ++i) {
+      const mmx_ellipsoid_limit& e = pb->ellipsoids[i];
+      std::memcpy(&ed[i], &e, sizeof(e));
+      const int32_t p = cj(e.parent), ep = cj(e.ellipsoid_parent);
+      ed[i].parent = p;
+      ed[i].ellipsoidParent = ep;
+      ed[i].tinParent = cTin[size_t(p)];
+      const bool onChain = cTin[size_t(ep)] <= cTin[size_t(p)] && cTin[size_t(p)] < cTout[size_t(ep)];
+      ed[i].tinStop = onChain ? cTin[size_t(ep)] : -1;
+    }
+    MMX_HIP(upload(pb->vEllipsoids, ed));
+    std::vector<mmx_parameter_limit> lims(pb->limits);
+    auto crow = [&](int32_t row) { return MMX_PARAMS_PER_JOINT * cj(row / MMX_PARAMS_PER_JOINT) + row % MMX_PARAMS_PER_JOINT; };
+    for (mmx_parameter_limit& lm : lims) {
+      if (lm.type == MMX_LIMIT_MINMAX_JOINT || lm.type == MMX_LIMIT_LINEAR_JOINT) {
+        lm.index0 = crow(lm.index0);
+      }
+      if (lm.type == MMX_LIMIT_LINEAR_JOINT) {
+        lm.index1 = crow(lm.index1);
+      }
+    }
+    MMX_HIP(upload(pb->vLimits, lims));
+  }
+  std::vector<int32_t> subSize(nJc), dfsJoint(nJc), loadedPos, posUnitStart(nJc + 1, pb->U);
+  for (int32_t c = 0; c < Jc; ++c) {
+    subSize[size_t(cTin[size_t(c)])] = cTout[size_t(c)] - cTin[size_t(c)];
+    dfsJoint[size_t(cTin[size_t(c)])] = c;
+  }
+  for (int32_t k = 0; k < J; ++k) {
+    if (posOf[size_t(k)] >= 0) {
+      posUnitStart[size_t(posOf[size_t(k)])] = f.posUnitStart[size_t(k)];
+      if (f.posUnitStart[size_t(k) + 1] > f.posUnitStart[size_t(k)]) {
+        loadedPos.push_back(posOf[size_t(k)]);
+      }
+    }
+  }
+  std::vector<mmx::ColumnSource> vs(slots);
+  for (mmx::ColumnSource& cs : vs) {
+    if (cs.tin == cs.tout || !lj.live[size_t(cs.joint)]) {
+      cs = mmx::ColumnSource{0, cs.dof, 0, 0, -1, cs.weight};
+      continue;
+    }
+    const int32_t c = lj.compactOf[size_t(cs.joint)];
+    cs.joint = c;
+    cs.parent = cj(cs.parent);
+    cs.tin = cTin[size_t(c)];
+    cs.tout = cTout[size_t(c)];
+  }
+  MMX_HIP(upload(pb->vSubSize, subSize));
+  MMX_HIP(upload(pb->vDfsJoint, dfsJoint));
+  MMX_HIP(upload(pb->vLoadedPos, loadedPos));
+  MMX_HIP(upload(pb->vPosUnitStart, posUnitStart));
+  MMX_HIP(upload(pb->vSrcs, vs));
+  pb->viewBuilt = true;
+  return MMX_OK;
 }
 
 int32_t uploadProblemTables(mmx_problem* pb) {
@@ -677,6 +945,10 @@
     }
     pb->fdev.GT = pb->dev.G + int32_t(pb->ellipsoids.size());
     pb->fdev.genRows = pb->fdev.GT > 0 ? pb->dev.rowsJoint - 3 * pb->U : 0;
+    const int32_t rcView = uploadSolveView(pb, slots);
+    if (rcView != MMX_OK) {
+      return rcView;
+    }
   }
   {
     const size_t J = size_t(rig->J);
@@ -808,6 +1080,38 @@
   return MMX_OK;
 }
 
+struct SolveView {
+  mmx::RigDev rig;
+  mmx::ProblemDev pb;
+  mmx::FusedDev fd;
+};
+bool solveViewActive(const mmx_problem* pb) {
+  return pb->viewBuilt && pb->tuning.joint_pruning == 0 && pb->rigDev.instPreRot == nullptr && pb->rigDev.instOffset == nullptr &&
+      pb->dev.instPosParent == nullptr && pb->dev.instOriParent == nullptr;
+}
+SolveView solveView(const mmx_problem* pb) {
+  SolveView v{pb->rigDev, pb->dev, pb->fdev};
+  if (!solveViewActive(pb)) {
+    return v;
+  }
+  v.rig = pb->vRig;
+  v.pb.unitJoint = pb->vUnitJoint.as<int32_t>();
+  v.pb.unitTin = pb->vUnitTin.as<int32_t>();
+  v.pb.jointTin = pb->vJointTin.as<int32_t>();
+  v.pb.genJoint = pb->vGenJoint.as<int32_t>();
+  v.pb.genTin = pb->vGenTin.as<int32_t>();
+  v.pb.ellipsoids = pb->vEllipsoids.as<mmx::EllipsoidDev>();
+  v.pb.limits = pb->vLimits.as<mmx::LimitDev>();
+  v.fd.nnz = pb->vNnz;
+  v.fd.subSize = pb->vSubSize.as<int32_t>();
+  v.fd.dfsJoint = pb->vDfsJoint.as<int32_t>();
+  v.fd.loadedPos = pb->vLoadedPos.as<int32_t>();
+  v.fd.unitJoint = pb->vUnitJoint.as<int32_t>();
+  v.fd.posUnitStart = pb->vPosUnitStart.as<int32_t>();
+  v.fd.srcs = pb->vSrcs.as<mmx::ColumnSourceDev>();
+  return v;
+}
+
 bool fusedUsable(const mmx_problem* pb) {
   const int nb = mmx::fusedBlocksFor(pb->fdev.n);
   if (nb < 0) {
@@ -940,6 +1244,34 @@
   }
   if (num_enabled) {
     *num_enabled = int32_t(t.eliminationList.size());
+  }
+  return MMX_OK;
+}
+
+int32_t mmx_host_live_joints(const mmx_rig_desc* desc, int32_t n, const int32_t* joints, uint8_t* live, int32_t* compact_of, int32_t* num_live) {
+  std::string err;
+  const int32_t rc = mmx::validateRigDesc(desc, err);
+  if (rc != MMX_OK) {
+    return fail(rc, err);
+  }
+  if (n < 0 || (n > 0 && joints == nullptr)) {
+    return fail(MMX_ERR_INVALID_ARGUMENT, "mmx_host_live_joints: negative count or null joint list");
+  }
+  for (int32_t i = 0; i < n; ++i) {
+    if (joints[i] < 0 || joints[i] >= desc->num_joints) {
+      return fail(MMX_ERR_INVALID_ARGUMENT, "mmx_host_live_joints: joint index out of range");
+    }
+  }
+  mmx::LiveJoints lj;
+  mmx::buildLiveJoints(desc->parent, desc->num_joints, joints, n, lj);
+  if (live) {
+    std::memcpy(live, lj.live.data(), lj.live.size());
+  }
+  if (compact_of) {
+    std::memcpy(compact_of, lj.compactOf.data(), sizeof(int32_t) * lj.compactOf.size());
+  }
+  if (num_live) {
+    *num_live = lj.numLive;
   }
   return MMX_OK;
 }
@@ -1128,53 +1460,15 @@
   UP(r->dPtOffsets, r->ptOffsets);
   UP(r->dLevelOrder, r->topo.levelOrder);
   UP(r->dLevelStart, r->topo.levelStart);
-  std::vector<int32_t> ell(size_t(R) * 4, 0), jumpParent(size_t(r->J));
-  bool ellOk = true;
-  for (int32_t row = 0; row < R; ++row) {
-    const int32_t k0 = r->ptOuter[row], k1 = r->ptOuter[row + 1];
-    if (k1 - k0 > 2) {
-      ellOk = false;
-      break;
-    }
-    for (int s = 0; s < 2; ++s) {
-      int32_t idx = -1, bits = 0;
-      if (k0 + s < k1) {
-        idx = r->ptInner[k0 + s];
-        std::memcpy(&bits, &r->ptValue[k0 + s], 4);
-      }
-      ell[4 * size_t(row) + 2 * s] = idx;
-      ell[4 * size_t(row) + 2 * s + 1] = bits;
-    }
-  }
-  for (int32_t j = 0; j < r->J; ++j) {
-    jumpParent[j] = ((r->parent[j] + 1) << 16) | (r->parent[j] + 1);
-  }
+  const RigDerived rd = deriveRigTables(r->J, r->P, r->parent, r->ptOuter, r->ptInner, r->ptValue, int32_t(r->topo.levelStart.size()) - 1);
+  const bool ellOk = rd.ellOk;
+  const std::vector<int32_t>& rowRec = rd.rowRec;
   if (ellOk) {
-    UP(r->dPtEll, ell);
-  }
-  UP(r->dJumpParent, jumpParent);
-  std::vector<int32_t> rowRec;
-  if (R < 65536 && r->P <= 65535) {
-    std::vector<int32_t> rows;
-    for (int32_t row = 0; row < R; ++row) {
-      if (r->ptOuter[row + 1] > r->ptOuter[row]) {
-        rows.push_back(row);
-      }
-    }
-    for (size_t t = 0; t < rows.size(); ++t) {
-      const int32_t row = rows[t], next = t + 1 < rows.size() ? rows[t + 1] : R;
-      const int32_t k0 = r->ptOuter[row], cnt = r->ptOuter[row + 1] - k0;
-      if (cnt > 65535 || next - row > 65535) {
-        rowRec.clear();
-        break;
-      }
-      int32_t bits = 0;
-      std::memcpy(&bits, &r->ptValue[k0], 4);
-      rowRec.insert(rowRec.end(), {row | ((next - row) << 16), r->ptInner[k0] | (cnt << 16), bits, k0});
-    }
-    if (!rowRec.empty()) {
-      UP(r->dPtRowRec, rowRec);
-    }
+    UP(r->dPtEll, rd.ell);
+  }
+  UP(r->dJumpParent, rd.jumpParent);
+  if (!rowRec.empty()) {
+    UP(r->dPtRowRec, rowRec);
   }
 #undef UP
   mmx::RigDev& dv = r->dev;
@@ -1182,11 +1476,9 @@
   dv.numRowRec = int32_t(rowRec.size() / 4);
   dv.ptEll = ellOk ? r->dPtEll.as<int4>() : nullptr;
   dv.jumpParent = r->dJumpParent.as<int32_t>();
-  dv.jumpRounds = 0;
-  while ((1 << dv.jumpRounds) < int32_t(r->topo.levelStart.size()) - 1) {
-    ++dv.jumpRounds;
-  }
+  dv.jumpRounds = rd.jumpRounds;
   dv.J = r->J;
+  dv.layoutJ = r->J;
   dv.P = r->P;
   dv.R = R;
   dv.numLevels = int32_t(r->topo.levelStart.size()) - 1;
@@ -1317,6 +1609,9 @@
   if (!(tuning->mixed_tolerance >= 0.f) || tuning->mixed_tolerance > 1e-2f || tuning->mixed_max_cg < 0 || tuning->mixed_max_cg > 64) {
     return fail(MMX_ERR_INVALID_ARGUMENT, "mmx_tuning::mixed_tolerance: 0 (default) or (0, 1e-2]; mixed_max_cg: 0 (default) or 1..64");
   }
+  if (tuning->joint_pruning != 0 && tuning->joint_pruning != -1) {
+    return fail(MMX_ERR_INVALID_ARGUMENT, "mmx_tuning::joint_pruning: 0 (on) or -1 (off)");
+  }
   for (int32_t r : tuning->reserved) {
     if (r != 0) {
       return fail(MMX_ERR_INVALID_ARGUMENT, "mmx_tuning::reserved must be zero");
@@ -1328,6 +1623,13 @@
 
 int32_t mmx_problem_last_route(const mmx_problem* pb) {
   return pb != nullptr ? pb->lastRoute : MMX_ROUTE_AUTO;
+}
+
+int32_t mmx_problem_num_solve_joints(const mmx_problem* pb) {
+  if (pb == nullptr || pb->rig == nullptr) {
+    return 0;
+  }
+  return solveViewActive(pb) ? pb->liveJoints.numLive : pb->rig->J;
 }
 
 int32_t mmx_problem_set_enabled(mmx_problem* pb, const uint8_t* enabled) {
@@ -1976,7 +2278,8 @@
   MMX_HIP(hipSetDevice(pb->rig->device));
   hipStream_t s = static_cast<hipStream_t>(stream);
   MMX_HIP(mmx::zeroAsync(jtj_dev, size_t(pb->B) * size_t(pb->dev.n) * size_t(pb->dev.n) * sizeof(float), s));
-  MMX_HIP(mmx::launchTreeNormalEquations(pb->rigDev, pb->dev, pb->fdev, theta_dev, jtj_dev, jtr_dev, nullptr, nullptr, nullptr, nullptr, nullptr, false, s));
+  const SolveView sv = solveView(pb);
+  MMX_HIP(mmx::launchTreeNormalEquations(sv.rig, sv.pb, sv.fd, theta_dev, jtj_dev, jtr_dev, nullptr, nullptr, nullptr, nullptr, nullptr, false, s));
   return MMX_OK;
 }
 
@@ -2198,7 +2501,8 @@
     clk = pb->sClk.as<long long>();
     MMX_HIP(armPhaseStop(clk, s));
   }
-  MMX_HIP(mmx::launchFusedMixed(pb->rigDev, pb->dev, pb->fdev, theta_dev, fst, fp, sel, pb->B, clk, s));
+  const SolveView sv = solveView(pb);
+  MMX_HIP(mmx::launchFusedMixed(sv.rig, sv.pb, sv.fd, theta_dev, fst, fp, sel, pb->B, clk, s));
   if (clk != nullptr) {
     long long h[32];
     MMX_HIP(hipMemcpyAsync(h, clk, sizeof(h), hipMemcpyDeviceToHost, s));
@@ -2362,7 +2666,8 @@
     wp.doLineSearch = o->do_line_search;
     wp.stepRule = o->step_rule;
     MMX_ZONE("wave solve: all iterations in one launch, one wavefront per instance");
-    MMX_HIP(mmx::launchWaveSolve(pb->rigDev, pb->dev, pb->fdev, theta_dev, wst, wp, s));
+    const SolveView sv = solveView(pb);
+    MMX_HIP(mmx::launchWaveSolve(sv.rig, sv.pb, sv.fd, theta_dev, wst, wp, s));
     return MMX_OK;
   }
   const bool forceWide = route == MMX_ROUTE_WIDE;
@@ -2429,7 +2734,8 @@
     {
       MMX_ZONE("fused solve: all iterations of GaussNewtonSolverT::doIteration in one launch");
       MMX_HIP(pb->sFusedArgs.ensure(mmx::fusedArgsBytes()));
-      MMX_HIP(mmx::launchFusedSolve(pb->rigDev, pb->dev, pb->fdev, theta_dev, fst, fp, nullptr, nullptr, clk, pb->sFusedArgs.p, s));
+      const SolveView sv = solveView(pb);
+      MMX_HIP(mmx::launchFusedSolve(sv.rig, sv.pb, sv.fd, theta_dev, fst, fp, nullptr, nullptr, clk, pb->sFusedArgs.p, s));
     }
     if (clk != nullptr) {
       long long h[32];
@@ -2565,6 +2871,7 @@
       genState = pb->sGenState.as<float>();
     }
   }
+  const SolveView sv = solveView(pb);
   for (int it = 0; it < o->max_iterations; ++it) {
     sp.iteration = it;
     MMX_ZONE("GaussNewtonSolverT::doIteration");
@@ -2572,7 +2879,7 @@
       {
         MMX_ZONE("Get JtJ and JtR");
         MMX_HIP(mmx::launchTreeNormalEquations(
-            pb->rigDev, pb->dev, pb->fdev, theta_dev, pb->sJtj.as<float>(), pb->sJtr.as<float>(), st.done, pb->sErr.as<double>(),
+            sv.rig, sv.pb, sv.fd, theta_dev, pb->sJtj.as<float>(), pb->sJtr.as<float>(), st.done, pb->sErr.as<double>(),
             pb->sTreeState.as<float>(), sp.clk != nullptr ? sp.clk + 8 : nullptr, genState, true, s));
       }
       MMX_ZONE("Dense gauss newton step");
@@ -2582,7 +2889,7 @@
             pb->sErr.as<double>(), theta_dev, who, sp, s));
         for (int round = 0; round < sp.refine; ++round) {
           MMX_HIP(mmx::launchTreeRefine(
-              pb->rigDev, pb->dev, pb->fdev, theta_dev, pb->sTreeState.as<float>(), genState, pb->sDvec.as<float>(), pb->sRhoVec.as<float>(), pb->sRefState.as<int32_t>(),
+              sv.rig, sv.pb, sv.fd, theta_dev, pb->sTreeState.as<float>(), genState, pb->sDvec.as<float>(), pb->sRhoVec.as<float>(), pb->sRefState.as<int32_t>(),
               sp.lambda, sp.lambdaPer, s));
           MMX_HIP(mmx::launchCholeskyFinishTiled(
               ds, pb->rig->P, factorScratch, pb->sDvec.as<float>(), pb->sRhoVec.as<float>(), pb->sRefState.as<int32_t>(), pb->sErr.as<double>(),
@@ -2846,7 +3153,8 @@
   fp.minIterations = 1;
   fp.maxIterations = 1;
   fp.refine = 0;
-  MMX_HIP(mmx::launchFusedSolve(pb->rigDev, pb->dev, pb->fdev, pb->sTheta.as<float>(), fst, fp, jtj_dev, jtr_dev, nullptr, nullptr, s));
+  const SolveView sv = solveView(pb);
+  MMX_HIP(mmx::launchFusedSolve(sv.rig, sv.pb, sv.fd, pb->sTheta.as<float>(), fst, fp, jtj_dev, jtr_dev, nullptr, nullptr, s));
   return MMX_OK;
 }
 
diff --git a/momentum_amd/csrc/mmx_device.hpp b/momentum_amd/csrc/mmx_device.hpp
--- a/momentum_amd/csrc/mmx_device.hpp
+++ b/momentum_amd/csrc/mmx_device.hpp
@@ -97,6 +97,7 @@
   const float* ptValue;
   const float* ptOffsets;
   int32_t ptOffsetsNonZero;
+  int32_t layoutJ;
   const int32_t* levelOrder;
   const int32_t* levelStart;
   const int4* ptEll;
diff --git a/momentum_amd/csrc/mmx_fused.hip b/momentum_amd/csrc/mmx_fused.hip
--- a/momentum_amd/csrc/mmx_fused.hip
+++ b/momentum_amd/csrc/mmx_fused.hip
@@ -493,7 +493,7 @@
 template <class FV, typename YFn>
 __device__ __forceinline__ void mixAdjoint(const FV& fd, const FusedLds& s, const MixLds& m, int J, int NP, int n, int nsrc, int tid, YFn yOf, double* out) {
   double *sub, *slot;
-  if (size_t(7 * fd.U) <= mixXDoubles(J, nsrc) && size_t(nsrc) <= mixYDoubles(J, 0)) {
+  if (size_t(7 * fd.U) <= mixXDoubles(m.layoutJ, nsrc) && size_t(nsrc) <= mixYDoubles(m.layoutJ, 0)) {
     for (int u = tid; u < fd.U; u += 256) {
       const D3 pu{m.up[3 * u], m.up[3 * u + 1], m.up[3 * u + 2]};
       const D3 y = yOf(u, fd.unitPos[u], pu);
@@ -1334,6 +1334,7 @@
   const SolveStateDev& st = kArgLazy ? argsDev->st : stV;
   const FusedParams& fp = kArgLazy ? argsDev->fp : fpV;
   const int J = rig.J, P = rig.P, U = fd.U, n = fd.n, nsrc = fd.nsrc;
+  const int JL = rig.layoutJ;
   const int kR = rig.R;
 
   FusedLds s;
@@ -1347,8 +1348,9 @@
   constexpr bool kLeanOps = kFour;
   constexpr bool kLeanAcc = kFour;
   const int kNnz = fd.nnz;
-  const FusedLayout lay = fusedLayout(NB, J, P, U, nsrc, n, fd.numCells, kRule < 0, kGen ? fd.GT : 0, kGen ? fd.genRows : 0, kTR, 0, kMix);
+  const FusedLayout lay = fusedLayout(NB, JL, P, U, nsrc, n, fd.numCells, kRule < 0, kGen ? fd.GT : 0, kGen ? fd.genRows : 0, kTR, 0, kMix);
   MixLds m{};
+  m.layoutJ = JL;
   {
     float* p = smem;
     auto take = [&](size_t count) {
@@ -1361,15 +1363,15 @@
     s.mTin = reinterpret_cast<int*>(take(nsrc));
     s.mInfo = reinterpret_cast<int*>(take(nsrc));
     s.mW = take(nsrc);
-    lParent = reinterpret_cast<int*>(take(J));
-    lParentPos = takeS(J);
-    lSubSize = takeS(J);
-    lPosUnitStart = takeS(J + 1);
+    lParent = reinterpret_cast<int*>(take(JL));
+    lParentPos = takeS(JL);
+    lSubSize = takeS(JL);
+    lPosUnitStart = takeS(JL + 1);
     lPosUnits = takeS(U);
     lUnitJoint = takeS(U);
     lSolveList = takeS(n);
-    lDfsJoint = takeS(J);
-    lLoadedPos = takeS(J);
+    lDfsJoint = takeS(JL);
+    lLoadedPos = takeS(JL);
     lColToSolve = takeS(P);
     if (kCsrLds) {
       lPtOuter = reinterpret_cast<int*>(take(kR + 1));
@@ -1378,11 +1380,11 @@
     }
     if (kMix) {
       s.th = s.js = s.up = s.us = s.ur = s.g = s.d0 = nullptr;
-      m.lo = takeS(J);
-      m.hi = takeS(J);
+      m.lo = takeS(JL);
+      m.hi = takeS(JL);
     } else {
       s.th = take(P);
-      s.js = take(size_t(kJs) * J);
+      s.js = take(size_t(kJs) * JL);
       s.up = take(3 * size_t(U));
       s.ur = take(3 * size_t(U));
       s.us = take(U);
@@ -1404,22 +1406,22 @@
     arena = take(lay.arenaFloats);
     if (kMix) {
       m.X = reinterpret_cast<double*>(arena);
-      m.Y = m.X + mixXDoubles(J, nsrc);
+      m.Y = m.X + mixXDoubles(JL, nsrc);
     }
     s.srcT = arena;
     s.tanOwn = arena, s.jd = arena + lay.t9, s.tanPre = arena + lay.t9, s.dfull = arena + 2 * lay.t9;
     float* region = p;
-    s.fkA = reinterpret_cast<double*>(take(fkBufFloats(J)));
+    s.fkA = reinterpret_cast<double*>(take(fkBufFloats(JL)));
     s.fkB = reinterpret_cast<double*>(p);
-    s.own2 = take(size_t(kC2) * J);
-    s.sub2 = take(size_t(kC2) * J);
+    s.own2 = take(size_t(kC2) * JL);
+    s.sub2 = take(size_t(kC2) * JL);
     s.umom = take(lay.umomFloats);
     s.own1 = region, s.sub1 = s.umom;
     s.L = region;
     if (kMix) {
-      double* d = reinterpret_cast<double*>(smem + (lay.total - alignUp4(2 * mixPersistentDoubles(J, P, U, NP))));
+      double* d = reinterpret_cast<double*>(smem + (lay.total - alignUp4(2 * mixPersistentDoubles(JL, P, U, NP))));
       m.th = d, d += P;
-      m.js = d, d += size_t(kJsD) * J;
+      m.js = d, d += size_t(kJsD) * JL;
       m.up = d, d += 3 * size_t(U);
       m.uf = d, d += 3 * size_t(U);
       m.us = d, d += U;
@@ -2312,7 +2314,7 @@
         o[0] = C.x, o[1] = C.y, o[2] = C.z, o[3] = Om.x, o[4] = Om.y, o[5] = Om.z, o[6] = d[6], o[7] = 0.f;
       }
       __syncthreads();
-      if (J <= 256) {
+      if (JL <= 256) {
         float acc[7];
         int target = -1;
         if (tid < J) {
@@ -2354,7 +2356,7 @@
         treeSum<7, false, kTan>(fv, s.tanOwn, s.tanPre, J, wave, lane);
         __syncthreads();
       }
-      const bool unitPath = U <= J;
+      const bool unitPath = U <= JL;
       float* refOwn = unitPath ? arena + lay.t9 : arena;
       float* refSub = unitPath ? arena : arena + lay.t9;
       FusedLds sr = s;
@@ -2408,7 +2410,7 @@
       treeSum<kC1, true>(fv, refOwn, refSub, J, wave, lane);
       __syncthreads();
       MMX_CLK(18)
-      const bool perSource = nsrc <= kTan * J;
+      const bool perSource = nsrc <= kTan * JL;
       float* perS = refOwn;
       if (perSource) {
         for (int e = tid; e < nsrc; e += 256) {
@@ -2965,10 +2967,11 @@
   selectInstanceRig(rig, b);
   selectInstanceWeights(pb, b);
   const int J = rig.J, P = rig.P, U = fd.U, n = fd.n, nsrc = fd.nsrc;
+  const int JL = rig.layoutJ;
   const int NB = (n + 15) >> 4, NP = 16 * NB, T = NB * (NB + 1) / 2;
   static_assert(!kCompact || !kExtraRows, "the compact carve is the plain instantiation's");
   TreeNeLds t;
-  const size_t baseFloats = kCompact ? treeNeCompactLdsFloats(J, P, U, nsrc, &t, smem) : treeNeLdsFloats(J, P, U, nsrc, &t, smem);
+  const size_t baseFloats = kCompact ? treeNeCompactLdsFloats(JL, P, U, nsrc, &t, smem) : treeNeLdsFloats(JL, P, U, nsrc, &t, smem);
   TreeNeExtraLds x{};
   if (kExtraRows) {
     treeNeExtraLdsFloats(P, n, fd.GT, fd.genRows, U, &x, smem + baseFloats);
@@ -3371,13 +3374,13 @@
     float* genState,
     bool tileMajor,
     hipStream_t stream) {
-  const size_t lds = treeNormalEquationsLdsBytes(rig.J, rig.P, fd.U, fd.nsrc, fd.n, fd.GT, fd.genRows);
+  const size_t lds = treeNormalEquationsLdsBytes(rig.layoutJ, rig.P, fd.U, fd.nsrc, fd.n, fd.GT, fd.genRows);
   if (lds > 160 * 1024 - 64) {
     return hipErrorInvalidValue;
   }
   const bool extra = pb.M > pb.rowsJoint || fd.GT > 0 || pb.instPosParent != nullptr || pb.instOriParent != nullptr;
   if (!extra && state != nullptr) {
-    const size_t compact = treeNeCompactLdsFloats(rig.J, rig.P, fd.U, fd.nsrc, nullptr, nullptr) * sizeof(float);
+    const size_t compact = treeNeCompactLdsFloats(rig.layoutJ, rig.P, fd.U, fd.nsrc, nullptr, nullptr) * sizeof(float);
     if (compact > 0 && compact <= 80 * 1024 - 64) {
       static LdsLimitCache ldsLimitC;
       hipError_t rc = ldsLimitC.ensure(reinterpret_cast<const void*>(treeNormalEquationsKernel<false, 8, true>), compact);
@@ -3467,10 +3470,11 @@
   }
   selectInstanceWeights(pb, b);
   const int J = rig.J, P = rig.P, U = fd.U, n = fd.n;
+  const int JL = rig.layoutJ;
   const int NP = (n + 15) & ~15;
   const float lambda = lambdaPer != nullptr ? lambdaPer[b] : lambdaAll;
   TreeRefLds t;
-  treeRefineLdsFloats(J, P, U, n, &t, smem, fd.genRows);
+  treeRefineLdsFloats(JL, P, U, n, &t, smem, fd.genRows);
   const bool hasGen = fd.GT > 0 && genState != nullptr;
   const int gst = srcStrideFor(NP), rowsGp = (fd.genRows + 3) & ~3;
   FusedLds s{};
@@ -3563,7 +3567,7 @@
   __syncthreads();
   treeSumT<7, false, kTan, 8>(fv.subSize, fv.loadedPos, fv.numLoaded, s.tanOwn, s.tanPre, J, wave, kWaves, lane);
   __syncthreads();
-  if (U <= J) {
+  if (U <= JL) {
     for (int u = tid; u < U; u += kT) {
       const float* pre = s.tanPre + kTan * fv.unitPos[u];
       const F3 p{s.up[3 * u], s.up[3 * u + 1], s.up[3 * u + 2]};
@@ -3655,7 +3659,7 @@
     float lambda,
     const float* lambdaPer,
     hipStream_t stream) {
-  const size_t lds = treeRefineLdsBytes(rig.J, rig.P, fd.U, fd.n, fd.genRows);
+  const size_t lds = treeRefineLdsBytes(rig.layoutJ, rig.P, fd.U, fd.n, fd.genRows);
   if (lds > 160 * 1024 - 64) {
     return hipErrorInvalidValue;
   }
@@ -3706,7 +3710,7 @@
     void* argsBuf,
     hipStream_t stream) {
   constexpr bool kFourL = FusedFour<NB, kTR, kGen, kRule>::value;
-  const size_t lds = fusedLdsBytes(NB, rig.J, rig.P, fd.U, fd.nsrc, fd.n, fd.numCells, kRule < 0, kGen ? fd.GT : 0, kGen ? fd.genRows : 0, kTR, kFourL ? 0 : fusedCsrFloats(rig.J, fd.nnz));
+  const size_t lds = fusedLdsBytes(NB, rig.layoutJ, rig.P, fd.U, fd.nsrc, fd.n, fd.numCells, kRule < 0, kGen ? fd.GT : 0, kGen ? fd.genRows : 0, kTR, kFourL ? 0 : fusedCsrFloats(rig.layoutJ, fd.nnz));
   if (lds > 160 * 1024) {
     return hipErrorInvalidValue;
   }
@@ -3776,7 +3780,7 @@
 
 template <int NB>
 static hipError_t launchFusedMixedNB(const RigDev& rig, const ProblemDev& pb, const FusedDev& fd, float* theta, const SolveStateDev& st, const FusedParams& fp, const MixSelect& sel, int blocks, long long* dbgClk, hipStream_t stream) {
-  const size_t lds = fusedLdsBytes(NB, rig.J, rig.P, fd.U, fd.nsrc, fd.n, fd.numCells, true, 0, 0, false, 0, true);
+  const size_t lds = fusedLdsBytes(NB, rig.layoutJ, rig.P, fd.U, fd.nsrc, fd.n, fd.numCells, true, 0, 0, false, 0, true);
   if (lds > 160 * 1024) {
     return hipErrorInvalidValue;
   }
diff --git a/momentum_amd/csrc/mmx_host_tables.cpp b/momentum_amd/csrc/mmx_host_tables.cpp
--- a/momentum_amd/csrc/mmx_host_tables.cpp
+++ b/momentum_amd/csrc/mmx_host_tables.cpp
@@ -333,6 +333,30 @@
   }
   (void)err;
   return MMX_OK;
+}
+
+void buildLiveJoints(const int32_t* parent, int32_t J, const int32_t* joints, int32_t n, LiveJoints& out) {
+  out.live.assign(size_t(J), 0);
+  int32_t count = 0;
+  for (int32_t i = 0; i < n; ++i) {
+    for (int32_t a = joints[i]; a >= 0 && a < J && !out.live[size_t(a)]; a = parent[a]) {
+      out.live[size_t(a)] = 1;
+      ++count;
+    }
+  }
+  if (count == 0) {
+    out.live.assign(size_t(J), 1);
+    count = J;
+  }
+  out.numLive = count;
+  out.compactOf.assign(size_t(J), -1);
+  out.fullOf.clear();
+  for (int32_t j = 0; j < J; ++j) {
+    if (out.live[size_t(j)]) {
+      out.compactOf[size_t(j)] = int32_t(out.fullOf.size());
+      out.fullOf.push_back(j);
+    }
+  }
 }
 
 TileMasks eliminationTileMasks(int32_t n, const std::vector<uint8_t>& related, bool dense) {
diff --git a/momentum_amd/csrc/mmx_host_tables.hpp b/momentum_amd/csrc/mmx_host_tables.hpp
--- a/momentum_amd/csrc/mmx_host_tables.hpp
+++ b/momentum_amd/csrc/mmx_host_tables.hpp
@@ -87,6 +87,17 @@
     const HostTables& t, const std::vector<int32_t>& solveList, const int32_t* posParent, int32_t Kp, const int32_t* oriParent, int32_t Ko,
     int32_t unitsPerChunk, F64AssemblyListHost& out);
 
+struct LiveJoints {
+  int32_t numLive = 0;
+  std::vector<uint8_t> live;
+  std::vector<int32_t> compactOf;
+  std::vector<int32_t> fullOf;
+  bool identity() const {
+    return numLive == int32_t(live.size());
+  }
+};
+void buildLiveJoints(const int32_t* parent, int32_t J, const int32_t* joints, int32_t n, LiveJoints& out);
+
 int32_t validateRigDesc(const mmx_rig_desc* d, std::string& err);
 
 int32_t buildHostTables(const mmx_rig_desc* d, const uint8_t* enabled, HostTables& out, std::string& err);
diff --git a/momentum_amd/csrc/mmx_mixed.hpp b/momentum_amd/csrc/mmx_mixed.hpp
--- a/momentum_amd/csrc/mmx_mixed.hpp
+++ b/momentum_amd/csrc/mmx_mixed.hpp
@@ -25,6 +25,7 @@
   double* Y;
   int16_t* lo;
   int16_t* hi;
+  int layoutJ;
 };
 __host__ __device__ inline size_t mixXDoubles(int J, int nsrc) {
   return size_t(7 * J > nsrc ? 7 * J : nsrc);
```

After: 2.227 million solves/s (median of 6 runs). 6.2% higher.
